# jirsat/wavenets

Measured on AMD Instinct MI355X. Metric: audio samples/sec (training step, 16 kHz mu-law), higher is better.
Workload: dtype f32 (fp16 hi|lo split operands, fp32 accumulate)

## Files before the change

### include/wn_hip.h

```cpp
#ifndef WN_HIP_H
#define WN_HIP_H
#include <stdint.h>

#ifdef __cplusplus
extern "C" {
#endif

#define WN_OK 0
#define WN_E_INVALID (-1)
#define WN_E_UNSUPPORTED (-2)
#define WN_E_HIP (-3)

#define WN_ACT_LINEAR 0
#define WN_ACT_RELU 1
#define WN_ACT_LEAKY_RELU 2
#define WN_ACT_TANH 3
#define WN_ACT_SIGMOID 4
#define WN_ACT_ELU 5

#define WN_HEAD_CATEGORICAL 0
#define WN_HEAD_LOGISTIC 1
#define WN_HEAD_GAUSSIAN 2

#define WN_MAX_FINAL 8
#define WN_MAX_MAPPING 8

typedef struct wn_config {
  int32_t kernel_size;
  int32_t channels;
  int32_t blocks;
  int32_t layers_per_block;
  int32_t activation;
  int32_t dilation_bound;
  int32_t num_mixtures;
  int32_t head;
  int32_t bits;
  int32_t skip_channels;
  int32_t dilation_channels;
  int32_t use_residual;
  int32_t use_skip;
  int32_t n_final;
  int32_t final_channels[WN_MAX_FINAL];
  int32_t cond_inputs;
  int32_t n_mapping;
  int32_t mapping_channels[WN_MAX_MAPPING];
  int32_t mapping_activation;
  float l2_reg_factor;
} wn_config;

typedef struct wn_plan wn_plan;

const char* wn_last_error_string(void);

wn_plan* wn_plan_create(const wn_config* cfg);
void wn_plan_destroy(wn_plan* p);

typedef struct wn_exec wn_exec;
wn_exec* wn_exec_create(const wn_plan* p);
void wn_exec_destroy(wn_exec* e);
int wn_exec_bind(wn_exec* e);
int64_t wn_plan_param_count(const wn_plan* p);
int32_t wn_plan_num_tensors(const wn_plan* p);
int wn_plan_tensor_info(const wn_plan* p, int32_t idx, int64_t* offset, int64_t* len,
                        int32_t* ndim, int64_t* shape3, int32_t* is_kernel);
int32_t wn_plan_receptive_field(const wn_plan* p);
int32_t wn_plan_out_channels(const wn_plan* p);
int32_t wn_plan_dilation(const wn_plan* p, int32_t conv_index);
int64_t wn_plan_workspace_floats(const wn_plan* p, int32_t B, int32_t T, int32_t training);

int wn_plan_set_dropout(wn_plan* p, float rate, uint64_t seed, uint64_t step);
uint32_t wn_dropout_key_for(uint64_t seed, int32_t block, uint64_t step);

int wn_debug_set(int key, int value);
int wn_debug_value(int key);
int wn_debug_gen_ts(unsigned long long* out_96);
int wn_plan_describe(const wn_plan* p, char* buf, int32_t len);
int wn_prof_enable(wn_plan* p, int32_t max_launches);
int wn_prof_read(wn_plan* p, int32_t* launches, float* avg_ms);
int wn_debug_ws_region(const wn_plan* p, int32_t B, int32_t T, int32_t what, int32_t idx, int64_t* off,
                       int64_t* len);
int wn_debug_eval_region(const wn_plan* p, int32_t B, int32_t T, int32_t what, int64_t* off, int64_t* len);
int wn_debug_fwd_paths(const wn_plan* p, int32_t B, int32_t T, int32_t training, int32_t loss, char* buf, int32_t len);
int wn_stack_prof_enable(wn_plan* p, int32_t max_passes);
int wn_stack_prof_read(wn_plan* p, int32_t* passes, float* avg_ms);
int wn_stack_prof_read_foldprep(wn_plan* p, int32_t* passes, float* avg_ms);
int wn_phase_enable(wn_plan* p, int32_t on);
int wn_phase_read(wn_plan* p, float* ms4);

int wn_forward(wn_plan* p, const float* params, const float* x, const float* cond, int32_t B,
               int32_t T, float* out, float* logits_out, float* workspace, int64_t ws_floats,
               void* stream);

int wn_forward_training(wn_plan* p, const float* params, const float* x, const float* cond, int32_t B,
                        int32_t T, float* out, float* logits_out, float* workspace, int64_t ws_floats,
                        void* stream);

int wn_train_fwd_bwd(wn_plan* p, const float* params, const float* x_full, const float* cond,
                     int32_t B, int32_t T, int32_t global_batch, int32_t n_replicas, float* grads,
                     float* loss_out, float* pred_out, float* workspace, int64_t ws_floats,
                     void* stream);

int wn_vjp(wn_plan* p, const float* params, const float* x, const float* cond, int32_t B, int32_t T,
           const float* g_out, int32_t g_kind, float* grads, float* g_x, float* g_cond,
           float* workspace, int64_t ws_floats, void* stream);

int wn_eval_loss(wn_plan* p, const float* params, const float* x_full, const float* cond,
                 int32_t B, int32_t T, int32_t global_batch, float* loss_out, float* pred_out,
                 float* workspace, int64_t ws_floats, void* stream);

int wn_score(wn_plan* p, const float* params, const float* x_full, const float* cond, int32_t B, int32_t T,
             float* nll_out, float* weight_out, float* rows_out, float* flag_out,
             float* workspace, int64_t ws_floats, void* stream);

int wn_adam_step(wn_plan* p, float* params, const float* grads, float* m, float* v, int64_t step,
                 float lr, float beta1, float beta2, float eps, float clipnorm, float* scratch,
                 void* stream);
int wn_adam_step_guarded(wn_plan* p, float* params, const float* grads, float* m, float* v, int64_t step,
                         float lr, float beta1, float beta2, float eps, float clipnorm, float* scratch,
                         const float* skip_flag, void* stream);
int wn_adam_step_ema(wn_plan* p, float* params, const float* grads, float* m, float* v, float* ema, int64_t step,
                     float lr, float beta1, float beta2, float eps, float clipnorm, float ema_momentum,
                     int32_t ema_overwrite, float* scratch, const float* skip_flag, void* stream);

int wn_clip_gradients(wn_plan* p, float* grads, float clipnorm, float* scratch, void* stream);

int64_t wn_plan_range_slot(const wn_plan* p, int32_t B, int32_t T, int32_t training);
float wn_range_limit(void);

int wn_generate(wn_plan* p, const float* params, const float* window, const float* cond, int32_t B,
                int32_t length, int32_t deterministic, int32_t queued, uint64_t seed, float* out,
                float* workspace, int64_t ws_floats, void* stream);
typedef struct wn_sampling { float temperature; int32_t top_k; uint64_t seed; float top_p; } wn_sampling;
int wn_generate_sampled(wn_plan* p, const float* params, const float* window, const float* cond, int32_t B,
                        int32_t length, int32_t deterministic, int32_t queued, const wn_sampling* sampling, float* out,
                        float* workspace, int64_t ws_floats, void* stream);
int wn_generate_chunk(wn_plan* p, const float* params, const float* window, const float* cond, int32_t B,
                      int64_t first, int32_t length, int32_t deterministic, int32_t queued, const wn_sampling* sampling,
                      float* out, float* workspace, int64_t ws_floats, void* stream);
typedef struct wn_sampling_row { float T, inv_T; int32_t top_k; float top_p; uint64_t seed, stream; } wn_sampling_row;
#define WN_SAMPLING_ROWS_ON 1
#define WN_SAMPLING_ROWS_TOP_P 2
int64_t wn_sampling_rows_floats(int32_t B);
int wn_sampling_rows_pack(const wn_sampling* sampling, const uint64_t* stream, int32_t B, int32_t head, int32_t classes,
                          wn_sampling_row* rows, int32_t* flags);
int wn_generate_rows_chunk(wn_plan* p, const float* params, const float* window, const float* cond, int32_t B,
                           int64_t first, int32_t length, int32_t deterministic, int32_t queued,
                           const wn_sampling_row* rows, int32_t rows_flags, float* out, float* workspace,
                           int64_t ws_floats, void* stream);
int wn_generate_rows_begin(wn_plan* p, const float* params, const float* window, const float* cond, int32_t B,
                           int64_t first, int32_t length, int32_t deterministic, int32_t queued,
                           const wn_sampling_row* rows, int32_t rows_flags, float* out, float* workspace,
                           int64_t ws_floats, void* stream);
int64_t wn_generate_admit_scratch_floats(const wn_plan* p, int32_t k);
int wn_generate_admit(wn_plan* p, const float* params, const float* windows, const float* cond, int32_t k,
                      const int32_t* slots, int32_t B, int64_t position, int32_t deterministic,
                      const wn_sampling_row* rows_k, int32_t rows_flags_k, float* first_out, float* workspace,
                      int64_t ws_floats, float* scratch, int64_t scratch_floats, void* stream);
int wn_generate_admit_describe(const wn_plan* p, int32_t k, int32_t B, char* buf, int32_t len);
int64_t wn_generate_workspace_floats(const wn_plan* p, int32_t B, int32_t queued);
int wn_generate_state_range(const wn_plan* p, int32_t B, int32_t queued, int64_t* offset, int64_t* floats);
int64_t wn_generate_guard_slot(const wn_plan* p, int32_t B, int32_t queued);

typedef struct wn_layer_desc {
  int32_t kernel_size, channels, dilation_channels, skip_channels ;
  int32_t depth;
  int32_t dilations[16];
  int32_t activation, residual, cond_channels ;
  int32_t in_channels;
} wn_layer_desc;
int64_t wn_layer_saved_floats(const wn_layer_desc* d, int32_t B, int32_t T);
int64_t wn_layer_workspace_floats(const wn_layer_desc* d, int32_t B, int32_t T);
int wn_layer_fwd(const wn_layer_desc* d, const float* params, const float* x, const float* cond,
                 int32_t B, int32_t T, float* x_out, float* skip_out, float* saved,
                 float* workspace, void* stream);
int wn_layer_bwd(const wn_layer_desc* d, const float* params, const float* x, const float* cond,
                 const float* saved, const float* g_x_out, const float* g_skip, int32_t B, int32_t T,
                 float* g_x, float* g_cond, float* g_params, float* workspace, void* stream);
int64_t wn_layer_param_count(const wn_layer_desc* d);
int wn_layer_describe(const wn_layer_desc* d, int32_t B, int32_t T, char* buf, int32_t len);

int wn_quantize(const float* x, int32_t* idx, int64_t n, int32_t bits, void* stream);
int wn_dequantize(const int32_t* idx, float* x, int64_t n, int32_t bits, void* stream);
int wn_mulaw(const float* x, float* y, int64_t n, void* stream);
int wn_inv_mulaw(const float* y, float* x, int64_t n, void* stream);
int wn_loss_fn(int32_t head, const void* target, const float* pred, int64_t rows, int32_t C,
               int32_t num_mixtures, int32_t bits, float* loss_rows, void* stream);
int wn_plan_arm_step_sample(wn_plan* plan, float* sample_out, int32_t deterministic, uint64_t seed, uint64_t offset);
int wn_plan_set_train_phases(wn_plan* plan, int32_t phases);
int wn_sum_squared_error(const float* a, const float* b, int64_t n, float scale, float* out, float* scratch,
                         void* stream);
int wn_plan_arm_row_weights(wn_plan* plan, const float* w, int64_t rows);
int wn_weighted_squared_error(const float* a, const float* b, const float* w, int64_t n, float scale, float* out,
                              float* scratch, void* stream);
int wn_sample_waveform(int32_t head, const float* pred, int64_t rows, int32_t C,
                       int32_t num_mixtures, int32_t bits, int32_t deterministic, uint64_t seed,
                       uint64_t offset, float* out, void* stream);
int wn_sample_waveform_sampled(int32_t head, const float* pred, int64_t rows, int32_t C,
                               int32_t num_mixtures, int32_t bits, int32_t deterministic, const wn_sampling* sampling,
                               uint64_t offset, float* out, void* stream);

#ifdef __cplusplus
}
#endif
#endif
```

### wavenets_amd/_lib.py

```python
from __future__ import annotations

import ctypes as C
import os
import subprocess

_HERE = os.path.dirname(os.path.abspath(__file__))
LIB_PATH = os.environ.get('WN_HIP_LIB') or os.path.join(_HERE, 'libwn_hip.so')

WN_OK, WN_E_INVALID, WN_E_UNSUPPORTED, WN_E_HIP = 0, -1, -2, -3
ACTIVATIONS = {None: 0, 'linear': 0, 'relu': 1, 'leaky_relu': 2, 'tanh': 3, 'sigmoid': 4, 'elu': 5}
HEADS = {'categorical': 0, 'logistic': 1, 'gaussian': 2}
WN_MAX_FINAL = 8
WN_MAX_MAPPING = 8
WN_TOP_K_MAX_CLASSES = 1024


class WnConfig(C.Structure):
  _fields_ = [
      ('kernel_size', C.c_int32), ('channels', C.c_int32), ('blocks', C.c_int32),
      ('layers_per_block', C.c_int32), ('activation', C.c_int32), ('dilation_bound', C.c_int32),
      ('num_mixtures', C.c_int32), ('head', C.c_int32), ('bits', C.c_int32),
      ('skip_channels', C.c_int32), ('dilation_channels', C.c_int32), ('use_residual', C.c_int32),
      ('use_skip', C.c_int32), ('n_final', C.c_int32), ('final_channels', C.c_int32 * WN_MAX_FINAL),
      ('cond_inputs', C.c_int32), ('n_mapping', C.c_int32),
      ('mapping_channels', C.c_int32 * WN_MAX_MAPPING), ('mapping_activation', C.c_int32),
      ('l2_reg_factor', C.c_float),
  ]


class WnSampling(C.Structure):
  _fields_ = [('temperature', C.c_float), ('top_k', C.c_int32), ('seed', C.c_uint64), ('top_p', C.c_float)]


class WnSamplingRow(C.Structure):
  _fields_ = [('T', C.c_float), ('inv_T', C.c_float), ('top_k', C.c_int32), ('top_p', C.c_float), ('seed', C.c_uint64),
              ('stream', C.c_uint64)]


WN_SAMPLING_ROWS_ON, WN_SAMPLING_ROWS_TOP_P = 1, 2


class WnLayerDesc(C.Structure):
  _fields_ = [
      ('kernel_size', C.c_int32), ('channels', C.c_int32), ('dilation_channels', C.c_int32),
      ('skip_channels', C.c_int32), ('depth', C.c_int32), ('dilations', C.c_int32 * 16),
      ('activation', C.c_int32), ('residual', C.c_int32), ('cond_channels', C.c_int32),
      ('in_channels', C.c_int32),
  ]


def build_library(verbose: bool = False) -> str:
  cmd = ['make', '-C', os.path.join(_HERE, 'csrc'), '-j8']
  res = subprocess.run(cmd, capture_output=not verbose, text=True)
  if res.returncode != 0:
    raise RuntimeError('building libwn_hip.so failed:\n' + (res.stdout or '') + (res.stderr or ''))
  return LIB_PATH


_P = C.c_void_p
_SIGS = {
    'wn_last_error_string': (C.c_char_p, []),
    'wn_plan_create': (_P, [C.POINTER(WnConfig)]),
    'wn_plan_destroy': (None, [_P]),
    'wn_plan_param_count': (C.c_int64, [_P]),
    'wn_plan_num_tensors': (C.c_int32, [_P]),
    'wn_plan_tensor_info': (C.c_int, [_P, C.c_int32, C.POINTER(C.c_int64), C.POINTER(C.c_int64),
                                      C.POINTER(C.c_int32), C.POINTER(C.c_int64), C.POINTER(C.c_int32)]),
    'wn_plan_receptive_field': (C.c_int32, [_P]),
    'wn_plan_out_channels': (C.c_int32, [_P]),
    'wn_plan_dilation': (C.c_int32, [_P, C.c_int32]),
    'wn_plan_workspace_floats': (C.c_int64, [_P, C.c_int32, C.c_int32, C.c_int32]),
    'wn_debug_set': (C.c_int, [C.c_int, C.c_int]),
    'wn_exec_create': (_P, [_P]),
    'wn_exec_destroy': (None, [_P]),
    'wn_exec_bind': (C.c_int, [_P]),
    'wn_debug_value': (C.c_int, [C.c_int]),
    'wn_debug_gen_ts': (C.c_int, [_P]),
    'wn_plan_set_dropout': (C.c_int, [_P, C.c_float, C.c_uint64, C.c_uint64]),
    'wn_dropout_key_for': (C.c_uint32, [C.c_uint64, C.c_int32, C.c_uint64]),
    'wn_plan_describe': (C.c_int, [_P, C.c_char_p, C.c_int32]),
    'wn_prof_enable': (C.c_int, [_P, C.c_int32]),
    'wn_prof_read': (C.c_int, [_P, C.POINTER(C.c_int32), C.POINTER(C.c_float)]),
    'wn_debug_ws_region': (C.c_int, [_P, C.c_int32, C.c_int32, C.c_int32, C.c_int32, C.POINTER(C.c_int64),
                                     C.POINTER(C.c_int64)]),
    'wn_debug_eval_region': (C.c_int, [_P, C.c_int32, C.c_int32, C.c_int32, C.POINTER(C.c_int64), C.POINTER(C.c_int64)]),
    'wn_debug_fwd_paths': (C.c_int, [_P, C.c_int32, C.c_int32, C.c_int32, C.c_int32, C.c_char_p, C.c_int32]),
    'wn_stack_prof_enable': (C.c_int, [_P, C.c_int32]),
    'wn_stack_prof_read': (C.c_int, [_P, C.POINTER(C.c_int32), C.POINTER(C.c_float)]),
    'wn_stack_prof_read_foldprep': (C.c_int, [_P, C.POINTER(C.c_int32), C.POINTER(C.c_float)]),
    'wn_phase_enable': (C.c_int, [_P, C.c_int32]),
    'wn_phase_read': (C.c_int, [_P, C.POINTER(C.c_float)]),
    'wn_forward': (C.c_int, [_P, _P, _P, _P, C.c_int32, C.c_int32, _P, _P, _P, C.c_int64, _P]),
    'wn_forward_training': (C.c_int, [_P, _P, _P, _P, C.c_int32, C.c_int32, _P, _P, _P, C.c_int64, _P]),
    'wn_train_fwd_bwd': (C.c_int, [_P, _P, _P, _P, C.c_int32, C.c_int32, C.c_int32, C.c_int32, _P, _P, _P,
                                   _P, C.c_int64, _P]),
    'wn_vjp': (C.c_int, [_P, _P, _P, _P, C.c_int32, C.c_int32, _P, C.c_int32, _P, _P, _P, _P, C.c_int64, _P]),
    'wn_eval_loss': (C.c_int, [_P, _P, _P, _P, C.c_int32, C.c_int32, C.c_int32, _P, _P, _P, C.c_int64, _P]),
    'wn_score': (C.c_int, [_P, _P, _P, _P, C.c_int32, C.c_int32, _P, _P, _P, _P, _P, C.c_int64, _P]),
    'wn_adam_step': (C.c_int, [_P, _P, _P, _P, _P, C.c_int64, C.c_float, C.c_float, C.c_float, C.c_float,
                               C.c_float, _P, _P]),
    'wn_adam_step_guarded': (C.c_int, [_P, _P, _P, _P, _P, C.c_int64, C.c_float, C.c_float, C.c_float, C.c_float,
                                       C.c_float, _P, _P, _P]),
    'wn_adam_step_ema': (C.c_int, [_P, _P, _P, _P, _P, _P, C.c_int64, C.c_float, C.c_float, C.c_float, C.c_float,
                                   C.c_float, C.c_float, C.c_int32, _P, _P, _P]),
    'wn_clip_gradients': (C.c_int, [_P, _P, C.c_float, _P, _P]),
    'wn_plan_range_slot': (C.c_int64, [_P, C.c_int32, C.c_int32, C.c_int32]),
    'wn_range_limit': (C.c_float, []),
    'wn_generate': (C.c_int, [_P, _P, _P, _P, C.c_int32, C.c_int32, C.c_int32, C.c_int32, C.c_uint64, _P,
                              _P, C.c_int64, _P]),
    'wn_generate_sampled': (C.c_int, [_P, _P, _P, _P, C.c_int32, C.c_int32, C.c_int32, C.c_int32, C.POINTER(WnSampling), _P,
                                      _P, C.c_int64, _P]),
    'wn_generate_chunk': (C.c_int, [_P, _P, _P, _P, C.c_int32, C.c_int64, C.c_int32, C.c_int32, C.c_int32,
                                    C.POINTER(WnSampling), _P, _P, C.c_int64, _P]),
    'wn_sampling_rows_floats': (C.c_int64, [C.c_int32]),
    'wn_sampling_rows_pack': (C.c_int, [C.POINTER(WnSampling), C.POINTER(C.c_uint64), C.c_int32, C.c_int32, C.c_int32,
                                        C.POINTER(WnSamplingRow), C.POINTER(C.c_int32)]),
    'wn_generate_rows_chunk': (C.c_int, [_P, _P, _P, _P, C.c_int32, C.c_int64, C.c_int32, C.c_int32, C.c_int32, _P,
                                         C.c_int32, _P, _P, C.c_int64, _P]),
    'wn_generate_rows_begin': (C.c_int, [_P, _P, _P, _P, C.c_int32, C.c_int64, C.c_int32, C.c_int32, C.c_int32, _P,
                                         C.c_int32, _P, _P, C.c_int64, _P]),
    'wn_generate_admit_scratch_floats': (C.c_int64, [_P, C.c_int32]),
    'wn_generate_admit': (C.c_int, [_P, _P, _P, _P, C.c_int32, C.POINTER(C.c_int32), C.c_int32, C.c_int64, C.c_int32, _P,
                                    C.c_int32, _P, _P, C.c_int64, _P, C.c_int64, _P]),
    'wn_generate_admit_describe': (C.c_int, [_P, C.c_int32, C.c_int32, C.c_char_p, C.c_int32]),
    'wn_generate_state_range': (C.c_int, [_P, C.c_int32, C.c_int32, C.POINTER(C.c_int64), C.POINTER(C.c_int64)]),
    'wn_generate_workspace_floats': (C.c_int64, [_P, C.c_int32, C.c_int32]),
    'wn_generate_guard_slot': (C.c_int64, [_P, C.c_int32, C.c_int32]),
    'wn_layer_saved_floats': (C.c_int64, [C.POINTER(WnLayerDesc), C.c_int32, C.c_int32]),
    'wn_layer_workspace_floats': (C.c_int64, [C.POINTER(WnLayerDesc), C.c_int32, C.c_int32]),
    'wn_layer_param_count': (C.c_int64, [C.POINTER(WnLayerDesc)]),
    'wn_layer_fwd': (C.c_int, [C.POINTER(WnLayerDesc), _P, _P, _P, C.c_int32, C.c_int32, _P, _P, _P, _P, _P]),
    'wn_layer_bwd': (C.c_int, [C.POINTER(WnLayerDesc), _P, _P, _P, _P, _P, _P, C.c_int32, C.c_int32, _P, _P,
                               _P, _P, _P]),
    'wn_layer_describe': (C.c_int, [C.POINTER(WnLayerDesc), C.c_int32, C.c_int32, C.c_char_p, C.c_int32]),
    'wn_quantize': (C.c_int, [_P, _P, C.c_int64, C.c_int32, _P]),
    'wn_dequantize': (C.c_int, [_P, _P, C.c_int64, C.c_int32, _P]),
    'wn_mulaw': (C.c_int, [_P, _P, C.c_int64, _P]),
    'wn_inv_mulaw': (C.c_int, [_P, _P, C.c_int64, _P]),
    'wn_loss_fn': (C.c_int, [C.c_int32, _P, _P, C.c_int64, C.c_int32, C.c_int32, C.c_int32, _P, _P]),
    'wn_plan_arm_step_sample': (C.c_int, [_P, _P, C.c_int32, C.c_uint64, C.c_uint64]),
    'wn_plan_set_train_phases': (C.c_int, [_P, C.c_int32]),
    'wn_sum_squared_error': (C.c_int, [_P, _P, C.c_int64, C.c_float, _P, _P, _P]),
    'wn_plan_arm_row_weights': (C.c_int, [_P, _P, C.c_int64]),
    'wn_weighted_squared_error': (C.c_int, [_P, _P, _P, C.c_int64, C.c_float, _P, _P, _P]),
    'wn_sample_waveform': (C.c_int, [C.c_int32, _P, C.c_int64, C.c_int32, C.c_int32, C.c_int32, C.c_int32,
                                     C.c_uint64, C.c_uint64, _P, _P]),
    'wn_sample_waveform_sampled': (C.c_int, [C.c_int32, _P, C.c_int64, C.c_int32, C.c_int32, C.c_int32, C.c_int32,
                                             C.POINTER(WnSampling), C.c_uint64, _P, _P]),
}
EXPORTS = tuple(_SIGS)

_lib = None


def lib() -> C.CDLL:
  global _lib
  if _lib is None:
    if not os.path.exists(LIB_PATH):
      raise RuntimeError(
          f'{LIB_PATH} is missing: build it with `python -c "import __graft_entry__ as g; g.build()"` '
          '(wavenets_amd has no CPU fallback)')
    l = C.CDLL(LIB_PATH)
    for name, (res, args) in _SIGS.items():
      fn = getattr(l, name)
      fn.restype = res
      fn.argtypes = args
    _lib = l
  return _lib


class WnError(RuntimeError):
  pass


def check(rc: int) -> None:
  if rc == WN_OK:
    return
  msg = lib().wn_last_error_string().decode()
  if rc == WN_E_INVALID:
    raise ValueError(msg)
  if rc == WN_E_UNSUPPORTED:
    raise NotImplementedError(msg)
  raise WnError(f'HIP error: {msg}')


def ptr(t):
  return None if t is None else C.c_void_p(t.data_ptr())


def stream_ptr():
  import torch
  return C.c_void_p(torch.cuda.current_stream().cuda_stream)
```

### wavenets_amd/csrc/wn_forward.hip

```cpp
#include "wn_plan_internal.h"

namespace {

__global__ void wn_ring_capture_kernel(const float* src, int B, int T, int C, int nslots, float* ring, int64_t t0) {
  const int64_t n = (int64_t)nslots * B * C;
  for (int64_t i = (int64_t)blockIdx.x * blockDim.x + threadIdx.x; i < n; i += (int64_t)gridDim.x * blockDim.x) {
    const int c = (int)(i % C);
    const int b = (int)((i / C) % B);
    const int k = (int)(i / ((int64_t)C * B));
    const int t = T - nslots + k;
    if (t >= 0) ring[((int64_t)((t + t0) % nslots) * B + b) * C + c] = src[((int64_t)b * T + t) * C + c];
  }
}

__global__ void wn_shift_split_kernel(const float* x_full, int B, int T, float* inputs, float* y_true) {
  const int64_t n = (int64_t)B * T;
  for (int64_t i = (int64_t)blockIdx.x * blockDim.x + threadIdx.x; i < n; i += (int64_t)gridDim.x * blockDim.x) {
    const int64_t b = i / T, t = i % T;
    inputs[i] = x_full[b * (T + 1) + t];
    y_true[i] = x_full[b * (T + 1) + t + 1];
  }
}

}

namespace wnp {

BlockPtrs block_ptrs(const wn_plan* p, int b, const float* params, const float* fragbase, int B, int T) {
  BlockPtrs k;
  memset(&k, 0, sizeof(k));
  const BlockInfo& bi = p->blocks[b];
  k.B = B; k.T = T; k.KS = p->KS; k.R = p->R; k.D = p->D; k.S = p->S; k.Cin = p->R; k.depth = p->LPB;
  k.act = p->c.activation; k.residual = p->c.use_residual;
  for (int i = 0; i < p->LPB; ++i) {
    const ConvInfo& c = bi.dil[i];
    k.dil[i] = c.dil;
    k.Wd[i] = params + p->tensors[c.kernel_t].off;
    k.bd[i] = params + p->tensors[c.bias_t].off;
    k.Fd[i] = fragbase + c.fragF; k.Fd_stride[i] = c.fragF_stride;
    k.Bd[i] = fragbase + c.fragB; k.Bd_stride[i] = c.fragB_stride;
  }
  k.br = params + p->tensors[bi.conv1.bias_t].off;
  k.Fr = fragbase + bi.conv1.fragF; k.Br_ = fragbase + bi.conv1.fragB;
  if (bi.has_skip) { k.bs = params + p->tensors[bi.conv_skip.bias_t].off; k.Bs = fragbase + bi.conv_skip.fragB; }
  k.Cc = 0; k.cond = nullptr; k.cb = nullptr;
  k.fused = p->fused_ok;
  if (p->fused16_ok && p->LPB == 1) { k.F16d = fragbase + bi.dil.back().frag16; k.F16r = fragbase + bi.conv1.frag16; }
  if (bi.f16gate >= 0) { k.F16g = fragbase + bi.f16gate; k.F16r = fragbase + bi.conv1.frag16; }
  if (bi.f16nat >= 0) k.F16n = fragbase + bi.f16nat;
  if (bi.g16u >= 0 && p->LPB == 1) k.G16u = fragbase + bi.g16u;
  if (bi.g16uf >= 0) k.G16uf = fragbase + bi.g16uf;
  if (p->LPB == 1 && bi.dil[0].frag16B >= 0) k.G16x = fragbase + bi.dil[0].frag16B;
  return k;
}

void deep16_ptrs(const wn_plan* p, int b, const float* fragbase, BlockPtrs& k) {
  if (!deep16(p)) return;
  const BlockInfo& bi = p->blocks[b];
  k.F16d = fragbase + bi.dil.back().frag16; k.F16r = fragbase + bi.conv1.frag16;
  for (int i = 0; i < p->LPB; ++i) {
    const ConvInfo& c = bi.dil[i];
    if (bi.d16F[i] >= 0) { k.F16i[i] = fragbase + bi.d16F[i]; k.JTi[i] = std::max(2, ceil32(c.cout)); }
    if (bi.d16B[i] >= 0) { k.G16i[i] = fragbase + bi.d16B[i]; k.JTb[i] = std::max(2, ceil32(c.cin)); }
  }
  if (bi.g16u >= 0) { k.G16u = fragbase + bi.g16u; k.JTu = std::max(2, ceil32(p->D)); }
}

int ring_capture(const float* src, int B, int T, int C, int nslots, float* ring, int64_t t0, hipStream_t s) {
  const int64_t n = (int64_t)nslots * B * C;
  hipLaunchKernelGGL(wn_ring_capture_kernel, dim3((unsigned)std::min<int64_t>((n + 255) / 256, 4096)), dim3(256), 0, s,
                     src, B, T, C, nslots, ring, t0);
  WN_HIP_CHECK(hipGetLastError());
  return WN_OK;
}

struct FwdCall {
  wn_exec& e;
  wn_plan* p; const float* params; const float* x; const float* cond; int B, T; bool training, prep;
  float* ws; const WsLayout& L; hipStream_t s; const GenRings* rings; LossFuse* lf;
  int64_t rows; float* fragbase;
  float* fam;
  FwdPaths fp;
  bool stack_prof = false;
  const float* hin = nullptr;

  FwdCall(wn_plan* p_, const float* params_, const float* x_, bool prep_, const float* cond_, int B_, int T_, bool training_,
          float* ws_, const WsLayout& L_, hipStream_t s_, const GenRings* rings_, LossFuse* lf_)
      : e(wnp::ex(p_)), p(p_), params(params_), x(x_), cond(cond_), B(B_), T(T_), training(training_), prep(prep_), ws(ws_),
        L(L_), s(s_), rings(rings_), lf(lf_), rows((int64_t)B_ * T_), fragbase(ws_ + L_.frag), fam(ws_ + L_.fwd_absmax),
        fp(fwd_paths(p_, e, B_, T_, training_, prep_, rings_ != nullptr, !lf_ ? FWD_LOSS_NONE : lf_->eval ? FWD_LOSS_EVAL : FWD_LOSS_TRAIN)) {}

  const float* par(int tensor) const { return params + p->tensors[tensor].off; }

  static bool pair_free(const std::vector<hipEvent_t>& ev, int used) { return used + 2 <= (int)ev.size(); }
  static void mark(const std::vector<hipEvent_t>& ev, int& used, bool stop, hipStream_t sp) {
    (void)hipEventRecord(ev[used + (stop ? 1 : 0)], sp);
    if (stop) used += 2;
  }

  int weight_images() {
    return prep ? wn_launch_prep_table(p->d_prep, (int)p->prep.size(), params, fragbase, s) : WN_OK;
  }

  int fold_prep(hipStream_t sp) {
    const bool fp_prof = fp.fold && pair_free(e.foldprep_ev, e.foldprep_used);
    if (fp_prof) mark(e.foldprep_ev, e.foldprep_used, false, sp);
    if (p->c.use_skip) {
      const ConvInfo& c0 = p->blocks[0].has_skip ? p->blocks[0].conv_skip : p->blocks[0].conv1;
      WnVecSumArgs v;
      v.base = params; v.off0 = p->tensors[c0.bias_t].off;
      v.stride = p->N > 1 ? (p->tensors[(p->blocks[1].has_skip ? p->blocks[1].conv_skip : p->blocks[1].conv1).bias_t].off - v.off0) : 0;
      v.count = p->N; v.len = p->Sh; v.out = ws + L.bias_sum;
      const int r = wn_launch_vecsum(v, sp);
      if (r) return r;
    }
    if (fp.fold) {
      const BlockInfo& b0 = p->blocks[0];
      const int64_t wst = p->N > 1 ? p->tensors[p->blocks[1].conv_skip.kernel_t].off - p->tensors[b0.conv_skip.kernel_t].off : 0;
      int r = wn_launch_skip_fold(params, p->tensors[b0.conv_skip.kernel_t].off, wst, p->tensors[p->finals[0].kernel_t].off,
                                  p->tensors[p->finals[0].bias_t].off, ws + L.bias_sum, p->N, p->D, p->S, p->fold_F0, ws + L.vfold,
                                  ws + L.bfold, ws + L.wsall, sp);
      if (r) return r;
      r = wn_launch_prep_table(p->d_prep2, (int)p->prep2.size(), ws, fragbase, sp, 64);
      if (r) return r;
    }
    if (fp_prof) mark(e.foldprep_ev, e.foldprep_used, true, sp);
    return WN_OK;
  }

  int fold_prep_fork() {
    if (!e.side) {
      WN_HIP_CHECK(hipStreamCreateWithFlags(&e.side, hipStreamNonBlocking));
      WN_HIP_CHECK(hipEventCreateWithFlags(&e.ev_fork, hipEventDisableTiming));
      WN_HIP_CHECK(hipEventCreateWithFlags(&e.ev_join, hipEventDisableTiming));
    }
    if (!e.ev_ffork) {
      WN_HIP_CHECK(hipEventCreateWithFlags(&e.ev_ffork, hipEventDisableTiming));
      WN_HIP_CHECK(hipEventCreateWithFlags(&e.ev_fjoin, hipEventDisableTiming));
    }
    WN_HIP_CHECK(hipEventRecord(e.ev_ffork, s));
    WN_HIP_CHECK(hipStreamWaitEvent(e.side, e.ev_ffork, 0));
    const int rc = fold_prep(e.side);
    if (rc) return rc;
    WN_HIP_CHECK(hipEventRecord(e.ev_fjoin, e.side));
    return WN_OK;
  }

  int condition() {
    if (fp.cond == FWD_COND_NONE) return WN_OK;
    if (!cond) { wn_set_error("Conditioning must be provided."); return WN_E_INVALID; }
    const bool small = fp.cond == FWD_COND_SMALL;
    const float* m = cond;
    int mc = p->c.cond_inputs, rc;
    for (size_t j = 0; j < p->mapping.size(); ++j) {
      const ConvInfo& c = p->mapping[j];
      if (small)
        rc = wn_launch_sgemm_small_batched(m, mc, 1, 0, par(c.kernel_t), c.cout, 1, 0, ws + L.M[j], c.cout, 0,
                                           B, c.cout, mc, 1, par(c.bias_t), p->c.mapping_activation, s);
      else
        rc = Gemm(1, B, c.cout, ceil32(c.cout)).seg(m, mc, mc, 0, fragbase + c.fragF)
                 .bias(par(c.bias_t)).act(p->c.mapping_activation).run(ws + L.M[j], c.cout, s);
      if (rc) return rc;
      m = ws + L.M[j]; mc = c.cout;
    }
    const int D2 = 2 * p->D;
    if (!fp.cond_batched) {
      for (int b = 0; b < p->N; ++b) {
        const ConvInfo& c = p->blocks[b].conv_cond;
        rc = Gemm(1, B, D2, ceil32(D2)).seg(m, p->Cc, p->Cc, 0, fragbase + c.fragF)
                 .bias(par(c.bias_t)).run(ws + L.cb + (int64_t)b * B * D2, D2, s);
        if (rc) return rc;
      }
      return WN_OK;
    }
    const ConvInfo& c0 = p->blocks[0].conv_cond;
    const int64_t bst = p->N > 1 ? p->tensors[p->blocks[1].conv_cond.bias_t].off - p->tensors[c0.bias_t].off : 0;
    if (small) {
      const int64_t wst = p->N > 1 ? p->tensors[p->blocks[1].conv_cond.kernel_t].off - p->tensors[c0.kernel_t].off : 0;
      rc = wn_launch_sgemm_small_batched(m, p->Cc, 1, 0, par(c0.kernel_t), D2, 1, wst, ws + L.cbt, p->N * D2, D2,
                                         B, D2, p->Cc, p->N, nullptr, 0, s);
    } else {
      rc = Gemm(1, B, p->N * D2, ceil32(p->N * D2)).seg(m, p->Cc, p->Cc, 0, fragbase + p->frag_condF).run(ws + L.cbt, p->N * D2, s);
    }
    if (rc) return rc;
    return wn_launch_cond_scatter(ws + L.cbt, params, p->tensors[c0.bias_t].off, bst, B, p->N, D2, ws + L.cb, s);
  }

  int input_conv() {
    WN_HIP_CHECK(hipMemsetAsync(fam, 0, sizeof(float), s));
    int rc;
    if (fp.inconv_elem) {
      rc = wn_launch_inconv_fwd(x, par(p->causal.kernel_t), par(p->causal.bias_t), B, T, p->R, p->KS, ws + L.H[0], fam, s);
    } else {
      Gemm g(B, T, p->R, ceil32(p->R));
      for (int t = 0; t < p->KS; ++t)
        g.seg(x, 1, 1, (p->KS - 1 - t), fragbase + p->causal.fragF + t * p->causal.fragF_stride);
      rc = g.bias(par(p->causal.bias_t)).run(ws + L.H[0], p->R, s);
    }
    if (rc) return rc;
    if (rings) {
      rc = ring_capture(x, B, T, 1, p->KS, rings->xin, rings->t0, s);
      if (!rc) rc = ring_capture(ws + L.H[0], B, T, p->R, rings->nslots[0], rings->h[0], rings->t0, s);
    }
    return rc;
  }

  int blocks() {
    int rc;
    if (fp.zfill) {
      rc = wn_launch_fill(ws + L.Z, 0.f, rows * p->N * p->Dp, s);
      if (rc) return rc;
    }
    const bool prof_chain = e.prof_on && !rings && p->LPB == 1 && p->c.cond_inputs == 0 && p->R == p->D && !fp.drop && p->fused_ok;
    stack_prof = !rings && pair_free(e.stack_ev, e.stack_used);
    if (stack_prof) mark(e.stack_ev, e.stack_used, false, s);
    if (fp.prep == FWD_PREP_SIDE) {
      rc = fold_prep_fork();
      if (rc) return rc;
    }
    for (int b = 0; b < p->N; ++b) {
      BlockPtrs k = block_ptrs(p, b, params, fragbase, B, T);
      if (fp.deep16) deep16_ptrs(p, b, fragbase, k);
      if (fp.cond != FWD_COND_NONE) k.cb = ws + L.cb + (int64_t)b * B * 2 * p->D;
      BlockBufs f;
      memset(&f, 0, sizeof(f));
      const int hi = training ? b : (b & 1), ho = training ? b + 1 : ((b + 1) & 1);
      f.x = ws + L.H[hi];
      if (fp.drop) {
        rc = wn_launch_dropout(ws + L.H[hi], nullptr, ws + L.XD[b], rows * p->R, e.drop_rate,
                               wn_dropout_key(e.drop_seed, b, e.drop_step), nullptr, s);
        if (rc) return rc;
        f.x = ws + L.XD[b];
        f.res = ws + L.H[hi];
      }
      for (int i = 0; i + 1 < p->LPB; ++i) f.P[i] = ws + L.P[b][i];
      f.U = ws + L.U;
      f.AG = training ? ws + L.AG[b] : nullptr;
      f.Z = ws + L.Z + (int64_t)b * rows * p->Dp; f.ldz = p->Dp;
      f.O = nullptr;
      f.x_out = ws + L.H[ho];
      f.fwd_absmax = fam;
      const bool prof = e.prof_on && pair_free(e.prof_ev, e.prof_used);
      if (prof && (!prof_chain || b == 0)) mark(e.prof_ev, e.prof_used, false, s);
      rc = block_forward(k, f, s);
      if (rc) return rc;
      if (prof && (!prof_chain || b == p->N - 1)) {
        e.prof_cnt[e.prof_used / 2] = prof_chain ? p->N : 1;
        mark(e.prof_ev, e.prof_used, true, s);
      }
      if (rings && b + 1 < p->N) {
        rc = ring_capture(f.x_out, B, T, p->R, rings->nslots[b + 1], rings->h[b + 1], rings->t0, s);
        if (rc) return rc;
      }
      if (rings)
        for (int i = 0; i + 1 < p->LPB; ++i) {
          rc = ring_capture(f.P[i], B, T, p->D, rings->nslots_p[b][i], rings->hp[b][i], rings->t0, s);
          if (rc) return rc;
        }
    }
    if (fp.prep == FWD_PREP_SIDE) WN_HIP_CHECK(hipStreamWaitEvent(s, e.ev_fjoin, 0));
    return WN_OK;
  }

  int skip() {
    int rc = WN_OK;
    switch (fp.skip) {
      case FWD_SKIP_FOLD_PLANES:
        rc = Planes(B, T, fp.hc0).operand(ws + L.Z, p->Dp, p->D, p->N, rows * p->Dp).w16(fragbase + p->frag16_foldF)
                 .bias(ws + L.bfold).act(p->c.activation).absmax_fwd(fam).run(ws + L.HA[0], fp.hc0, s);
        hin = ws + L.HA[0];
        break;
      case FWD_SKIP_FOLD_ROWS:
        rc = Gemm(B, T, fp.hc0, ceil32(fp.hc0)).seg_planes(ws + L.Z, p->Dp, rows * p->Dp, p->N * p->Dp, nullptr)
                 .w16(fragbase + p->frag16_foldF).bias(ws + L.bfold).act(p->c.activation).absmax_fwd(fam)
                 .run(ws + L.HA[0], fp.hc0, s);
        hin = ws + L.HA[0];
        break;
      case FWD_SKIP_SUM:
        rc = Gemm(B, T, p->Sh, ceil32(p->Sh)).seg_planes(ws + L.Z, p->Dp, rows * p->Dp, p->N * p->Dp, fragbase + p->frag_skipF)
                 .w16(p->frag16_skipF >= 0 ? fragbase + p->frag16_skipF : nullptr)
                 .bias(ws + L.bias_sum).absmax_fwd(fam).run(ws + L.skipsum, p->Sh, s);
        hin = ws + L.skipsum;
        break;
      case FWD_SKIP_NONE:
        hin = ws + L.H[training ? p->N : (p->N & 1)];
        break;
    }
    if (rc) return rc;
    if (stack_prof) mark(e.stack_ev, e.stack_used, true, s);
    return WN_OK;
  }

  int head() {
    int hc = fp.hc0;
    for (int i = fp.first_final; i < fp.nhead; ++i) {
      const ConvInfo& c = p->finals[i];
      const bool last = (i + 1 == fp.nhead);
      float* dst = last ? ws + L.logits : ws + L.HA[i];
      int rc;
      switch (fp.head[i]) {
        case FWD_HEAD_EPILOGUE:
          rc = Planes(B, T, c.cout).operand(hin, hc, hc).w16(fragbase + c.frag16).bias(par(c.bias_t)).act(WN_ACT_LINEAR)
                   .loss(*lf).run(lf->g_logits, c.cout, s);
          if (rc) return rc;
          lf->done = true;
          return WN_OK;
        case FWD_HEAD_PLANES:
          rc = Planes(B, T, c.cout).operand(hin, hc, hc).w16(fragbase + c.frag16).bias(par(c.bias_t))
                   .act(last ? WN_ACT_LINEAR : p->c.activation).absmax_fwd(last ? nullptr : fam).run(dst, c.cout, s);
          break;
        default:
          rc = Gemm(B, T, c.cout, ceil32(c.cout)).seg(hin, hc, hc, 0, fragbase + c.fragF)
                   .w16(c.frag16 >= 0 ? fragbase + c.frag16 : nullptr)
                   .bias(par(c.bias_t)).act(last ? WN_ACT_LINEAR : p->c.activation)
                   .absmax_fwd(last ? nullptr : fam).run(dst, c.cout, s);
          break;
      }
      if (rc) return rc;
      hin = dst; hc = c.cout;
    }
    return WN_OK;
  }
};

int forward_core(wn_plan* p, const float* params, const float* x, bool prep, const float* cond, int B,
                 int T, bool training, float* ws, const WsLayout& L, hipStream_t s, const GenRings* rings, LossFuse* lf) {
  int rc = ensure_device_tables(p);
  if (rc) return rc;
  FwdCall c(p, params, x, prep, cond, B, T, training, ws, L, s, rings, lf);
  if ((rc = c.weight_images())) return rc;
  if (c.fp.prep == FWD_PREP_INLINE && (rc = c.fold_prep(s))) return rc;
  if ((rc = c.condition())) return rc;
  if ((rc = c.input_conv())) return rc;
  if ((rc = c.blocks())) return rc;
  if ((rc = c.skip())) return rc;
  return c.head();
}

int emit_outputs(const wn_plan* p, const float* ws, const WsLayout& L, int64_t rows, float* logits_out, float* out, hipStream_t s) {
  const size_t bytes = rows * p->Cout * sizeof(float);
  if (logits_out) WN_HIP_CHECK(hipMemcpyAsync(logits_out, ws + L.logits, bytes, hipMemcpyDeviceToDevice, s));
  if (!out) return WN_OK;
  if (p->c.head == WN_HEAD_CATEGORICAL) return wn_launch_softmax(ws + L.logits, out, rows, p->Cout, s);
  WN_HIP_CHECK(hipMemcpyAsync(out, ws + L.logits, bytes, hipMemcpyDeviceToDevice, s));
  return WN_OK;
}

int shift_split(const float* x_full, int B, int T, float* inputs, float* y_true, hipStream_t s) {
  const int64_t rows = (int64_t)B * T;
  hipLaunchKernelGGL(wn_shift_split_kernel, dim3((unsigned)std::min<int64_t>((rows + 255) / 256, 4096)), dim3(256), 0, s,
                     x_full, B, T, inputs, y_true);
  WN_HIP_CHECK(hipGetLastError());
  return WN_OK;
}

bool loss_fusable(const wn_plan* p, int64_t rows) {
  if (p->c.head != WN_HEAD_CATEGORICAL || p->Cout != 256 || wn_debug_get(1) == 1 || p->finals.empty()) return false;
  const ConvInfo& c = p->finals.back();
  return c.frag16 >= 0 && c.cout == 256 && rows > 0;
}

int loss_stage(wn_plan* p, int B, int T, int global_batch, bool want_grad, float* ws, const WsLayout& L,
               float* loss_out, float* absmax_out, hipStream_t s, bool fused_done, const float* row_weight) {
  const int64_t rows = (int64_t)B * T;
  const float gscale = 1.0f / (float)global_batch;
  int rc;
  if (fused_done) return wn_launch_sum(ws + L.loss_rows, rows, gscale, loss_out, ws + L.sum_scratch, s);
  float* g_logits = want_grad ? ws + L.GF.back() : nullptr;
  rc = loss_rows_stage(p, rows, gscale, g_logits, want_grad, ws, L, absmax_out, s, row_weight);
  if (rc) return rc;
  return wn_launch_sum(ws + L.loss_rows, rows, gscale, loss_out, ws + L.sum_scratch, s);
}

int loss_rows_stage(wn_plan* p, int64_t rows, float gscale, float* g_logits, bool want_grad, float* ws, const WsLayout& L,
                    float* absmax_out, hipStream_t s, const float* row_weight) {
  int rc;
  if (p->c.head == WN_HEAD_CATEGORICAL) {
    rc = wn_launch_quantize(ws + L.yt, reinterpret_cast<int32_t*>(ws + L.target), rows, p->c.bits, s);
    if (rc) return rc;
    float* so = nullptr;
    if (want_grad && wnp::ex(p).step_sample && !wnp::ex(p).step_sample_det && p->Cout <= 256) { so = wnp::ex(p).step_sample; wnp::ex(p).step_sample = nullptr; }
    rc = wn_launch_cat_loss(ws + L.logits, reinterpret_cast<const int32_t*>(ws + L.target), rows, p->Cout,
                            gscale, ws + L.loss_rows, g_logits, absmax_out, s, so, p->c.bits, wnp::ex(p).step_sample_seed,
                            wnp::ex(p).step_sample_off, row_weight);
  } else {
    rc = wn_launch_mix_loss(ws + L.logits, ws + L.yt, rows, p->c.num_mixtures, p->c.bits,
                            p->c.head == WN_HEAD_LOGISTIC ? 1 : 2, gscale, ws + L.loss_rows, g_logits, absmax_out, s, row_weight);
  }
  return rc;
}

int row_weights_check(const char* who, const wn_exec& e, int B, int T) {
  if (!e.row_weights || e.row_weights_n == (int64_t)B * T) return WN_OK;
  wn_set_error("%s: the armed row weights cover %lld rows, the call has B * T = %lld", who, (long long)e.row_weights_n,
               (long long)((int64_t)B * T));
  return WN_E_INVALID;
}

}

using namespace wnp;

static int forward_entry(const char* who, bool training, wn_plan* p, const float* params, const float* x, const float* cond,
                         int32_t B, int32_t T, float* out, float* logits_out, float* workspace, int64_t ws_floats, void* stream) {
  if (!p || !params || !x || !workspace || B < 1 || T < 1) { wn_set_error("%s: bad arguments", who); return WN_E_INVALID; }
  hipStream_t s = (hipStream_t)stream;
  const WsLayout L = make_layout(p, B, T, training);
  if (ws_floats < L.total) { wn_set_error("%s: workspace too small (%lld < %lld floats)", who, (long long)ws_floats, (long long)L.total); return WN_E_INVALID; }
  const int rc = forward_core(p, params, x, true, cond, B, T, training, workspace, L, s);
  if (rc) return rc;
  return emit_outputs(p, workspace, L, (int64_t)B * T, logits_out, out, s);
}

extern "C" int wn_forward(wn_plan* p, const float* params, const float* x, const float* cond, int32_t B,
                          int32_t T, float* out, float* logits_out, float* workspace, int64_t ws_floats,
                          void* stream) {
  return forward_entry("forward", false, p, params, x, cond, B, T, out, logits_out, workspace, ws_floats, stream);
}

extern "C" int wn_forward_training(wn_plan* p, const float* params, const float* x, const float* cond, int32_t B,
                                   int32_t T, float* out, float* logits_out, float* workspace, int64_t ws_floats,
                                   void* stream) {
  return forward_entry("forward_training", true, p, params, x, cond, B, T, out, logits_out, workspace, ws_floats, stream);
}

extern "C" int wn_eval_loss(wn_plan* p, const float* params, const float* x_full, const float* cond,
                            int32_t B, int32_t T, int32_t global_batch, float* loss_out, float* pred_out,
                            float* workspace, int64_t ws_floats, void* stream) {
  if (!p || !params || !x_full || !workspace || !loss_out || B < 1 || T < 1) { wn_set_error("eval_loss: bad arguments"); return WN_E_INVALID; }
  if (row_weights_check("eval_loss", wnp::ex(p), B, T)) return WN_E_INVALID;
  hipStream_t s = (hipStream_t)stream;
  const WsLayout L = make_layout(p, B, T, false);
  if (ws_floats < L.total) { wn_set_error("eval_loss: workspace too small"); return WN_E_INVALID; }
  const int64_t rows = (int64_t)B * T;
  float* inputs = workspace + L.probs;
  { const int rcs = shift_split(x_full, B, T, inputs, workspace + L.yt, s); if (rcs) return rcs; }
  int rc = forward_core(p, params, inputs, true, cond, B, T, false, workspace, L, s);
  if (rc) return rc;
  rc = loss_stage(p, B, T, global_batch > 0 ? global_batch : B, false, workspace, L, loss_out, nullptr, s, false,
                  wnp::ex(p).row_weights);
  if (rc) return rc;
  rc = wn_launch_guard_flag(workspace + L.fwd_absmax, WN_RANGE_LIMIT, wn_debug_get(1) != 1, loss_out + 2, s);
  if (rc) return rc;
  return emit_outputs(p, workspace, L, rows, nullptr, pred_out, s);
}

extern "C" int wn_score(wn_plan* p, const float* params, const float* x_full, const float* cond, int32_t B, int32_t T,
                        float* nll_out, float* weight_out, float* rows_out, float* flag_out,
                        float* workspace, int64_t ws_floats, void* stream) {
  if (!p) { wn_set_error("score: null plan"); return WN_E_INVALID; }
  if (!params || !x_full || !nll_out || !flag_out || !workspace) {
    wn_set_error("score: null %s", !params ? "params" : !x_full ? "x_full" : !nll_out ? "nll_out" : !flag_out ? "flag_out" : "workspace");
    return WN_E_INVALID;
  }
  if (p->c.cond_inputs > 0 && !cond) { wn_set_error("score: the plan is conditioned (%d inputs) and cond is null", p->c.cond_inputs); return WN_E_INVALID; }
  if (B < 1 || T < 1) { wn_set_error("score: B = %d, T = %d: both must be at least 1", (int)B, (int)T); return WN_E_INVALID; }
  if (row_weights_check("score", wnp::ex(p), B, T)) return WN_E_INVALID;
  hipStream_t s = (hipStream_t)stream;
  const WsLayout L = make_layout(p, B, T, false);
  if (ws_floats < L.total) {
    wn_set_error("score: workspace too small (%lld < %lld floats)", (long long)ws_floats, (long long)L.total);
    return WN_E_INVALID;
// ... 29 lines not shown
```

### wavenets_amd/csrc/wn_gemm16s.hip

```cpp
#include "wn_split16.h"
#include "wn_sample.h"

using namespace wn_split16;

namespace {

template <int RT, int JT_>
struct GS {
  static constexpr int JT = JT_;
  static constexpr int CHUNK = JT * 2048, NBUF = 3;
  static constexpr int XB = 3, XBUF = RT * 2048;
  static constexpr int WAVES = 4, THREADS = 256;
  static constexpr int PITCH = 36, STAGE = 32 * PITCH * 4;
  static constexpr int REGION = XB * XBUF;
  static constexpr int LDS = NBUF * CHUNK + WAVES * REGION + 32 * JT * 4;
  static constexpr int PT = CHUNK / 16 / THREADS;
  static constexpr int PX = 2 * RT;
  static_assert(STAGE <= REGION, "the output stage lives in the activation ring");
};

}

template <int RT, int JT_, int ACT, bool SHIFT = false>
__global__ __launch_bounds__(256, 2) void wn_gemm_planes16s_kernel(WnGemmPlanesArgs a) {
  using C = GS<RT, JT_>;
  constexpr int JT = C::JT, PT = C::PT, PX = C::PX, PITCH = C::PITCH;
  __shared__ __attribute__((aligned(16))) unsigned char smem[C::LDS];
  const int tid = threadIdx.x;
  const int lane = tid & 63, wave = __builtin_amdgcn_readfirstlane(tid >> 6);
  const int tl = lane & 31, h = lane >> 5;
  unsigned char* const xbuf = smem + C::NBUF * C::CHUNK + wave * C::REGION;
  float* stage = reinterpret_cast<float*>(xbuf);
  const unsigned smem_addr = lds_addr_of(smem), xbuf_addr = lds_addr_of(xbuf);
  float* sbias = reinterpret_cast<float*>(smem + C::NBUF * C::CHUNK + C::WAVES * C::REGION);
  if (tid < 32 * JT) sbias[tid] = (a.bias && tid < a.N) ? a.bias[tid] : 0.f;
  const bool has_bias = a.bias != nullptr;
  __syncthreads();
  float sc = 1.0f, inv_sc = 1.0f;
  if (ACT == -2 && a.absmax_in) pow2_scale(*a.absmax_in, sc, inv_sc);

  const int kpp = a.plane_k >> 4;
  const int nsteps = a.nplanes * kpp;
  const int tiles_per_b = (a.T + 32 * RT - 1) / (32 * RT);
  const int64_t ntiles = (int64_t)a.B * tiles_per_b;
  const int64_t per_pass = (int64_t)gridDim.x * C::WAVES;
  const int passes = (int)((ntiles + per_pass - 1) / per_pass);

  const unsigned woff = (unsigned)tid * 16u;
  const char* const wimg = reinterpret_cast<const char*>(a.w16);
  int ws_next = 0, ws_slot = 0;
  auto wpiece = [&](int i) {
    dma16(wimg + (int64_t)ws_next * C::CHUNK + 4096 * i, woff, smem_addr + ws_slot * C::CHUNK + (C::THREADS * i + wave * 64) * 16);
  };
  auto wadvance = [&]() {
    ws_next = ws_next + 1 == nsteps ? 0 : ws_next + 1;
    ws_slot = ws_slot + 1 == C::NBUF ? 0 : ws_slot + 1;
  };
#pragma unroll
  for (int i = 0; i < PT; ++i) wpiece(i);
  wadvance();
#pragma unroll
  for (int i = 0; i < PT; ++i) wpiece(i);
  wadvance();
  int slot = 0;
  float wmax = 0.f;

  for (int pass = 0; pass < passes; ++pass) {
    const int64_t tile = ((int64_t)pass * gridDim.x + blockIdx.x) * C::WAVES + wave;
    const bool live = tile < ntiles;
    const int b = live ? (int)(tile / tiles_per_b) : 0;
    const int t0 = live ? (int)(tile % tiles_per_b) * 32 * RT : 0;
    const int64_t row0 = (int64_t)b * a.T + t0;
    unsigned xoff[RT];
    bool xok[RT];
#pragma unroll
    for (int rt = 0; rt < RT; ++rt) {
      const int t = t0 + 32 * rt + tl;
      xok[rt] = live && t < a.T;
      xoff[rt] = (unsigned)(((int64_t)b * a.T + (xok[rt] ? t : 0)) * a.ld + 4 * h) * 4u;
    }
    const char* xs_base = reinterpret_cast<const char*>(a.z);
    int xs_k = 0, xs_buf = 0, xs_p = 0;
    auto shifted = [&](int rt, int pl, bool& ok) -> unsigned {
      const int sh = pl == 0 ? a.shift[0] : (pl == 1 ? a.shift[1] : (pl == 2 ? a.shift[2] : a.shift[3]));
      const int t = t0 + 32 * rt + tl, ts = t - sh;
      ok = live && t < a.T && ts >= 0 && ts < a.T;
      return (unsigned)(((int64_t)b * a.T + (ok ? ts : 0)) * a.ld + 4 * h) * 4u;
    };
    auto xdma = [&]() {
      const char* base = xs_base + 64 * xs_k;
      const unsigned dst = xbuf_addr + xs_buf * C::XBUF;
#pragma unroll
      for (int rt = 0; rt < RT; ++rt) {
        bool okd;
        const unsigned off = SHIFT ? shifted(rt, xs_p, okd) : xoff[rt];
        dma16(base, off, dst + rt * 2048);
        dma16(base + 32, off, dst + rt * 2048 + 1024);
      }
      if (++xs_k == kpp) { xs_k = 0; xs_base += a.plane_stride * 4; ++xs_p; }
      xs_buf = xs_buf + 1 == C::XB ? 0 : xs_buf + 1;
    };

    f32x16 acc[RT][JT];
#pragma unroll
    for (int rt = 0; rt < RT; ++rt)
#pragma unroll
      for (int j = 0; j < JT; ++j)
#pragma unroll
        for (int r = 0; r < 16; ++r) acc[rt][j][r] = 0.f;

    xdma();
    xdma();
    int xcur = 0;
    int cs_k = 0, cs_p = 0;
    auto step = [&](auto wait_, bool xnext) {
      constexpr int WAIT = decltype(wait_)::value;
      asm volatile("s_waitcnt vmcnt(%0)" ::"n"(WAIT) : "memory");
      asm volatile("s_barrier" ::: "memory");
      const h8* wl = reinterpret_cast<const h8*>(smem + slot * C::CHUNK) + lane;
      const f32x4* xl = reinterpret_cast<const f32x4*>(xbuf + xcur * C::XBUF) + lane;
      h8 bh[RT], bl[RT];
#pragma unroll
      for (int rt = 0; rt < RT; ++rt) {
        f32x4 q0 = xl[rt * 128], q1 = xl[rt * 128 + 64];
        bool okc = xok[rt];
        if constexpr (SHIFT) (void)shifted(rt, cs_p, okc);
        if (!okc) { q0 = f32x4{0.f, 0.f, 0.f, 0.f}; q1 = q0; }
        if constexpr (ACT == -2) split8s(q0, q1, sc, bh[rt], bl[rt]);
        else split8(q0, q1, bh[rt], bl[rt]);
      }
      h8 fr[2][2];
      fr[0][0] = wl[0];
      fr[0][1] = wl[64];
      wn_static_for<JT>([&](auto jc) {
        constexpr int j = decltype(jc)::value;
        if constexpr (j + 1 < JT) {
          fr[(j + 1) & 1][0] = wl[((j + 1) * 2 + 0) * 64];
          fr[(j + 1) & 1][1] = wl[((j + 1) * 2 + 1) * 64];
        }
#pragma unroll
        for (int rt = 0; rt < RT; ++rt) {
          mfma3(fr[j & 1][0], fr[j & 1][1], bh[rt], bl[rt], acc[rt][j]);
        }
        if constexpr (j < PT) wpiece(j);
        if constexpr (j == PT) { if (xnext) xdma(); }
        __builtin_amdgcn_sched_barrier(0);
      });
      wadvance();
      slot = slot + 1 == C::NBUF ? 0 : slot + 1;
      xcur = xcur + 1 == C::XB ? 0 : xcur + 1;
      if (++cs_k == kpp) { cs_k = 0; ++cs_p; }
    };
    step(std::integral_constant<int, PX>{}, true);
    for (int c = 1; c + 1 < nsteps; ++c) step(std::integral_constant<int, PT + PX>{}, c + 2 < nsteps);
    step(std::integral_constant<int, PT>{}, false);

    const unsigned voff = (unsigned)(lane >> 3) * (unsigned)(a.ldy * 4) + (unsigned)(lane & 7) * 16u;
    if constexpr (ACT <= -3) {
      constexpr bool WEIGHTED = ACT == -4 || ACT == -6;
      constexpr bool EVAL = ACT <= -5;
      static_assert(RT == 1 && JT == 8, "the loss epilogue is the 256-class form");
      const int rows_valid = live ? max(0, min(32, a.T - t0)) : 0;
      const bool rok = xok[0];
      const int64_t row = row0 + tl;
      int tgt = rok ? a.target[row] : 0;
      tgt = wn_ce_target(tgt, 256);
      float rw = 1.0f;
      [[maybe_unused]] float gscale = EVAL ? 0.f : a.gscale;
      if constexpr (WEIGHTED) {
        rw = rok ? a.row_weight[row] : 0.f;
        if constexpr (!EVAL) gscale = wn_w_gscale(gscale, rw);
      }
      auto xch = [](float v) { return __shfl_xor(v, 32); };
      float m = -INFINITY;
#pragma unroll
      for (int j = 0; j < JT; ++j)
#pragma unroll
        for (int rq = 0; rq < 4; ++rq) {
          const f32x4 bv = *reinterpret_cast<const f32x4*>(sbias + 32 * j + 8 * rq + 4 * h);
          acc[0][j][4 * rq + 0] += bv.x; acc[0][j][4 * rq + 1] += bv.y; acc[0][j][4 * rq + 2] += bv.z; acc[0][j][4 * rq + 3] += bv.w;
          m = fmaxf(fmaxf(m, fmaxf(acc[0][j][4 * rq + 0], acc[0][j][4 * rq + 1])), fmaxf(acc[0][j][4 * rq + 2], acc[0][j][4 * rq + 3]));
        }
      m = fmaxf(m, xch(m));
      float tsum[JT];
      float z = 0.f;
#pragma unroll
      for (int j = 0; j < JT; ++j) {
        float ts = 0.f;
#pragma unroll
        for (int r = 0; r < 16; ++r) { acc[0][j][r] = __builtin_amdgcn_exp2f(1.4426950408889634f * (acc[0][j][r] - m)); ts += acc[0][j][r]; }
        ts += xch(ts);
        tsum[j] = ts;
        z += ts;
      }
      const float inv = 1.0f / z;
      if (!EVAL && a.sample_out) {
        uint32_t rnd[4];
        wn_philox((uint64_t)row, a.offset, a.seed, rnd);
        const float thr = wn_u01(rnd[0]) * (z * inv);
        float run = 0.f, before = 0.f;
        int jsel = JT - 1;
        bool found = false;
#pragma unroll
        for (int j = 0; j < JT; ++j) {
          const float nxt = run + tsum[j] * inv;
          if (!found && nxt > thr) { found = true; jsel = j; before = run; }
          run = nxt;
        }
        float qv[16];
#pragma unroll
        for (int r = 0; r < 16; ++r) {
          float v = acc[0][0][r];
#pragma unroll
          for (int j = 1; j < JT; ++j) v = jsel == j ? acc[0][j][r] : v;
          qv[r] = v * inv;
        }
        float gown[4], goth[4];
#pragma unroll
        for (int rq = 0; rq < 4; ++rq) {
          gown[rq] = (qv[4 * rq] + qv[4 * rq + 1]) + (qv[4 * rq + 2] + qv[4 * rq + 3]);
          goth[rq] = xch(gown[rq]);
        }
        int kstar = 7;
        float runb = before, rr = before;
        bool fk = false;
#pragma unroll
        for (int k = 0; k < 8; ++k) {
          const float gk = ((k & 1) == h) ? gown[k >> 1] : goth[k >> 1];
          const float nxt = rr + gk;
          if (!fk && nxt > thr) { fk = true; kstar = k; runb = rr; }
          rr = nxt;
        }
        const int rqs = kstar >> 1;
        float r_ = runb;
        int es = 3;
        bool fe = false;
#pragma unroll
        for (int e = 0; e < 4; ++e) {
          const float ve = rqs == 0 ? qv[e] : (rqs == 1 ? qv[4 + e] : (rqs == 2 ? qv[8 + e] : qv[12 + e]));
          r_ += ve;
          if (!fe && r_ > thr) { fe = true; es = e; }
        }
        const int mine = 32 * jsel + 8 * rqs + 4 * h + es;
        const int theirs = __shfl_xor(mine, 32);
        const int drawn = ((kstar & 1) == h) ? mine : theirs;
        if (rok && h == 0) a.sample_out[row] = (float)drawn * a.inv_lv - 1.0f;
      }
      float S = 0.f, A = 0.f, qt = 0.f;
#pragma unroll
      for (int j = 0; j < JT; ++j)
#pragma unroll
        for (int r = 0; r < 16; ++r) {
          const float q = acc[0][j][r] * inv;
          if constexpr (!EVAL) acc[0][j][r] = q;
          S += wn_ce_clip(q);
          if constexpr (!EVAL) { if (wn_ce_inside(q)) A += q; }
          if (32 * j + 8 * (r >> 2) + 4 * h + (r & 3) == tgt) qt = q;
        }
      S += xch(S);
      if constexpr (!EVAL) A += xch(A);
      qt += xch(qt);
      if constexpr (EVAL) {
        const float pt = wn_ce_clip(qt);
        if (rok && h == 0) a.loss_rows[row] = WEIGHTED ? wn_w_loss(rw, wn_ce_loss(pt, S)) : wn_ce_loss(pt, S);
        continue;
      }
      const WnCeRow ce(S, A, qt);
      if (rok && h == 0) a.loss_rows[row] = WEIGHTED ? wn_w_loss(rw, wn_ce_loss(ce.pt, S)) : wn_ce_loss(ce.pt, S);
#pragma unroll
      for (int j = 0; j < JT; ++j) {
#pragma unroll
        for (int r = 0; r < 16; ++r) {
          const float q = acc[0][j][r];
          float gl = ce.grad(q, 32 * j + 8 * (r >> 2) + 4 * h + (r & 3) == tgt, gscale);
          if constexpr (WEIGHTED) gl = wn_w_grad(rw, gl);
          acc[0][j][r] = gl;
          if (rok) wmax = fmaxf(wmax, fabsf(gl));
        }
        if (rows_valid > 0) {
          float* dst = a.y + row0 * a.ldy + 32 * j;
          if (rows_valid == 32) store_tile<PITCH, true>(acc[0][j], stage, dst, voff, (unsigned)(a.ldy * 4), rows_valid, lane);
          else store_tile<PITCH, false>(acc[0][j], stage, dst, voff, (unsigned)(a.ldy * 4), rows_valid, lane);
        }
      }
      continue;
    }
#pragma unroll
    for (int rt = 0; rt < RT; ++rt) {
      const int rows_valid = live ? max(0, min(32, a.T - (t0 + 32 * rt))) : 0;
      if (rows_valid <= 0) continue;
#pragma unroll
      for (int j = 0; j < JT; ++j) {
        if (32 * j >= a.N) continue;
#pragma unroll
        for (int rq = 0; rq < 4; ++rq) {
          const int n0 = 32 * j + 8 * rq + 4 * h;
          float v[4] = {acc[rt][j][4 * rq + 0], acc[rt][j][4 * rq + 1], acc[rt][j][4 * rq + 2], acc[rt][j][4 * rq + 3]};
          if constexpr (ACT == -2) {
#pragma unroll
            for (int e = 0; e < 4; ++e) v[e] *= inv_sc;
          }
          if (has_bias) {
            const f32x4 bv = *reinterpret_cast<const f32x4*>(sbias + n0);
            v[0] += bv.x; v[1] += bv.y; v[2] += bv.z; v[3] += bv.w;
          }
          if constexpr (ACT == -2) {
            if (a.aux && xok[rt]) {
              const f32x4 yv = *(const __attribute__((address_space(1))) f32x4*)(a.aux + (row0 + 32 * rt + tl) * a.ld_aux + n0);
              v[0] *= wn_dact_from_y(yv.x, a.act); v[1] *= wn_dact_from_y(yv.y, a.act);
              v[2] *= wn_dact_from_y(yv.z, a.act); v[3] *= wn_dact_from_y(yv.w, a.act);
            }
          } else {
#pragma unroll
            for (int e = 0; e < 4; ++e) v[e] = wn_act(v[e], ACT >= 0 ? ACT : a.act);
          }
          if (xok[rt]) wmax = wn_absmax_acc(wmax, v[0], v[1], v[2], v[3]);
          acc[rt][j][4 * rq + 0] = v[0]; acc[rt][j][4 * rq + 1] = v[1]; acc[rt][j][4 * rq + 2] = v[2]; acc[rt][j][4 * rq + 3] = v[3];
        }
        float* dst = a.y + (row0 + 32 * rt) * a.ldy + 32 * j;
        if (rows_valid == 32) store_tile<PITCH, true>(acc[rt][j], stage, dst, voff, (unsigned)(a.ldy * 4), rows_valid, lane);
        else store_tile<PITCH, false>(acc[rt][j], stage, dst, voff, (unsigned)(a.ldy * 4), rows_valid, lane);
      }
    }
  }
  asm volatile("s_waitcnt vmcnt(0)" ::: "memory");
  if (ACT > -5 && a.absmax_out) {
    wmax = wn_wave_absmax_bits(wmax);
    if (lane == 0) { if (ACT == -2 || ACT == -3 || ACT == -4) wn_absmax_publish(a.absmax_out, wmax); else wn_absmax_publish_any(a.absmax_out, wmax); }
  }
}

int wn_gemm_taps16s_supported(int N, int plane_k, int ntaps, int ld, int ldy) {
  return (N == 32 || N == 64) && ntaps >= 1 && ntaps <= 4 && plane_k >= 16 && plane_k % 16 == 0 && ntaps * (plane_k / 16) >= 3 &&
         ld % 4 == 0 && ld >= plane_k && ldy % 4 == 0 && ldy >= N;
}

int wn_gemm_planes16s_supported(int N, int plane_k, int nplanes, int ld, int ldy) {
  return (N == 128 || N == 256) && plane_k >= 16 && plane_k % 16 == 0 && nplanes * (plane_k / 16) >= 3 && ld % 4 == 0 && ld >= plane_k && ldy % 4 == 0 &&
         ldy >= N;
}

int wn_launch_gemm_planes16s(const WnGemmPlanesArgs& a, hipStream_t s) {
  if (!(a.nshift > 0 ? wn_gemm_taps16s_supported(a.N, a.plane_k, a.nplanes, a.ld, a.ldy)
                     : wn_gemm_planes16s_supported(a.N, a.plane_k, a.nplanes, a.ld, a.ldy))) {
    wn_set_error("gemm_planes16s: unsupported shape N=%d plane_k=%d planes=%d", a.N, a.plane_k, a.nplanes);
    return WN_E_UNSUPPORTED;
  }
  if ((int64_t)a.B * a.T * a.ld * 4 >= (int64_t)1 << 32) { wn_set_error("gemm_planes16s: plane beyond 4 GiB"); return WN_E_UNSUPPORTED; }
  if ((int64_t)a.B * a.T <= 0) return WN_OK;
  const int rt = a.N == 256 ? 1 : 2;
  const int64_t tiles = (int64_t)a.B * ((a.T + 32 * rt - 1) / (32 * rt));
  int64_t gx = (tiles + 3) / 4;
  if (gx > 512) gx = 512;
#define WN_GS_LAUNCH(RT_, JT_, ACT_) hipLaunchKernelGGL((wn_gemm_planes16s_kernel<RT_, JT_, ACT_>), dim3((unsigned)gx), dim3(256), 0, s, a)
#define WN_GS_LAUNCH_S(ACT_) hipLaunchKernelGGL((wn_gemm_planes16s_kernel<2, 2, ACT_, true>), dim3((unsigned)gx), dim3(256), 0, s, a)
  if (a.N <= 64) {
    if (a.nshift != a.nplanes || a.plane_stride != 0 || a.nplanes > 4) { wn_set_error("gemm_planes16s: narrow outputs are the shifted form"); return WN_E_UNSUPPORTED; }
    if (a.bwd) WN_GS_LAUNCH_S(-2);
    else switch (a.act) {
      case WN_ACT_LINEAR: WN_GS_LAUNCH_S(WN_ACT_LINEAR); break;
      case WN_ACT_RELU: WN_GS_LAUNCH_S(WN_ACT_RELU); break;
      case WN_ACT_LEAKY_RELU: WN_GS_LAUNCH_S(WN_ACT_LEAKY_RELU); break;
      default: WN_GS_LAUNCH_S(-1); break;
    }
  } else if (a.cat_loss) {
    const bool eval = a.cat_loss == 2;
    if (a.N != 256 || a.bwd || !a.target || !a.loss_rows || (!eval && !a.y)) { wn_set_error("gemm_planes16s: the loss epilogue is the 256-class forward form"); return WN_E_UNSUPPORTED; }
    if (eval) { if (a.row_weight) WN_GS_LAUNCH(1, 8, -6); else WN_GS_LAUNCH(1, 8, -5); }
    else if (a.row_weight) WN_GS_LAUNCH(1, 8, -4);
    else WN_GS_LAUNCH(1, 8, -3);
  } else if (a.bwd) {
    if (a.N == 256) WN_GS_LAUNCH(1, 8, -2);
    else WN_GS_LAUNCH(2, 4, -2);
  } else if (a.N == 256) switch (a.act) {
    case WN_ACT_LINEAR: WN_GS_LAUNCH(1, 8, WN_ACT_LINEAR); break;
    case WN_ACT_RELU: WN_GS_LAUNCH(1, 8, WN_ACT_RELU); break;
    case WN_ACT_LEAKY_RELU: WN_GS_LAUNCH(1, 8, WN_ACT_LEAKY_RELU); break;
    default: WN_GS_LAUNCH(1, 8, -1); break;
  }
  else switch (a.act) {
    case WN_ACT_LINEAR: WN_GS_LAUNCH(2, 4, WN_ACT_LINEAR); break;
    case WN_ACT_RELU: WN_GS_LAUNCH(2, 4, WN_ACT_RELU); break;
    case WN_ACT_LEAKY_RELU: WN_GS_LAUNCH(2, 4, WN_ACT_LEAKY_RELU); break;
    default: WN_GS_LAUNCH(2, 4, -1); break;
  }
#undef WN_GS_LAUNCH
#undef WN_GS_LAUNCH_S
  WN_HIP_CHECK(hipGetLastError());
  return WN_OK;
}
```

### wavenets_amd/csrc/wn_kernels.h

```cpp
#pragma once
#include "wn_common.h"

struct WnTensorDesc { int64_t off; int64_t len; };

struct WnPrepDesc {
  int64_t src_off;
  int64_t dst_off;
  int32_t I;
  int32_t KK;
  int32_t ld;
  int32_t transpose;
  int32_t q_off;
  int32_t j_off;
  int32_t JT;
  int32_t kind;
};
int wn_launch_prep_table(const WnPrepDesc* d_table, int n, const float* params, float* ws,
                         hipStream_t s, int gx = 16);
int wn_launch_prep_one(WnPrepDesc d, const float* params, float* ws, hipStream_t s);
struct WnVecSumArgs { const float* base; int64_t off0; int64_t stride; int32_t count; int32_t len; float* out; };
int wn_launch_vecsum(WnVecSumArgs a, hipStream_t s);

#define WN_MAXSEG 4
struct WnSeg {
  const float* x;
  const float* frag;
  int32_t ldx;
  int32_t K;
  int32_t shift;
  int32_t vec;
  int32_t plane_k;
  int64_t plane_stride;
};
struct WnGemmArgs {
  WnSeg seg[WN_MAXSEG];
  int32_t nseg;
  int32_t B, T;
  int32_t N;
  int32_t JTtot;
  const float* bias;
  const float* rowbias;
  int32_t ld_rowbias;
  const float* addc;
  int32_t ld_addc;
  int32_t act;
  int32_t epi;
  const float* aux;
  int32_t ld_aux;
  const float* aux2;
  int32_t ld_aux2;
  float* y;
  int32_t ldy;
  int32_t vec_out;
  float* y2;
  int32_t ld_y2;
  int32_t absmax_any;
};
int wn_launch_gemm_rows(const WnGemmArgs& a, hipStream_t s);
int wn_gemm_rows16_ok(const WnGemmArgs& a);
int wn_launch_gemm_rows16(const WnGemmArgs& a, const float* w16, const float* absmax_in0,
                          const float* absmax_in1, float* absmax_out, hipStream_t s);

struct WnGemmPlanesArgs {
  const float* z;
  int64_t plane_stride;
  int32_t ld, plane_k, nplanes;
  const float* w16;
  const float* bias;
  int32_t act;
  float* y; int32_t ldy;
  int32_t N;
  int32_t B, T;
  float* absmax_out;
  int32_t bwd;
  const float* absmax_in;
  const float* aux; int32_t ld_aux;
  int32_t nshift; int32_t shift[4];
  int32_t cat_loss;
  const int32_t* target;
  float gscale;
  float* loss_rows;
  float* sample_out;
  float inv_lv;
  uint64_t seed, offset;
  const float* row_weight;
};
int wn_gemm_planes16s_supported(int N, int plane_k, int nplanes, int ld, int ldy);
int wn_gemm_taps16s_supported(int N, int plane_k, int ntaps, int ld, int ldy);
int wn_launch_gemm_planes16s(const WnGemmPlanesArgs& a, hipStream_t s);

struct WnWgradArgs {
  const float* x; int32_t ldx; int32_t K; int32_t shift;
  const float* g; int32_t ldg; int32_t N;
  int32_t B, T;
  int32_t splits_per_b;
  float* slab;
  float* slab_bias;
};
int wn_wgrad_choose_splits(int B, int T, int K, int N);
int wn_launch_wgrad(const WnWgradArgs& a, hipStream_t s);
struct WnWgJob {
  int64_t x_off, g_off, out_off, bias_off;
  int64_t gmax_off;
  int32_t ldx, ldg, K, N, shift, k0, n0, pad_;
};
struct WnWgLayer {
  int64_t x_off, du_off, z_off, go_off;
  int64_t dwd_off, dbd_off, dwr_off, dbr_off;
  int64_t gmax_u_off, gmax_h_off;
  int32_t dilation, ldz;
};
int wn_wgrad_layer_supported(int R, int D, int KS);
int wn_launch_wgrad_layers(const WnWgLayer* d_layers, int nlayers, int R, float* ws, float* slab, int64_t P, int B,
                           int T, int splits_per_b, hipStream_t s, int inner = 0);
struct WnWgPair {
  int64_t x_off, g_off;
  int64_t w_off, b_off;
  int64_t gmax_off;
  int32_t shift;
  union { int32_t pad_; int32_t nseg; };
  union { int64_t g2_off; int64_t seg_stride; };
  int64_t w2_off, b2_off, gmax2_off;
  struct Seg { int64_t g_off, gmax_off, w_off, b_off; } seg[2];
};
int wn_wgrad_pair_kind(int K, int N);
int wn_launch_wgrad_pairs(int kind, const WnWgPair* d_jobs, int njobs, float* ws, float* slab, int64_t P, int B, int T,
                          int splits_per_b, hipStream_t s);
int wn_wgrad_tr_kind(int K, int N, int taps);
int wn_launch_wgrad_tr(int kind, const WnWgPair* d_jobs, int njobs, float* ws, float* slab, int64_t P, int B, int T,
                       int splits_per_b, hipStream_t s, float* slab2 = nullptr, int64_t P2 = 0);
struct WnBwdPairArgs {
  const float* gu_in;
  const float* gx_res;
  const float* gf;
  const float* ag;
  const float* z; int32_t ldz;
  float* gx_out;
  float* gu_out;
  const float* wx16;
  const float* wu16;
  const float* am_gu_in; const float* am_gf;
  float* am_gx; float* am_gu;
  int32_t B, T, dil;
};
int wn_bwd_pair_supported(int R, int D, int KS, int F0);
int wn_launch_bwd_pair(const WnBwdPairArgs& a, hipStream_t s);
int wn_bwd_s128_supported(int R, int D, int KS, int F0);
int wn_launch_bwd_s128(const WnBwdPairArgs& a, hipStream_t s);
int wn_wgrad_skip_supported(int D, int S, int KZ);
int wn_launch_wgrad_skip(const float* z, int ldz, const float* g, int ldg, int64_t rows, int KZ, int S, int D,
                         int nsplit, float* slab, int64_t P, int64_t w_off0, int64_t w_stride, int64_t b_off0,
                         int64_t b_stride, int nblocks, const float* gmax, hipStream_t s);
int wn_wgrad_tile_k();
int wn_wgrad_tile_n();
int wn_launch_wgrad_batched(const WnWgJob* d_jobs, int njobs, float* ws, float* slab, int64_t P, int B, int T,
                            int splits_per_b, hipStream_t s, bool exact_fp32 = false);
int wn_launch_reduce_table(const float* slab, int nsplit, int64_t P, float* out, const WnTensorDesc* d_table,
                           int n, hipStream_t s, const WnTensorDesc* h_table = nullptr);
struct WnReduceArgs {
  const float* slab; int32_t nsplit; int32_t K; int32_t N;
  float* out; int32_t seg_len; int64_t seg_stride; int32_t accumulate;
  int32_t replicate; int64_t rep_stride;
};
int wn_launch_reduce(const WnReduceArgs& a, hipStream_t s);
int wn_reduce_two_stage(int nsplit);

struct WnLayerFwdArgs {
  const float* x;
  const float* frag_d;
  const float* frag_r;
  const float* bias_d;
  const float* bias_r;
  const float* cb;
  float* x_out;
  float* o_out;
  float* z_out; int32_t ldz;
  float* ag_out;
  const float* res;
  const float* xt[3];
  int32_t B, T, R, D, KS, dilation, residual;
  float* absmax_out;
};
int wn_layer_fwd_supported(int R, int D, int KS);
int wn_layer_fwd_f16_supported(int R, int D, int KS);
int wn_launch_layer_fwd_f16(const WnLayerFwdArgs& a, hipStream_t s);
size_t wn_frag16_floats(int I, int KK);
int wn_layer_fwd_s128_supported(int R, int D, int KS);
int wn_launch_layer_fwd_s128(const WnLayerFwdArgs& a, hipStream_t s);
int wn_launch_layer_fwd(const WnLayerFwdArgs& a, hipStream_t s);
int wn_gen_block128_supported(int R, int D, int KS);
int wn_launch_gen_block128(const WnLayerFwdArgs& a, hipStream_t s);

struct WnGenBlock {
  int64_t ring_off;
  int64_t w16d_off;
  int64_t w16r_off;
  int64_t bias_d_off;
  int64_t bias_r_off;
  int64_t cb_off;
  int32_t nslots, dilation;
};
struct WnGenStepArgs {
  const float* params;
  float* ws;
  const WnGenBlock* blocks;
  const float* xin;
  const float* causal_w;
  const float* causal_b;
  int64_t zrow_off;
  int64_t hrow_off;
  int64_t skip_w16_off;
  int64_t skip_bias_off;
  int64_t skiprow_off;
  int32_t skip_tiles, skip_ld;
  int32_t skip_act, pad1_;
  int64_t u0_off;
  int64_t tau;
  int32_t B, nblocks, residual;
  int32_t ntiles;
  unsigned long long* ts;
  int64_t bias_r_off0, bias_r_stride;
  WnGenBlock blk0[3];
  float* guard;
};
struct WnGen128Args {
  const float* params;
  float* ws;
  const WnGenBlock* blocks;
  int64_t zrow_off;
// ... 138 lines not shown
```

### wavenets_amd/csrc/wn_plan.hip

```cpp
#include "wn_plan_internal.h"

#include <string>

namespace {
using namespace wnp;

int add_tensor(wn_plan* p, int ndim, int64_t s0, int64_t s1, int64_t s2, int is_kernel) {
  TensorInfo t;
  t.off = p->nparams;
  t.ndim = ndim;
  t.shape[0] = s0; t.shape[1] = s1; t.shape[2] = s2;
  t.len = s0 * (ndim > 1 ? s1 : 1) * (ndim > 2 ? s2 : 1);
  t.is_kernel = is_kernel;
  p->nparams += t.len;
  p->tensors.push_back(t);
  return (int)p->tensors.size() - 1;
}

ConvInfo add_conv(wn_plan* p, int taps, int cin, int cout, int dil) {
  ConvInfo c;
  c.taps = taps; c.cin = cin; c.cout = cout; c.dil = dil;
  c.kernel_t = add_tensor(p, 3, taps, cin, cout, 1);
  c.bias_t = add_tensor(p, 1, cout, 1, 1, 0);
  return c;
// ... 28 lines not shown
    c.fragB_stride = (int64_t)wn_frag_floats(c.cin, c.cout);
    for (int t = 0; t < c.taps; ++t) {
      WnPrepDesc d;
      memset(&d, 0, sizeof(d));
      d.src_off = k.off + (int64_t)t * c.cin * c.cout;
      d.dst_off = c.fragB + t * c.fragB_stride;
      d.I = c.cin; d.KK = c.cout; d.ld = c.cout; d.transpose = 0;
      d.q_off = 0; d.j_off = 0; d.JT = ceil32(c.cin);
      p->prep.push_back(d);
    }
    p->frag_floats += c.taps * c.fragB_stride;
  }
}

void add_image16(wn_plan* p, ConvInfo& c) {
  const TensorInfo& k = p->tensors[c.kernel_t];
  c.frag16 = p->frag_floats;
  for (int t = 0; t < c.taps; ++t) {
    WnPrepDesc d;
    memset(&d, 0, sizeof(d));
    d.src_off = k.off + (int64_t)t * c.cin * c.cout;
    d.dst_off = c.frag16;
    d.I = c.cout; d.KK = c.cin; d.ld = c.cout; d.transpose = 1;
    d.q_off = t * (c.cin / 16); d.j_off = 0; d.JT = ceil32(c.cout); d.kind = 1;
    p->prep.push_back(d);
  }
  p->frag_floats += (int64_t)wn_frag16_floats(c.cout, c.taps * c.cin);
}

int64_t new_image16(wn_plan* p, int I, int Ktotal) {
  const int64_t off = p->frag_floats;
  p->frag_floats += (int64_t)wn_frag16_floats(I, Ktotal);
  return off;
}
void add_piece16(wn_plan* p, int64_t img, int I, int64_t src_off, int KK, int ld, int transpose, int ks_off,
                 int j_off = 0, int JT_img = 0) {
  WnPrepDesc d;
  memset(&d, 0, sizeof(d));
  d.src_off = src_off; d.dst_off = img; d.I = I; d.KK = KK; d.ld = ld; d.transpose = transpose;
  d.q_off = ks_off; d.j_off = j_off; d.JT = JT_img > 0 ? JT_img : ceil32(I); d.kind = 1;
  p->prep.push_back(d);
}


int jobs_for(int K, int N) {
  return ((K + wn_wgrad_tile_k() - 1) / wn_wgrad_tile_k()) * ((N + wn_wgrad_tile_n() - 1) / wn_wgrad_tile_n());
}

int count_jobs(const wn_plan* p) {
  int n = p->KS * jobs_for(1, p->R);
  for (const BlockInfo& b : p->blocks) {
    n += p->KS * jobs_for(p->R, 2 * p->D) + jobs_for(p->D, p->R);
    for (int i = 0; i + 1 < p->LPB; ++i) n += p->KS * jobs_for(i == 0 ? p->R : p->D, p->D);
    if (b.has_skip && p->c.use_skip) n += jobs_for(p->D, p->S);
  }
  for (const ConvInfo& c : p->finals) n += jobs_for(c.cin, c.cout);
  return n;
}

}

namespace wnp {

int64_t slab_need(int B, int T, int K, int N) {
  const int sp = wn_wgrad_choose_splits(B, T, K, N);
  return (int64_t)B * sp * ((int64_t)K * N + N);
}

static thread_local wn_exec* g_bound_exec = nullptr;
wn_exec& ex(const wn_plan* p) {
  return (g_bound_exec && g_bound_exec->plan == p) ? *g_bound_exec : *p->own;
}

void exec_release(wn_exec* e) {
  if (!e) return;
  for (hipEvent_t ev : e->prof_ev) (void)hipEventDestroy(ev);
  for (hipEvent_t ev : e->stack_ev) (void)hipEventDestroy(ev);
  for (hipEvent_t ev : e->foldprep_ev) (void)hipEventDestroy(ev);
  for (hipEvent_t ev : e->phase_ev) if (ev) (void)hipEventDestroy(ev);
  e->wg.release();
  if (e->ev_fork) (void)hipEventDestroy(e->ev_fork);
  if (e->ev_join) (void)hipEventDestroy(e->ev_join);
  if (e->ev_ffork) (void)hipEventDestroy(e->ev_ffork);
  if (e->ev_fjoin) (void)hipEventDestroy(e->ev_fjoin);
  if (e->side) (void)hipStreamDestroy(e->side);
  e->gen.release();
  e->admit.release();
  if (g_bound_exec == e) g_bound_exec = nullptr;
  delete e;
}

int ensure_device_tables(wn_plan* p) {
  std::lock_guard<std::mutex> lock(p->tables_mu);
  if (p->tables_ready) return WN_OK;
  WN_HIP_CHECK(hipMalloc((void**)&p->d_prep, p->prep.size() * sizeof(WnPrepDesc)));
  WN_HIP_CHECK(hipMemcpy(p->d_prep, p->prep.data(), p->prep.size() * sizeof(WnPrepDesc), hipMemcpyHostToDevice));
  WN_HIP_CHECK(hipMalloc((void**)&p->d_tdesc, p->tdesc.size() * sizeof(WnTensorDesc)));
  WN_HIP_CHECK(hipMemcpy(p->d_tdesc, p->tdesc.data(), p->tdesc.size() * sizeof(WnTensorDesc), hipMemcpyHostToDevice));
  if (!p->kdesc.empty()) {
    WN_HIP_CHECK(hipMalloc((void**)&p->d_kdesc, p->kdesc.size() * sizeof(WnTensorDesc)));
    WN_HIP_CHECK(hipMemcpy(p->d_kdesc, p->kdesc.data(), p->kdesc.size() * sizeof(WnTensorDesc), hipMemcpyHostToDevice));
  }
  if (!p->prep2.empty()) {
    WN_HIP_CHECK(hipMalloc((void**)&p->d_prep2, p->prep2.size() * sizeof(WnPrepDesc)));
    WN_HIP_CHECK(hipMemcpy(p->d_prep2, p->prep2.data(), p->prep2.size() * sizeof(WnPrepDesc), hipMemcpyHostToDevice));
    WnTensorDesc d;
    d.off = 0; d.len = (int64_t)p->N * p->D * p->fold_F0 + p->fold_F0;
    WN_HIP_CHECK(hipMalloc((void**)&p->d_cov_fold, sizeof(WnTensorDesc)));
    WN_HIP_CHECK(hipMemcpy(p->d_cov_fold, &d, sizeof(WnTensorDesc), hipMemcpyHostToDevice));
    p->h_cov_fold = d;
  }
  p->tables_ready = true;
  return WN_OK;
}


bool deep16(const wn_plan* p) { return p->deep16_ok && wn_debug_get(1) != 1; }

bool cond_small(const wn_plan* p) {
  if (p->c.cond_inputs <= 0) return false;
  for (int b = 1; b < p->N; ++b) {
    const int64_t w0 = p->tensors[p->blocks[0].conv_cond.kernel_t].off, w1 = p->tensors[p->blocks[1].conv_cond.kernel_t].off;
    if (!p->blocks[b].has_cond || p->tensors[p->blocks[b].conv_cond.kernel_t].off != w0 + (int64_t)b * (w1 - w0)) return false;
  }
  return p->blocks[0].has_cond;
}

bool fold_ok(const wn_plan* p) { return p->fold_F0 > 0 && wn_debug_get(1) != 1; }

bool head_pairs_ok(const wn_plan* p) {
  if (p->finals.empty() || wn_debug_get(1) == 1) return false;
  for (size_t i = fold_ok(p) ? 1 : 0; i < p->finals.size(); ++i)
    if (wn_wgrad_pair_kind(p->finals[i].cin, p->finals[i].cout) != 0) return true;
  return false;
}

TrainPaths train_paths(const wn_plan* p) {
  TrainPaths t;
  const bool split = wn_debug_get(1) != 1;
  t.fold = fold_ok(p);
  t.deep16 = deep16(p);
  t.head_pairs = head_pairs_ok(p);
  t.skipk = p->c.use_skip && p->S > 0 && p->Dp == p->D && p->N >= 1 && split && wn_wgrad_skip_supported(p->D, p->S, p->N * p->D);
  const bool layerk = (p->LPB == 1 || t.deep16) && wn_wgrad_layer_supported(p->R, p->D, p->KS) && p->Dp == p->R && split;
  const bool pairk = !layerk && p->LPB == 1 && p->KS == 2 && p->R == p->D && p->Dp == p->D && split &&
                     wn_wgrad_pair_kind(p->R, 2 * p->D) == 1 && wn_wgrad_pair_kind(p->D, p->R) == 2;
  t.wg = layerk ? (p->LPB > 1 ? WG_LAYER_INNER : WG_LAYER) : pairk ? WG_TR_PAIRS : (p->LPB > 1 && !t.deep16) ? WG_GENERIC_FP32 : WG_GENERIC;
  const bool m128 = t.fold && p->fold_F0 == 128 && p->Dp == p->D && p->S > 0;
  t.mfused = pairk && p->D == 128 && m128;
  t.mtr = (layerk && m128) ? (p->D == 64 ? 7 : (p->D == 32 ? 8 : 0)) : 0;
  if (t.fold && p->N >= 2 && p->c.use_residual && (p->c.cond_inputs == 0 || p->frag_condB >= 0) && p->Dp == p->D &&
      (wn_bwd_pair_supported(p->R, p->D, p->KS, p->fold_F0) || wn_bwd_s128_supported(p->R, p->D, p->KS, p->fold_F0)))
    t.bwd = p->R == 128 ? BWD_S128 : BWD_PAIR;
  return t;
}

TrainPaths train_paths(const wn_plan* p, const wn_exec& e, const WsLayout& L, int64_t rows) {
  TrainPaths t = train_paths(p);
  t.drop = e.drop_rate > 0.f;
  t.head_split = L.hsplits > 0;
  t.in_split = L.isplits > 0;
  t.rows32 = rows * 2 * p->D * 4 < ((int64_t)1 << 32);
  return t;
}

static bool gen_head_layers_ok(const wn_plan* p, size_t first, size_t end) {
  for (size_t i = first; i < end; ++i) {
    const ConvInfo& c = p->finals[i];
    if (!(c.frag16 >= 0 && c.cout % 32 == 0 && c.cout >= 64 && c.cout <= 256 && c.cin % 16 == 0 && c.cin <= 256)) return false;
  }
  return true;
}

GenPaths gen_paths(const wn_plan* p, int B, int length, int cu_count, bool relay_area, bool deterministic, const WnSampleCtl& ctl) {
  GenPaths g;
  const bool split = wn_debug_get(1) != 1;
  const int RF = wn_plan_receptive_field(p);
  const size_t nf = p->finals.size();
  const bool fits32 = (int64_t)(RF + 1) * B * std::max(p->R, p->D) < (1LL << 31) && (int64_t)RF + length < (1LL << 31) &&
                      (int64_t)p->N * B * p->D < (1LL << 31);
  const bool chain64 = p->fused16_ok && p->LPB == 1 && split && fits32 && wn_gen_blocks_supported(p->R, p->D, p->KS) &&
                       p->N <= wn_gen_chain_max_blocks();
  const bool chain128 = !chain64 && p->LPB == 1 && p->Dp == p->D && wn_gen_block128_supported(p->R, p->D, p->KS) &&
                        !p->blocks.empty() && p->blocks[0].f16nat >= 0 && p->blocks[0].conv1.frag16 >= 0 && split && fits32;
  const bool relay = chain128 && relay_area && wn_debug_get(2) == 0 && (int64_t)((B + 31) / 32) * p->N <= cu_count;
  g.chain = chain64 ? GEN_CHAIN64 : relay ? GEN_RELAY128 : chain128 ? GEN_CHAIN128 : GEN_BLOCKS;
  g.inconv_in_chain = chain64 || (chain128 && p->KS == 2);
  g.fold = fold_ok(p);
  g.skipw = g.fold ? p->fold_F0 : p->Sh;
  g.skip_img = g.fold ? p->frag16_foldF : p->frag16_skipF;
  g.first_final = g.fold ? 1 : 0;
  g.hc0 = (g.fold && p->c.use_skip) ? g.skipw : p->Hin;
  const bool skip_in_chain = (chain64 && p->c.use_skip && g.skip_img >= 0 && wn_gen_skip_fusable(g.skipw)) ||
                             (chain128 && g.fold && p->c.use_skip && g.skipw == 128 && g.skip_img >= 0);
  g.skip = skip_in_chain ? GEN_SKIP_IN_CHAIN : p->c.use_skip ? GEN_SKIP_LAUNCH : GEN_SKIP_NONE;
  const size_t ff = (size_t)g.first_final;
  const bool hc_ok = g.hc0 % 16 == 0 && g.hc0 <= 256;
  const bool head_fused = chain64 && nf > ff && (int)(nf - ff) <= WN_GEN_HEAD_MAX && hc_ok && gen_head_layers_ok(p, ff, nf);
  bool head_mix = !head_fused && split && p->c.head != WN_HEAD_CATEGORICAL && p->c.num_mixtures > 0 && nf >= ff + 2 &&
                  (int)(nf - ff - 1) <= WN_GEN_HEAD_MAX && hc_ok && fits32 && gen_head_layers_ok(p, ff, nf - 1);
  if (head_mix) {
    const ConvInfo& cl = p->finals.back();
    head_mix = cl.cout == 3 * p->c.num_mixtures && cl.cout <= 32 && cl.cin % 64 == 0 && cl.cin <= 256 && cl.fragF >= 0;
  }
  g.head = head_fused ? GEN_HEAD_FUSED : head_mix ? GEN_HEAD_MIX : GEN_HEAD_LAYERS;
  g.pre_in_head = head_fused;
  const bool cat = p->c.head == WN_HEAD_CATEGORICAL;
  g.head_tail = head_fused && cat && p->Cout <= 256 && B <= 8 && (deterministic || !(ctl.top_p > 0.f));
  g.sampler = (g.head_tail || head_mix) ? GEN_SAMPLE_IN_HEAD : deterministic ? GEN_SAMPLE_DET
              : (!cat || wn_sample_from_logits_supported(p->Cout)) ? GEN_SAMPLE_RAND : GEN_SAMPLE_ROWS;
  return g;
}

FwdPaths fwd_paths(const wn_plan* p, const wn_exec& e, int B, int T, bool training, bool prep, bool rings, FwdLoss loss) {
  FwdPaths f;
  const bool split = wn_debug_get(1) != 1;
  const int64_t rows = (int64_t)B * T;
  if (p->c.cond_inputs > 0) {
    f.cond = cond_small(p) ? FWD_COND_SMALL : FWD_COND_ROWS;
    f.cond_batched = p->frag_condF >= 0;
  }
  f.inconv_elem = p->R % 4 == 0 && split;
  f.zfill = p->Dp != p->D;
  f.fold = fold_ok(p);
  f.prep = (prep && f.fold && p->c.use_skip && wn_debug_get(9) == 0) ? FWD_PREP_SIDE
           : (prep && (f.fold || p->c.use_skip)) ? FWD_PREP_INLINE : FWD_PREP_NONE;
  f.drop = training && e.drop_rate > 0.f;
  f.deep16 = training && !rings && deep16(p);
  const size_t nf = p->finals.size();
  if (f.fold) {
    const ConvInfo& c0 = p->finals[0];
    f.skip = (p->Dp == p->D && Planes::takes(false, c0.cout, p->D, p->N, p->Dp, c0.cout, rows, {p->Dp, c0.cout}))
             ? FWD_SKIP_FOLD_PLANES : FWD_SKIP_FOLD_ROWS;
    f.first_final = 1;
  } else if (p->c.use_skip) {
    f.skip = FWD_SKIP_SUM;
  }
  f.hc0 = f.fold ? p->finals[0].cout : p->Hin;
  f.nhead = (int)nf;
  int hc = f.hc0;
  for (size_t i = (size_t)f.first_final; i < nf; ++i) {
    const ConvInfo& c = p->finals[i];
    const bool planes = Planes::takes(false, c.cout, hc, 1, hc, c.cout, rows, {hc});
    if (i + 1 == nf && loss != FWD_LOSS_NONE && loss_fusable(p, rows) && planes) f.head[i] = FWD_HEAD_EPILOGUE;
    else if (c.frag16 >= 0 && split && planes) f.head[i] = FWD_HEAD_PLANES;
    else f.head[i] = FWD_HEAD_ROWS;
    hc = c.cout;
  }
  return f;
}

WsLayout make_layout(const wn_plan* p, int B, int T, bool training) {
  WsLayout L;
  Carver cv;
  const int64_t rows = (int64_t)B * T;
  L.frag = cv.take(p->frag_floats);
  L.bias_sum = cv.take(p->Hin);
  L.vfold = cv.take(p->fold_F0 > 0 ? (int64_t)(p->N * p->D + 1) * p->fold_F0 : 0);
  L.bfold = cv.take(p->fold_F0 > 0 ? p->fold_F0 : 0);
  L.wsall = cv.take(p->fold_F0 > 0 ? (int64_t)(p->N * p->D + 1) * p->S : 0);
  L.mslab = L.mtot = L.ytmp = 0;
  const int nH = training ? p->N + 1 : 2;
  const int hc = std::max(p->R, p->D);
  for (int i = 0; i < nH; ++i) L.H.push_back(cv.take(rows * hc));
  L.P.resize(p->N);
  if (p->LPB > 1) {
    const int nP = training ? p->N : 1;
    std::vector<std::vector<int64_t>> tmp(nP);
    for (int b = 0; b < nP; ++b)
      for (int i = 0; i < p->LPB - 1; ++i) tmp[b].push_back(cv.take(rows * p->D));
    for (int b = 0; b < p->N; ++b) L.P[b] = tmp[training ? b : 0];
  }
  L.Z = cv.take(rows * p->N * p->Dp);
  if (training) for (int b = 0; b < p->N; ++b) L.AG.push_back(cv.take(rows * p->D));
  L.U = cv.take(rows * 2 * p->D);
  L.O = cv.take(rows * p->R);
  L.skipsum = cv.take(rows * p->Hin);
  int maxC = std::max(p->Hin, p->Cout);
  for (size_t i = 0; i + 1 < p->finals.size(); ++i) {
    L.HA.push_back(cv.take(rows * p->finals[i].cout));
    maxC = std::max(maxC, p->finals[i].cout);
  }
  L.logits = cv.take(rows * p->Cout);
  L.probs = cv.take(rows * p->Cout);
  L.target = cv.take(rows);
  L.loss_rows = cv.take(rows);
  L.yt = cv.take(rows);
  L.sum_scratch = cv.take(2048 + 64);
  L.n_absmax = AbsmaxSlots{(int)p->finals.size(), p->N, p->LPB}.count();
  L.absmax = cv.take(L.n_absmax);
  L.fwd_absmax = cv.take(1);
  if (p->c.cond_inputs > 0) {
    for (size_t j = 0; j < p->mapping.size(); ++j) L.M.push_back(cv.take((int64_t)B * p->mapping[j].cout));
    L.cb = cv.take((int64_t)p->N * B * 2 * p->D);
    L.dcb = cv.take((int64_t)B * 2 * p->D);
    L.cbt = cv.take((int64_t)B * p->N * 2 * p->D);
    int mw = std::max(p->Cc, p->c.cond_inputs);
    for (auto& m : p->mapping) mw = std::max(mw, m.cout);
    L.g_m0 = cv.take((int64_t)B * mw);
    L.g_m1 = cv.take((int64_t)B * mw);
  } else {
    L.cb = L.dcb = L.g_m0 = L.g_m1 = L.cbt = 0;
  }
  L.gxd = 0;
  if (training && wnp::ex(p).drop_rate > 0.f) {
    for (int b = 0; b < p->N; ++b) L.XD.push_back(cv.take(rows * p->R));
    L.gxd = cv.take(rows * p->R);
  }
  if (training) {
    L.g_skipsum = cv.take(rows * p->Hin);
    int64_t need = 0;
    need = std::max(need, slab_need(B, T, 1, p->R));
    for (const BlockInfo& b : p->blocks) {
      for (const ConvInfo& c : b.dil) need = std::max(need, slab_need(B, T, c.cin, c.cout));
      need = std::max(need, slab_need(B, T, p->D, p->R));
      if (b.has_skip) need = std::max(need, slab_need(B, T, p->D, p->S));
    }
    for (const ConvInfo& c : p->finals) need = std::max(need, slab_need(B, T, c.cin, c.cout));
    if (p->fold_F0 > 0) need = std::max(need, slab_need(1, p->N * p->D + 1, p->S, p->fold_F0));
    for (const ConvInfo& c : p->mapping) need = std::max(need, slab_need(1, B, c.cin, c.cout));
    if (p->c.cond_inputs > 0) {
      need = std::max(need, slab_need(1, B, p->Cc, 2 * p->D));
      need = std::max(need, wn_colsum_scratch_floats(B, 2 * p->D));
    }
    L.slab_floats = need;
    L.slab = cv.take(need);
    L.bslab = 0; L.bsplits = 0;
    L.hslab = 0; L.hsplits = 0; L.head_base = 0; L.head_span = 0;
    L.islab = 0; L.isplits = 0;
    for (int b = 0; b < p->N; ++b) L.GU.push_back(cv.take(rows * 2 * p->D));
    L.GP.assign(p->N, std::vector<int64_t>());
    for (int b = 0; b < p->N; ++b)
      for (int i = 0; i + 1 < p->LPB; ++i) L.GP[b].push_back(cv.take(rows * p->D));
    for (int b = 0; b <= p->N; ++b) L.GH.push_back(cv.take(rows * p->R));
    if (p->S == 0) for (int b = 0; b < p->N; ++b) L.GO.push_back(cv.take(rows * p->R));
    for (size_t i = 0; i < p->finals.size(); ++i) L.GF.push_back(cv.take(rows * p->finals[i].cout));
    const int nj = count_jobs(p);
    int sp = (int)((5000 + (int64_t)nj * B - 1) / ((int64_t)nj * B));
    const int maxsp = std::max(1, (T + 255) / 256);
    sp = std::max(1, std::min(sp, maxsp));
    L.bsplits = sp;
    L.bslab = cv.take((int64_t)B * sp * p->nparams);
    if (p->fold_F0 > 0) {
      const int64_t pm = (int64_t)p->N * p->D * p->fold_F0 + p->fold_F0;
      L.mslab = cv.take((int64_t)B * sp * pm);
      L.mtot = cv.take(pm);
      L.ytmp = cv.take((int64_t)(p->N * p->D + 1) * p->S);
    }
    if (wn_inconv_wgrad_supported(p->R, p->KS) && p->tensors[p->causal.kernel_t].off == 0 &&
        p->tensors[p->causal.bias_t].off == (int64_t)p->KS * p->R) {
      L.isplits = std::max(1, std::min((512 + B - 1) / B, std::max(1, T / 64)));
      L.islab = cv.take((int64_t)B * L.isplits * (p->KS + 1) * p->R);
    }
    if (!p->finals.empty()) {
      int njh = 0;
      for (const ConvInfo& c : p->finals) njh += jobs_for(c.cin, c.cout);
      int hs = (int)((1536 + (int64_t)njh * B - 1) / ((int64_t)njh * B));
      if (head_pairs_ok(p)) hs = std::max(1, (256 + B - 1) / B);
      hs = std::max(sp, std::min(hs, maxsp));
      if (hs > sp) {
        L.head_base = p->tensors[p->finals.front().kernel_t].off;
        const TensorInfo& last = p->tensors[p->finals.back().bias_t];
        L.head_span = last.off + last.len - L.head_base;
        L.hsplits = hs;
        L.hslab = cv.take((int64_t)B * hs * L.head_span);
      }
    }
  } else {
    L.bslab = 0; L.bsplits = 0;
    L.hslab = 0; L.hsplits = 0; L.head_base = 0; L.head_span = 0;
    L.islab = 0; L.isplits = 0;
    L.g_skipsum = L.slab = 0;
    L.slab_floats = 0;
  }
  L.total = cv.pos;
  return L;
}

}

using namespace wnp;

extern "C" wn_plan* wn_plan_create(const wn_config* cfg) {
  if (!cfg) { wn_set_error("plan_create: null config"); return nullptr; }
  const wn_config& c = *cfg;
  if (c.kernel_size < 2) { wn_set_error("Kernel size must be at least 2."); return nullptr; }
  if (c.layers_per_block < 1 || c.layers_per_block > 16) { wn_set_error("Layers per block must be in 1..16."); return nullptr; }
  if (c.blocks < 1) { wn_set_error("Blocks must be at least 1."); return nullptr; }
  if (c.channels < 1) { wn_set_error("channels must be positive"); return nullptr; }
  {
    const double lg = log((double)c.dilation_bound) / log((double)c.kernel_size);
    int64_t pw = 1; int mp = 0;
    while (pw < c.dilation_bound) { pw *= c.kernel_size; ++mp; }
    if (pw != c.dilation_bound || mp < 1) { wn_set_error("dilation bound must be power of kernel_size."); return nullptr; }
    (void)lg;
  }
  if (c.head == WN_HEAD_CATEGORICAL && c.num_mixtures != 0) { wn_set_error("Categorical sampling cannot be used with mixtures."); return nullptr; }
  if (c.head != WN_HEAD_CATEGORICAL && c.num_mixtures < 1) { wn_set_error("Number of mixtures must be at least 1 for mixture heads."); return nullptr; }
  if (c.n_final < 0 || c.n_final > WN_MAX_FINAL || c.n_mapping < 0 || c.n_mapping > WN_MAX_MAPPING) { wn_set_error("too many final / mapping layers"); return nullptr; }
  if (c.bits < 1 || c.bits > 16) { wn_set_error("bits must be in 1..16"); return nullptr; }
  if (c.kernel_size > 3) { wn_set_error("kernel_size > 3 is not supported by the gfx950 kernels"); return nullptr; }

  wn_plan* p = new wn_plan();
  p->c = c;
  p->KS = c.kernel_size; p->R = c.channels; p->D = c.dilation_channels > 0 ? c.dilation_channels : c.channels;
  p->S = c.skip_channels; p->N = c.blocks; p->LPB = c.layers_per_block;
  p->Cout = c.num_mixtures > 0 ? 3 * c.num_mixtures : (1 << c.bits);
  p->Sh = p->S > 0 ? p->S : p->R;
  p->Hin = c.use_skip ? p->Sh : p->R;
  p->Dp = ceil8(p->D);
  {
    int mp = 0; int64_t pw = 1;
    while (pw < c.dilation_bound) { pw *= c.kernel_size; ++mp; }
    for (int i = 0; i < p->LPB * p->N; ++i) {
      int d = 1;
      for (int e = 0; e < i % mp; ++e) d *= c.kernel_size;
      p->dilations.push_back(d);
    }
  }
  p->Cc = 0;
  if (c.cond_inputs > 0) p->Cc = c.n_mapping > 0 ? c.mapping_channels[c.n_mapping - 1] : c.cond_inputs;

  p->causal = add_conv(p, p->KS, 1, p->R, 1);
  for (int b = 0; b < p->N; ++b) {
    BlockInfo bi;
    int cin = p->R;
    for (int i = 0; i < p->LPB; ++i) {
      const int cout = (i == p->LPB - 1) ? 2 * p->D : p->D;
      bi.dil.push_back(add_conv(p, p->KS, cin, cout, p->dilations[b * p->LPB + i]));
      cin = cout;
    }
    bi.conv1 = add_conv(p, 1, p->D, p->R, 1);
    bi.has_skip = p->S > 0;
    if (bi.has_skip) bi.conv_skip = add_conv(p, 1, p->D, p->S, 1);
    bi.has_cond = c.cond_inputs > 0;
    if (bi.has_cond) bi.conv_cond = add_conv(p, 1, p->Cc, 2 * p->D, 1);
    p->blocks.push_back(bi);
  }
  {
    int cprev = p->Hin;
    for (int i = 0; i < c.n_final; ++i) { p->finals.push_back(add_conv(p, 1, cprev, c.final_channels[i], 1)); cprev = c.final_channels[i]; }
    p->finals.push_back(add_conv(p, 1, cprev, p->Cout, 1));
  }
  if (c.cond_inputs > 0) {
    int cin = c.cond_inputs;
    for (int j = 0; j < c.n_mapping; ++j) { p->mapping.push_back(add_dense(p, cin, c.mapping_channels[j])); cin = c.mapping_channels[j]; }
  }
  for (const TensorInfo& t : p->tensors) {
    WnTensorDesc d; d.off = t.off; d.len = t.len;
    p->tdesc.push_back(d);
    if (t.is_kernel) p->kdesc.push_back(d);
  }

  add_images(p, p->causal, true, false);
  for (BlockInfo& bi : p->blocks) {
    for (ConvInfo& cv : bi.dil) add_images(p, cv, true, true);
    add_images(p, bi.conv1, true, true);
    if (bi.has_skip) add_images(p, bi.conv_skip, false, true);
    if (bi.has_cond) add_images(p, bi.conv_cond, true, true);
  }
  for (ConvInfo& cv : p->finals) add_images(p, cv, true, true);
  for (ConvInfo& cv : p->mapping) add_images(p, cv, true, true);
  {
    bool all_cond = p->c.cond_inputs > 0 && (2 * p->D) % 32 == 0 && p->N > 0;
    for (const BlockInfo& bi : p->blocks) all_cond = all_cond && bi.has_cond;
    if (all_cond) {
      const int D2 = 2 * p->D;
      p->frag_condF = p->frag_floats;
      for (int b = 0; b < p->N; ++b) {
        WnPrepDesc d;
        memset(&d, 0, sizeof(d));
        d.src_off = p->tensors[p->blocks[b].conv_cond.kernel_t].off;
        d.dst_off = p->frag_condF;
        d.I = D2; d.KK = p->Cc; d.ld = D2; d.transpose = 1;
        d.q_off = 0; d.j_off = b * (D2 / 32); d.JT = p->N * (D2 / 32);
        p->prep.push_back(d);
      }
      p->frag_floats += (int64_t)wn_frag_floats(p->N * D2, p->Cc);
      p->frag_condB = p->frag_floats;
      for (int b = 0; b < p->N; ++b) {
        WnPrepDesc d;
        memset(&d, 0, sizeof(d));
        d.src_off = p->tensors[p->blocks[b].conv_cond.kernel_t].off;
        d.dst_off = p->frag_condB;
        d.I = p->Cc; d.KK = D2; d.ld = D2; d.transpose = 0;
        d.q_off = b * (D2 / 8); d.j_off = 0; d.JT = ceil32(p->Cc);
        p->prep.push_back(d);
      }
      p->frag_floats += (int64_t)wn_frag_floats(p->Cc, p->N * D2);
    }
  }
  p->frag_skipF = p->frag_floats;
  for (int b = 0; b < p->N; ++b) {
    const ConvInfo& src = p->blocks[b].has_skip ? p->blocks[b].conv_skip : p->blocks[b].conv1;
    WnPrepDesc d;
    memset(&d, 0, sizeof(d));
    d.src_off = p->tensors[src.kernel_t].off;
    d.dst_off = p->frag_skipF;
    d.I = p->Sh; d.KK = p->D; d.ld = p->Sh; d.transpose = 1;
    d.q_off = b * (p->Dp / 8); d.j_off = 0; d.JT = ceil32(p->Sh);
    p->prep.push_back(d);
  }
  p->frag_floats += (int64_t)wn_frag_floats(p->Sh, p->N * p->Dp);
  p->fused_ok = wn_layer_fwd_supported(p->R, p->D, p->KS) != 0;
  p->fused16_ok = p->fused_ok && wn_layer_fwd_f16_supported(p->R, p->D, p->KS) != 0;
  if (p->fused16_ok)
    for (BlockInfo& bi : p->blocks) {
      add_image16(p, bi.dil.back());
      add_image16(p, bi.conv1);
    }
  if (!p->fused16_ok && p->LPB == 1 && p->D % 64 == 0 && m16(p->R) && m32(p->R))
    for (BlockInfo& bi : p->blocks) {
      const ConvInfo& c = bi.dil.back();
      bi.f16gate = new_image16(p, 2 * p->D, p->KS * p->R);
      for (int t = 0; t < p->KS; ++t)
        for (int q = 0; q < p->D / 64; ++q)
          for (int half = 0; half < 2; ++half)
            add_piece16(p, bi.f16gate, 64, p->tensors[c.kernel_t].off + (int64_t)t * p->R * 2 * p->D + half * p->D + 64 * q,
                        p->R, 2 * p->D, 1, t * (p->R / 16), 4 * q + 2 * half, 2 * p->D / 32);
// ... 129 lines not shown
  wnp::ex(p).prof_on = max_launches > 0;
  for (int i = 0; i < 2 * max_launches; ++i) {
    hipEvent_t e;
    WN_HIP_CHECK(hipEventCreate(&e));
    wnp::ex(p).prof_ev.push_back(e);
  }
  return WN_OK;
}
extern "C" int wn_stack_prof_enable(wn_plan* p, int32_t max_passes) {
  if (!p) return WN_E_INVALID;
  for (hipEvent_t e : wnp::ex(p).stack_ev) (void)hipEventDestroy(e);
  for (hipEvent_t e : wnp::ex(p).foldprep_ev) (void)hipEventDestroy(e);
  wnp::ex(p).stack_ev.clear();
  wnp::ex(p).foldprep_ev.clear();
  wnp::ex(p).stack_used = 0;
  wnp::ex(p).foldprep_used = 0;
  for (int i = 0; i < 2 * max_passes; ++i) {
    hipEvent_t e;
    WN_HIP_CHECK(hipEventCreate(&e));
    wnp::ex(p).stack_ev.push_back(e);
    WN_HIP_CHECK(hipEventCreate(&e));
    wnp::ex(p).foldprep_ev.push_back(e);
  }
  return WN_OK;
}
extern "C" int wn_stack_prof_read_foldprep(wn_plan* p, int32_t* passes, float* avg_ms) {
  if (!p || !passes || !avg_ms) return WN_E_INVALID;
  double tot = 0.0;
  int n = 0;
  for (int i = 0; i + 1 < wnp::ex(p).foldprep_used; i += 2) {
    float ms = 0.f;
    WN_HIP_CHECK(hipEventElapsedTime(&ms, wnp::ex(p).foldprep_ev[i], wnp::ex(p).foldprep_ev[i + 1]));
    tot += ms; ++n;
  }
  *passes = n;
  *avg_ms = n ? (float)(tot / n) : 0.f;
  wnp::ex(p).foldprep_used = 0;
  return WN_OK;
}
extern "C" int wn_stack_prof_read(wn_plan* p, int32_t* passes, float* avg_ms) {
  if (!p || !passes || !avg_ms) return WN_E_INVALID;
  double tot = 0.0;
  int n = 0;
  for (int i = 0; i + 1 < wnp::ex(p).stack_used; i += 2) {
    float ms = 0.f;
    WN_HIP_CHECK(hipEventElapsedTime(&ms, wnp::ex(p).stack_ev[i], wnp::ex(p).stack_ev[i + 1]));
    tot += ms; ++n;
  }
  *passes = n;
  *avg_ms = n ? (float)(tot / n) : 0.f;
  wnp::ex(p).stack_used = 0;
  return WN_OK;
}
extern "C" int wn_phase_enable(wn_plan* p, int32_t on) {
  if (!p) return WN_E_INVALID;
  if (on && !wnp::ex(p).phase_ev[0])
    for (hipEvent_t& e : wnp::ex(p).phase_ev) WN_HIP_CHECK(hipEventCreate(&e));
  wnp::ex(p).phase_on = on != 0;
  return WN_OK;
}
extern "C" int wn_phase_read(wn_plan* p, float* ms4) {
  if (!p || !ms4 || !wnp::ex(p).phase_ev[0]) return WN_E_INVALID;
  for (int i = 0; i < 4; ++i) WN_HIP_CHECK(hipEventElapsedTime(ms4 + i, wnp::ex(p).phase_ev[i], wnp::ex(p).phase_ev[i + 1]));
  return WN_OK;
}
extern "C" int wn_prof_read(wn_plan* p, int32_t* launches, float* avg_ms) {
  if (!p || !launches || !avg_ms) return WN_E_INVALID;
  double tot = 0.0;
  int n = 0;
  for (int i = 0; i + 1 < wnp::ex(p).prof_used; i += 2) {
    float ms = 0.f;
    WN_HIP_CHECK(hipEventElapsedTime(&ms, wnp::ex(p).prof_ev[i], wnp::ex(p).prof_ev[i + 1]));
    tot += ms; n += wnp::ex(p).prof_cnt[i / 2];
  }
  *launches = n;
  *avg_ms = n ? (float)(tot / n) : 0.f;
  wnp::ex(p).prof_used = 0;
  return WN_OK;
}

extern "C" int64_t wn_plan_param_count(const wn_plan* p) { return p ? p->nparams : 0; }
extern "C" int32_t wn_plan_num_tensors(const wn_plan* p) { return p ? (int32_t)p->tensors.size() : 0; }
extern "C" int wn_plan_tensor_info(const wn_plan* p, int32_t idx, int64_t* offset, int64_t* len,
                                   int32_t* ndim, int64_t* shape3, int32_t* is_kernel) {
  if (!p || idx < 0 || idx >= (int32_t)p->tensors.size()) { wn_set_error("tensor_info: bad index"); return WN_E_INVALID; }
  const TensorInfo& t = p->tensors[idx];
  if (offset) *offset = t.off;
  if (len) *len = t.len;
  if (ndim) *ndim = t.ndim;
  if (shape3) { shape3[0] = t.shape[0]; shape3[1] = t.shape[1]; shape3[2] = t.shape[2]; }
  if (is_kernel) *is_kernel = t.is_kernel;
  return WN_OK;
}
extern "C" int32_t wn_plan_receptive_field(const wn_plan* p) {
  int64_t s = 0;
  for (int d : p->dilations) s += d;
  return (int32_t)(1 + s * (p->KS - 1) + 1);
}
extern "C" int32_t wn_plan_out_channels(const wn_plan* p) { return p->Cout; }
extern "C" int32_t wn_plan_dilation(const wn_plan* p, int32_t i) {
  return (i >= 0 && i < (int32_t)p->dilations.size()) ? p->dilations[i] : -1;
}
extern "C" int64_t wn_plan_workspace_floats(const wn_plan* p, int32_t B, int32_t T, int32_t training) {
  if (!p || B < 1 || T < 1) return 0;
  return make_layout(p, B, T, training != 0).total;
}

extern "C" int wn_plan_describe(const wn_plan* p, char* buf, int32_t len) {
  if (!p || !buf || len < 1) return WN_E_INVALID;
  const bool exact = wn_debug_get(1) == 1;
  const char* fwd;
  if (p->LPB > 1 && deep16(p)) fwd = "per conv of the stack, split precision in training passes (rows contractions + the fused block kernel for the gated conv)";
  else if (p->LPB > 1) fwd = "composed per conv (rows GEMM fp32 + fused fp32 kernel for the gated conv where the shape allows)";
  else if (!exact && p->fused16_ok) fwd = "fused split-precision block kernel, weights LDS-resident (wn_layer_fwd_f16_kernel)";
  else if (!exact && !p->blocks.empty() && p->blocks[0].f16nat >= 0)
    fwd = "fused split-precision block kernel, weights streamed through an LDS ring (wn_layer_fwd_s128_kernel)";
  else if (!exact && !p->blocks.empty() && p->blocks[0].f16gate >= 0)
    fwd = "two split-precision contractions per block (gated conv + gate, 1x1 + residual)";
  else if (p->fused_ok) fwd = "fused exact-fp32 block kernel (wn_layer_fwd_kernel)";
  else fwd = "composed: rows GEMM -> gate kernel -> rows GEMM";
  const TrainPaths tp = train_paths(p);
  const bool fold = tp.fold;
  const char* bwd;
  if (p->LPB > 1) bwd = "per-block composed backward, one rows contraction per conv of the stack (layers_per_block > 1)";
  else if (tp.bwd == BWD_PAIR) bwd = "two products per launch (wn_bwd_pair_kernel: g_x(b+1) and g_u(b))";
  else if (tp.bwd == BWD_S128)
    bwd = "two products per launch, weights streamed through an LDS ring (wn_bwd_s128_kernel: g_x(b+1) and g_u(b))";
  else if (!exact) bwd = "two split-precision rows contractions per block (g_u with the gate derivative, g_x)";
  else bwd = "two exact-fp32 rows contractions per block";
  const char* wg = "";
  switch (tp.wg) {
    case WG_LAYER_INNER: wg = "one workgroup per (conv, utterance, time range): the last conv + 1x1 of a block as for depth 1, inner convs through the kernel's INNER form (wn_wgrad_layer_kernel)"; break;
    case WG_LAYER: wg = "one workgroup per (block, utterance, time range) for dW_d, db_d, dW_r, db_r (wn_wgrad_layer_kernel)"; break;
    case WG_TR_PAIRS:
      wg = tp.mfused ? "two jobs per block on transposed LDS reads: both taps of dW_d from one read of du; dW_r together with the "
                       "folded skip path's M = Z^T dL/da from one read of z (wn_wgrad_tr_kernel)"
                     : "two jobs per block on transposed LDS reads: both taps of dW_d from one read of du; dW_r (wn_wgrad_tr_kernel)";
      break;
    case WG_GENERIC_FP32: wg = "generic batched job table in exact fp32, every conv of every stack in one launch (wn_wgrad_batched_kernel)"; break;
    case WG_GENERIC:
      wg = p->LPB > 1 ? "generic batched job table, split precision, every conv of every stack in one launch (wn_wgrad_batched_kernel)"
                      : "generic batched job table (wn_wgrad_batched_kernel)";
      break;
  }
  snprintf(buf, (size_t)len,
           "math: %s | block forward: %s | skip path: %s | backward data: %s | block weight gradients: %s",
           exact ? "exact fp32 MFMA" : "fp16 hi|lo split, 3 products, fp32 accumulate", fwd,
           fold ? "folded into the head's first conv (V = W_s W_f0, training / inference / generation)"
                : (p->c.use_skip ? "one contraction over all blocks' gated activations, then the head" : "none (use_skip False)"),
           bwd, wg);
  return WN_OK;
}

extern "C" int wn_debug_fwd_paths(const wn_plan* p, int32_t B, int32_t T, int32_t training, int32_t loss, char* buf, int32_t len) {
  if (!p || !buf || len < 1 || B < 1 || T < 1 || loss < 0 || loss > 2) return WN_E_INVALID;
  wn_exec none;
  const FwdPaths f = fwd_paths(p, none, B, T, training != 0, true, false, (FwdLoss)loss);
  static const char* const cond[] = {"none", "small", "rows"};
  static const char* const prep[] = {"none", "inline", "side"};
  static const char* const skip[] = {"none", "folded/planes", "folded/rows", "sum"};
  static const char* const head[] = {"rows", "planes", "epilogue"};
  std::string h;
  for (int i = f.first_final; i < f.nhead; ++i) h += std::string(h.empty() ? "" : ",") + head[f.head[i]];
  snprintf(buf, (size_t)len, "cond=%s conv_cond=%s inconv=%s zfill=%d fold=%d prep=%s drop=%d deep16=%d skip=%s first_final=%d hc0=%d head=%s",
           cond[f.cond], f.cond == FWD_COND_NONE ? "none" : f.cond_batched ? "batched" : "per_block",
           f.inconv_elem ? "elementwise" : "rows", (int)f.zfill, (int)f.fold, prep[f.prep], (int)f.drop, (int)f.deep16, skip[f.skip],
           f.first_final, f.hc0, h.c_str());
  return WN_OK;
}

extern "C" int wn_debug_ws_region(const wn_plan* p, int32_t B, int32_t T, int32_t what, int32_t idx, int64_t* off,
                                  int64_t* len) {
  if (!p || !off || !len || B < 1 || T < 1) return WN_E_INVALID;
  const WsLayout L = make_layout(p, B, T, true);
  const int64_t rows = (int64_t)B * T;
  auto in = [&](size_t n) { return idx >= 0 && (size_t)idx < n; };
  *off = -1; *len = 0;
  switch (what) {
    case 0: if (in(L.H.size())) { *off = L.H[idx]; *len = rows * p->R; } break;
    case 1: if (in((size_t)p->N)) { *off = L.Z + (int64_t)idx * rows * p->Dp; *len = rows * p->Dp; } break;
    case 2: if (in(L.AG.size())) { *off = L.AG[idx]; *len = rows * p->D; } break;
    case 3: if (!fold_ok(p)) { *off = L.skipsum; *len = rows * p->Hin; } break;
    case 4: if (in(L.HA.size())) { *off = L.HA[idx]; *len = rows * p->finals[idx].cout; } break;
    case 5: *off = L.logits; *len = rows * p->Cout; break;
    case 6: if (in(L.GF.size())) { *off = L.GF[idx]; *len = rows * p->finals[idx].cout; } break;
    case 7: if (!fold_ok(p)) { *off = L.g_skipsum; *len = rows * p->Hin; } break;
    case 8: if (in(L.GU.size())) { *off = L.GU[idx]; *len = rows * 2 * p->D; } break;
    case 9: if (in(L.GH.size())) { *off = L.GH[idx]; *len = rows * p->R; } break;
    case 10: *off = L.absmax; *len = L.n_absmax; break;
    case 11: {
      const int inner = p->LPB - 1;
      if (inner > 0 && idx >= 0 && idx < p->N * inner && (size_t)(idx / inner) < L.P.size() &&
          (size_t)(idx % inner) < L.P[idx / inner].size()) { *off = L.P[idx / inner][idx % inner]; *len = rows * p->D; }
      break;
    }
    case 12: *off = L.loss_rows; *len = rows; break;
    case 13: {
      const int inner = p->LPB - 1;
      if (inner > 0 && idx >= 0 && idx < p->N * inner && (size_t)(idx / inner) < L.GP.size() &&
          (size_t)(idx % inner) < L.GP[idx / inner].size()) { *off = L.GP[idx / inner][idx % inner]; *len = rows * p->D; }
      break;
    }
    case 14: if (in(L.XD.size())) { *off = L.XD[idx]; *len = rows * p->R; } break;
    default: break;
  }
  if (*off < 0) { wn_set_error("ws_region: no such region (%d, %d)", what, idx); return WN_E_INVALID; }
  return WN_OK;
}

extern "C" int wn_debug_eval_region(const wn_plan* p, int32_t B, int32_t T, int32_t what, int64_t* off, int64_t* len) {
  if (!p || !off || !len || B < 1 || T < 1) return WN_E_INVALID;
  const WsLayout L = make_layout(p, B, T, false);
  const int64_t rows = (int64_t)B * T;
  switch (what) {
    case 5: *off = L.logits; *len = rows * p->Cout; return WN_OK;
    case 12: *off = L.loss_rows; *len = rows; return WN_OK;
    default: break;
  }
  *off = -1; *len = 0;
  wn_set_error("eval_region: no such region (%d)", what);
  return WN_E_INVALID;
}

extern "C" int64_t wn_plan_range_slot(const wn_plan* p, int32_t B, int32_t T, int32_t training) {
  if (!p || B < 1 || T < 1) return -1;
  return make_layout(p, B, T, training != 0).fwd_absmax;
}
extern "C" float wn_range_limit(void) { return WN_RANGE_LIMIT; }
```

### wavenets_amd/csrc/wn_plan_internal.h

```cpp
#pragma once
#include <math.h>
#include <stdlib.h>
#include <string.h>

#include <algorithm>
#include <mutex>
#include <vector>

#include "../../include/wn_hip.h"
#include "wn_kernels.h"

namespace wnp {

inline int64_t align64(int64_t v) { return (v + 63) & ~(int64_t)63; }
inline int ceil32(int v) { return (v + 31) / 32; }
inline int ceil8(int v) { return (v + 7) / 8 * 8; }

struct TensorInfo {
  int64_t off, len;
  int ndim;
  int64_t shape[3];
  int is_kernel;
};

struct ConvInfo {
  int kernel_t = -1, bias_t = -1;
  int taps = 1, cin = 0, cout = 0, dil = 1;
  int64_t fragF = -1;
  int64_t fragB = -1;
  int64_t fragF_stride = 0, fragB_stride = 0;
  int64_t frag16 = -1;
  int64_t frag16B = -1;
};

struct BlockInfo {
  std::vector<ConvInfo> dil;
  ConvInfo conv1, conv_skip, conv_cond;
  bool has_skip = false, has_cond = false;
  int64_t g16u = -1;
  int64_t f16gate = -1;
  int64_t f16nat = -1;
  int64_t g16uf = -1;
  int64_t d16F[16], d16B[16];
  BlockInfo() { for (int i = 0; i < 16; ++i) d16F[i] = d16B[i] = -1; }
};

struct AbsmaxSlots {
  int nf, N, LPB;
  int gf(int i) const { return i; }
  int gskip() const { return nf; }
  int gu(int b) const { return nf + 1 + b; }
  int gh(int b) const { return nf + 1 + N + b; }
  int gp(int b, int i) const { return nf + 1 + N + (N + 1) + b * (LPB - 1) + i; }
  int count() const { return gp(N, 0); }
};

enum WgFamily { WG_LAYER, WG_LAYER_INNER, WG_TR_PAIRS, WG_GENERIC, WG_GENERIC_FP32 };
enum BwdFamily { BWD_BLOCKS, BWD_PAIR, BWD_S128 };
struct TrainPaths {
  WgFamily wg = WG_GENERIC;
  BwdFamily bwd = BWD_BLOCKS;
  int mtr = 0;
  bool mfused = false;
  bool skipk = false, fold = false, deep16 = false, head_pairs = false;
  bool drop = false, head_split = false, in_split = false, rows32 = true;
  bool layerk() const { return wg == WG_LAYER || wg == WG_LAYER_INNER; }
  bool pairk() const { return wg == WG_TR_PAIRS; }
  bool headpairs() const { return head_pairs && head_split; }
  bool bwd_pairs() const { return bwd != BWD_BLOCKS && !drop && (bwd != BWD_S128 || rows32); }
  bool operator==(const TrainPaths& o) const {
    return wg == o.wg && bwd == o.bwd && mtr == o.mtr && mfused == o.mfused && skipk == o.skipk && fold == o.fold &&
           deep16 == o.deep16 && head_pairs == o.head_pairs && drop == o.drop && head_split == o.head_split &&
           in_split == o.in_split && rows32 == o.rows32;
  }
};

enum GenChain { GEN_BLOCKS, GEN_CHAIN64, GEN_CHAIN128, GEN_RELAY128 };
enum GenSkip { GEN_SKIP_NONE, GEN_SKIP_IN_CHAIN, GEN_SKIP_LAUNCH };
enum GenHead { GEN_HEAD_LAYERS, GEN_HEAD_FUSED, GEN_HEAD_MIX };
enum GenSampler { GEN_SAMPLE_IN_HEAD, GEN_SAMPLE_DET, GEN_SAMPLE_RAND, GEN_SAMPLE_ROWS };
struct GenPaths {
  GenChain chain = GEN_BLOCKS;
  bool inconv_in_chain = false;
  GenSkip skip = GEN_SKIP_NONE;
  bool fold = false;
  int skipw = 0, first_final = 0, hc0 = 0;
  int64_t skip_img = -1;
  GenHead head = GEN_HEAD_LAYERS;
  bool pre_in_head = false;
  bool head_tail = false;
  GenSampler sampler = GEN_SAMPLE_DET;
  bool chain128() const { return chain == GEN_CHAIN128 || chain == GEN_RELAY128; }
  bool table() const { return chain != GEN_BLOCKS; }
  bool operator==(const GenPaths& o) const {
    return chain == o.chain && inconv_in_chain == o.inconv_in_chain && skip == o.skip && fold == o.fold && skipw == o.skipw &&
           first_final == o.first_final && hc0 == o.hc0 && skip_img == o.skip_img && head == o.head &&
           pre_in_head == o.pre_in_head && head_tail == o.head_tail && sampler == o.sampler;
  }
};

enum FwdCond { FWD_COND_NONE, FWD_COND_SMALL, FWD_COND_ROWS };
enum FwdPrep { FWD_PREP_NONE, FWD_PREP_INLINE, FWD_PREP_SIDE };
enum FwdSkip { FWD_SKIP_NONE, FWD_SKIP_FOLD_PLANES, FWD_SKIP_FOLD_ROWS, FWD_SKIP_SUM };
enum FwdHead : uint8_t { FWD_HEAD_ROWS, FWD_HEAD_PLANES, FWD_HEAD_EPILOGUE };
enum FwdLoss { FWD_LOSS_NONE, FWD_LOSS_TRAIN, FWD_LOSS_EVAL };
struct FwdPaths {
  FwdCond cond = FWD_COND_NONE;
  bool cond_batched = false;
  bool inconv_elem = false;
  bool zfill = false;
  bool fold = false;
  FwdPrep prep = FWD_PREP_NONE;
  bool drop = false;
  bool deep16 = false;
  FwdSkip skip = FWD_SKIP_NONE;
  int first_final = 0, hc0 = 0;
  int nhead = 0;
  FwdHead head[WN_MAX_FINAL + 1] = {};
  bool operator==(const FwdPaths& o) const {
    return cond == o.cond && cond_batched == o.cond_batched && inconv_elem == o.inconv_elem && zfill == o.zfill && fold == o.fold &&
           prep == o.prep && drop == o.drop && deep16 == o.deep16 && skip == o.skip && first_final == o.first_final &&
           hc0 == o.hc0 && nhead == o.nhead && std::equal(head, head + WN_MAX_FINAL + 1, o.head);
  }
};

template <class T> struct DevTable {
  T* d = nullptr;
  void release() { if (d) (void)hipFree(d); d = nullptr; }
  int upload(const std::vector<T>& v, size_t min_count = 0) {
    release();
    const size_t n = std::max(v.size(), min_count);
    if (n == 0) return WN_OK;
    WN_HIP_CHECK(hipMalloc((void**)&d, n * sizeof(T)));
    if (!v.empty()) WN_HIP_CHECK(hipMemcpy(d, v.data(), v.size() * sizeof(T), hipMemcpyHostToDevice));
    return WN_OK;
  }
};

struct WgSpan {
  enum Op : uint8_t { INCONV, JOBS, PAIRS, TR, LAYERS, SKIP } op;
  enum Slab : uint8_t { BATCH, HEAD, MFOLD } slab;
  int kind;
  int first, count;
};

struct WgSchedule {
  bool valid = false;
  int B = 0, T = 0, bsplits = 0;
  TrainPaths paths;
  DevTable<WnWgJob> jobs;
  DevTable<WnWgLayer> layers, inner;
  DevTable<WnWgPair> pairs;
  DevTable<WnTensorDesc> cov;
  std::vector<WnTensorDesc> h_cov;
  std::vector<WgSpan> spans;
  int n_side = 0;
  bool overlap = false;
  int cov_head = 0;
  void release() { valid = false; jobs.release(); layers.release(); inner.release(); pairs.release(); cov.release(); }
};

struct GenTable {
  bool valid = false;
  int B = 0;
  bool chain128 = false;
  DevTable<WnGenBlock> blocks;
  WnGenBlock blk0[3]{};
  int64_t bias_stride = 0;
  void release() { valid = false; blocks.release(); }
};

struct WnAdmitSeg { int64_t src, dst; int32_t nslots, width; };

struct AdmitTable {
  bool valid = false;
  int k = 0, B = 0;
  std::vector<int32_t> slots;
  DevTable<WnAdmitSeg> segs;
  DevTable<int32_t> slots_d;
  void release() { valid = false; segs.release(); slots_d.release(); }
};

}

struct wn_exec {
  const struct wn_plan* plan = nullptr;
  float drop_rate = 0.f;
  uint64_t drop_seed = 0, drop_step = 0;
  float* step_sample = nullptr; int step_sample_det = 0; uint64_t step_sample_seed = 0, step_sample_off = 0;
  const float* row_weights = nullptr; int64_t row_weights_n = 0;
  wnp::WgSchedule wg;
  wnp::GenTable gen;
  wnp::AdmitTable admit;
  hipStream_t side = nullptr;
  hipEvent_t ev_fork = nullptr, ev_join = nullptr;
  hipEvent_t ev_ffork = nullptr, ev_fjoin = nullptr;
  int train_phases = 3;
  std::vector<hipEvent_t> prof_ev;
  std::vector<int> prof_cnt;
  hipEvent_t phase_ev[5] = {nullptr, nullptr, nullptr, nullptr, nullptr};
  bool phase_on = false;
  int prof_used = 0;
  bool prof_on = false;
  std::vector<hipEvent_t> stack_ev;
  std::vector<hipEvent_t> foldprep_ev;
  int foldprep_used = 0;
  int stack_used = 0;
};

struct wn_plan {
  wn_config c;
  int KS, R, D, S, N, LPB, Cout, Sh, Hin, Cc, Dp;
  std::vector<int> dilations;
  std::vector<wnp::TensorInfo> tensors;
  int64_t nparams = 0;
  wnp::ConvInfo causal;
  std::vector<wnp::BlockInfo> blocks;
  std::vector<wnp::ConvInfo> finals, mapping;
  int64_t frag_skipF = -1;
  int64_t frag_condF = -1, frag_condB = -1;
  int64_t frag16_skipF = -1;
  int64_t frag_floats = 0;
  int fold_F0 = 0;
  int64_t frag16_foldF = -1;
  std::vector<WnPrepDesc> prep2;
  WnPrepDesc* d_prep2 = nullptr;
  WnTensorDesc* d_cov_fold = nullptr;
  WnTensorDesc h_cov_fold = {0, 0};
  std::vector<WnPrepDesc> prep;
  std::vector<WnTensorDesc> tdesc, kdesc;
  WnPrepDesc* d_prep = nullptr;
  WnTensorDesc* d_tdesc = nullptr;
  WnTensorDesc* d_kdesc = nullptr;
  bool fused_ok = false, fused16_ok = false;
  bool deep16_ok = false;
  std::mutex tables_mu;
  bool tables_ready = false;
  struct wn_exec* own = nullptr;
};

namespace wnp {
wn_exec& ex(const wn_plan* p);
void exec_release(wn_exec* e);


struct Carver {
  int64_t pos = 0;
  int64_t take(int64_t n) { int64_t o = pos; pos = align64(pos + (n > 0 ? n : 0)); return o; }
};

struct WsLayout {
  int64_t frag, bias_sum;
  std::vector<int64_t> H;
  std::vector<std::vector<int64_t>> P;
  int64_t Z;
  std::vector<int64_t> AG;
  std::vector<std::vector<int64_t>> GP;
  int64_t U;
  int64_t O;
  int64_t skipsum;
  std::vector<int64_t> HA;
  int64_t logits, probs;
  int64_t target, loss_rows, yt;
  int64_t g_skipsum;
  int64_t slab, slab_floats;
  std::vector<int64_t> GU, GH, GO, GF;
  int64_t bslab; int bsplits;
  int64_t hslab; int hsplits; int64_t head_base, head_span;
  int64_t islab; int isplits;
  int64_t vfold, bfold, wsall, mslab, mtot, ytmp;
  std::vector<int64_t> XD;
  int64_t gxd;
  int64_t absmax; int n_absmax;
  int64_t fwd_absmax;
  int64_t sum_scratch;
  std::vector<int64_t> M;
  int64_t cb;
  int64_t dcb, g_m0, g_m1;
  int64_t cbt;
  int64_t total;
};

inline bool al16(const void* p) { return (((uintptr_t)p) & 15) == 0; }

struct Gemm {
  WnGemmArgs a;
  const float* w16_ = nullptr;
  const float* am0_ = nullptr;
  const float* am1_ = nullptr;
  float* amo_ = nullptr;
  Gemm& w16(const float* img) { w16_ = img; return *this; }
  Gemm& absmax(const float* in0, const float* in1, float* out) { am0_ = in0; am1_ = in1; amo_ = out; return *this; }
  Gemm& absmax_fwd(float* out) { amo_ = out; a.absmax_any = out ? 1 : 0; return *this; }
  Gemm(int B, int T, int N, int JTtot) {
    memset(&a, 0, sizeof(a));
    a.B = B; a.T = T; a.N = N; a.JTtot = JTtot; a.act = WN_ACT_LINEAR; a.epi = WN_EPI_PLAIN;
  }
  Gemm& seg(const float* x, int ldx, int K, int shift, const float* frag) {
    WnSeg& s = a.seg[a.nseg++];
    s.x = x; s.ldx = ldx; s.K = K; s.shift = shift; s.frag = frag;
    s.vec = (ldx % 4 == 0 && K % 4 == 0 && al16(x)) ? 1 : 0;
    s.plane_k = 0; s.plane_stride = 0;
    return *this;
  }
  Gemm& seg_planes(const float* x, int plane_k, int64_t plane_stride, int K, const float* frag) {
    seg(x, plane_k, K, 0, frag);
    WnSeg& s = a.seg[a.nseg - 1];
    s.plane_k = plane_k; s.plane_stride = plane_stride;
    s.vec = (plane_k % 4 == 0 && plane_stride % 4 == 0 && al16(x)) ? 1 : 0;
    return *this;
  }
  Gemm& bias(const float* b) { a.bias = b; return *this; }
  Gemm& rowbias(const float* b, int ld) { a.rowbias = b; a.ld_rowbias = ld; return *this; }
  Gemm& addc(const float* c, int ld) { a.addc = c; a.ld_addc = ld; return *this; }
  Gemm& act(int act) { a.act = act; return *this; }
  Gemm& dact(const float* ysaved, int ld, int act) { a.epi = WN_EPI_DACT; a.aux = ysaved; a.ld_aux = ld; a.act = act; return *this; }
  Gemm& gate_bwd(const float* g, int ldg, const float* z, int ldz) {
    a.epi = WN_EPI_GATE_BWD; a.aux = g; a.ld_aux = ldg; a.aux2 = z; a.ld_aux2 = ldz;
    return *this;
  }
  Gemm& gate_fwd(float* sig, int ld) { a.epi = WN_EPI_GATE_FWD; a.y2 = sig; a.ld_y2 = ld; return *this; }
  int run(float* y, int ldy, hipStream_t s) {
    a.y = y; a.ldy = ldy;
    bool v = (a.N % 4 == 0) && (ldy % 4 == 0) && al16(y);
    if (a.bias) v = v && al16(a.bias);
    if (a.addc) v = v && (a.ld_addc % 4 == 0) && al16(a.addc);
    if (a.aux) v = v && (a.ld_aux % 4 == 0) && al16(a.aux);
    if (a.aux2) v = v && (a.ld_aux2 % 4 == 0) && al16(a.aux2);
    if (a.y2) v = v && (a.ld_y2 % 4 == 0) && al16(a.y2);
    a.vec_out = v ? 1 : 0;
    if (w16_ && wn_debug_get(1) != 1 && wn_gemm_rows16_ok(a)) return wn_launch_gemm_rows16(a, w16_, am0_, am1_, amo_, s);
    if (a.epi == WN_EPI_GATE_FWD) { wn_set_error("gate-forward contraction needs the split-precision kernel (alignment / shape)"); return WN_E_UNSUPPORTED; }
    for (int i = 0; i < a.nseg; ++i)
      if (!a.seg[i].frag) { wn_set_error("contraction without an fp32 weight image needs the split-precision kernel"); return WN_E_UNSUPPORTED; }
    return wn_launch_gemm_rows(a, s);
  }
};

struct LossFuse {
  const int32_t* target; float gscale; float* loss_rows; float* g_logits; float* absmax_out;
  float* sample_out; float inv_lv; uint64_t seed, offset;
  const float* row_weight;
  bool done;
  bool eval;
};

struct Planes {
  WnGemmPlanesArgs a;
  static bool takes(bool taps, int N, int plane_k, int nplanes, int ld, int ldy, int64_t rows, std::initializer_list<int> widths) {
    if (!(taps ? wn_gemm_taps16s_supported(N, plane_k, nplanes, ld, ldy) : wn_gemm_planes16s_supported(N, plane_k, nplanes, ld, ldy)))
      return false;
    for (int w : widths)
      if (!((int64_t)rows * w * 4 < ((int64_t)1 << 32))) return false;
    return true;
  }
  Planes(int B, int T, int N) {
    memset(&a, 0, sizeof(a));
    a.B = B; a.T = T; a.N = N;
  }
  Planes& operand(const float* z, int ld, int plane_k, int nplanes = 1, int64_t plane_stride = 0) {
    a.z = z; a.ld = ld; a.plane_k = plane_k; a.nplanes = nplanes; a.plane_stride = plane_stride;
    return *this;
  }
  Planes& taps(int n, int step) {
    a.nplanes = n; a.nshift = n;
    for (int t = 0; t < n; ++t) a.shift[t] = (n - 1 - t) * step;
    return *this;
  }
  Planes& w16(const float* img) { a.w16 = img; return *this; }
  Planes& bias(const float* b) { a.bias = b; return *this; }
  Planes& act(int act) { a.act = act; return *this; }
  Planes& absmax_fwd(float* out) { a.absmax_out = out; return *this; }
  Planes& bwd(const float* am_in, float* am_out, const float* aux = nullptr, int ld_aux = 0) {
    a.bwd = 1; a.absmax_in = am_in; a.absmax_out = am_out; a.aux = aux; a.ld_aux = ld_aux;
    return *this;
  }
  Planes& loss(const LossFuse& lf) {
    a.absmax_out = lf.absmax_out;
    a.cat_loss = lf.eval ? 2 : 1; a.target = lf.target; a.gscale = lf.gscale; a.loss_rows = lf.loss_rows;
    a.sample_out = lf.sample_out; a.inv_lv = lf.inv_lv; a.seed = lf.seed; a.offset = lf.offset;
    a.row_weight = lf.row_weight;
    return *this;
  }
  int run(float* y, int ldy, hipStream_t s) {
    a.y = y; a.ldy = ldy;
    return wn_launch_gemm_planes16s(a, s);
  }
};

struct BlockPtrs {
  int B, T, KS, R, D, S, Cin, depth, act, residual;
  int dil[16];
  const float* Wd[16]; const float* bd[16];
  const float* br; const float* bs; const float* bc;
  const float* Fd[16]; const float* Bd[16]; int64_t Fd_stride[16], Bd_stride[16];
  const float* Fr; const float* Br_;
  const float* Fs; const float* Bs;
  const float* Fc; const float* Bc;
  int Cc;
  const float* cond;
  const float* cb;
  bool fused;
  const float* F16d; const float* F16r;
  const float* G16u; const float* G16x;
  const float* G16uf;
  const float* F16g;
  const float* F16n;
  const float* F16i[16]; const float* G16i[16];
  int JTi[16], JTb[16], JTu;
};

struct BlockBufs {
  const float* x;
  float* P[16];
  float* U;
  float* AG;
  float* Z; int ldz;
  float* O;
  float* x_out;
  const float* xt[3];
  const float* res;
  bool pre_done;
  float* fwd_absmax;
};

struct BlockGrads {
  const float* g_xout;
  const float* g_skip;
  float* g_o_tmp;
  float* g_u;
  float* g_p;
  float* g_pi[16];
  float* g_x;
  float* g_cond;
  float* dWd[16]; float* dbd[16];
  float* dWr; float* dbr; float* dWs; float* dbs; float* dWc; float* dbc;
  float* dcb;
  float* slab;
  bool defer;
  const float* am_gxout; const float* am_gskip;
  float* am_gu; float* am_gx;
  float* am_gp[16];
  const float* g_fold; int fold_F0; const float* am_gfold;
  float drop_rate; uint32_t drop_key; float* g_xd;
};

struct GenRings {
  float* xin;
  std::vector<float*> h;
  std::vector<int> nslots;
  std::vector<std::vector<float*>> hp;
  std::vector<std::vector<int>> nslots_p;
  int64_t t0 = 0;
};

inline bool m16(int v) { return v > 0 && v % 16 == 0; }
inline bool m32(int v) { return v >= 64 && v % 32 == 0; }

int ensure_device_tables(wn_plan* p);
WsLayout make_layout(const wn_plan* p, int B, int T, bool training);
bool deep16(const wn_plan* p);
bool cond_small(const wn_plan* p);
bool fold_ok(const wn_plan* p);
bool head_pairs_ok(const wn_plan* p);
TrainPaths train_paths(const wn_plan* p);
TrainPaths train_paths(const wn_plan* p, const wn_exec& e, const WsLayout& L, int64_t rows);
GenPaths gen_paths(const wn_plan* p, int B, int length, int cu_count, bool relay_area, bool deterministic, const WnSampleCtl& ctl);
FwdPaths fwd_paths(const wn_plan* p, const wn_exec& e, int B, int T, bool training, bool prep, bool rings, FwdLoss loss);
int64_t slab_need(int B, int T, int K, int N);
int wgrad(const float* x, int ldx, int K, int shift, const float* g, int ldg, int N, int B, int T,
          float* dW, float* db, float* per_batch, float* slab, hipStream_t s);
int block_forward(const BlockPtrs& k, const BlockBufs& f, hipStream_t s);
int block_backward(const BlockPtrs& k, const BlockBufs& f, const BlockGrads& g, hipStream_t s);
bool loss_fusable(const wn_plan* p, int64_t rows);
BlockPtrs block_ptrs(const wn_plan* p, int b, const float* params, const float* fragbase, int B, int T);
void deep16_ptrs(const wn_plan* p, int b, const float* fragbase, BlockPtrs& k);
int forward_core(wn_plan* p, const float* params, const float* x, bool prep, const float* cond, int B,
                 int T, bool training, float* ws, const WsLayout& L, hipStream_t s, const GenRings* rings = nullptr,
                 LossFuse* lf = nullptr);
int emit_outputs(const wn_plan* p, const float* ws, const WsLayout& L, int64_t rows, float* logits_out, float* out, hipStream_t s);
int shift_split(const float* x_full, int B, int T, float* inputs, float* y_true, hipStream_t s);
int loss_stage(wn_plan* p, int B, int T, int global_batch, bool want_grad, float* ws, const WsLayout& L,
               float* loss_out, float* absmax_out, hipStream_t s, bool fused_done = false, const float* row_weight = nullptr);
int loss_rows_stage(wn_plan* p, int64_t rows, float gscale, float* g_logits, bool want_grad, float* ws, const WsLayout& L,
                    float* absmax_out, hipStream_t s, const float* row_weight);
int row_weights_check(const char* who, const wn_exec& e, int B, int T);

}

int wn_sampling_check(const char* who, const wn_sampling* sp, int head, int classes, WnSampleCtl* ctl);
```

### wavenets_amd/csrc/wn_train.hip

```cpp
#include "wn_plan_internal.h"

namespace {
using namespace wnp;

void add_jobs(std::vector<WnWgJob>& jobs, int64_t x_off, int ldx, int K, int shift, int64_t g_off, int ldg, int N,
              int64_t out_off, int64_t bias_off, int64_t gmax_off) {
  const int tk = wn_wgrad_tile_k(), tn = wn_wgrad_tile_n();
  for (int k0 = 0; k0 < K; k0 += tk)
    for (int n0 = 0; n0 < N; n0 += tn) {
      WnWgJob j;
      memset(&j, 0, sizeof(j));
      j.x_off = x_off; j.g_off = g_off; j.out_off = out_off; j.bias_off = (k0 == 0) ? bias_off : -1;
      j.gmax_off = gmax_off;
      j.ldx = ldx; j.ldg = ldg; j.K = K; j.N = N; j.shift = shift; j.k0 = k0; j.n0 = n0;
      jobs.push_back(j);
    }
}

int ensure_schedule(const wn_plan* p, wn_exec& e, const WsLayout& L, int B, int T, const TrainPaths& tp) {
  WgSchedule& g = e.wg;
  if (g.valid && g.B == B && g.T == T && g.bsplits == L.bsplits && g.paths == tp) return WN_OK;
  const bool layerk = tp.layerk(), pairk = tp.pairk(), fold = tp.fold;
  std::vector<WnWgLayer> wgl, wgli;
  std::vector<WnWgPair> pairs[3];
// ... 133 lines not shown
    cover(c.kernel_t); cover(c.bias_t);
  }
  std::vector<WnWgPair> all;
  int pfirst[3], hfirst[6] = {0, 0, 0, 0, 0, 0};
  for (int kd = 0; kd <= 2; ++kd) { pfirst[kd] = (int)all.size(); all.insert(all.end(), pairs[kd].begin(), pairs[kd].end()); }
  for (int kd = 1; kd <= 5; ++kd) { hfirst[kd] = (int)all.size(); all.insert(all.end(), hpairs[kd].begin(), hpairs[kd].end()); }
  std::vector<WgSpan> spans;
  auto span = [&](WgSpan::Op op, WgSpan::Slab slab, int kind, int first, size_t count) {
    if (count > 0) spans.push_back(WgSpan{op, slab, kind, first, (int)count});
  };
  const int njobs = (int)jobs.size();
  const bool head_own = tp.head_split && (head_first < njobs || tp.headpairs());
  span(WgSpan::INCONV, WgSpan::BATCH, 0, 0, tp.in_split);
  span(WgSpan::JOBS, WgSpan::BATCH, tp.wg == WG_GENERIC_FP32, 0, head_own ? head_first : njobs);
  if (head_own) span(WgSpan::JOBS, WgSpan::HEAD, 0, head_first, njobs - head_first);
  for (int kd = 1; kd <= 5; ++kd) {
    const int trk = kd == 1 ? 3 : (kd == 3 ? 4 : (kd == 5 ? 5 : (kd == 2 ? 2 : 0)));
    if (trk != 0 && tp.pairk()) span(WgSpan::TR, WgSpan::HEAD, trk, hfirst[kd], hpairs[kd].size());
    else span(WgSpan::PAIRS, WgSpan::HEAD, kd, hfirst[kd], hpairs[kd].size());
  }
  const int n_side = (int)spans.size();
  span(WgSpan::TR, WgSpan::BATCH, 1, pfirst[1], pairs[1].size());
  span(WgSpan::TR, WgSpan::BATCH, tp.mfused ? 6 : 2, pfirst[2], pairs[2].size());
  span(WgSpan::LAYERS, WgSpan::BATCH, tp.mtr == 7 ? 2 : 0, 0, wgl.size());
  span(WgSpan::LAYERS, WgSpan::BATCH, 1, 0, wgli.size());
  if (tp.mtr != 0) span(WgSpan::TR, WgSpan::MFOLD, tp.mtr, pfirst[0], pairs[0].size());
  else if (tp.fold) span(WgSpan::SKIP, WgSpan::MFOLD, 0, 0, !tp.mfused);
  else span(WgSpan::SKIP, WgSpan::BATCH, 0, 0, tp.skipk);
  g.valid = false;
  int rc = g.jobs.upload(jobs, 1);
  if (!rc) rc = g.cov.upload(cov);
  if (!rc) rc = g.layers.upload(wgl);
  if (!rc) rc = g.inner.upload(wgli);
  if (!rc) rc = g.pairs.upload(all);
  if (rc) return rc;
  g.h_cov.swap(cov); g.spans.swap(spans);
  g.n_side = n_side; g.overlap = layerk || pairk; g.cov_head = head_own ? cov_head : (int)g.h_cov.size();
  g.B = B; g.T = T; g.bsplits = L.bsplits; g.paths = tp;
  g.valid = true;
  return WN_OK;
}

struct TrainCall {
  wn_exec& e;
  wn_plan* p; const float* params; const float* x_full; const float* cond;
  int B, T, global_batch, n_replicas;
  float* grads; float* loss_out; float* pred_out; float* ws; hipStream_t s;
  WsLayout L;
  int64_t rows;
  float* inputs;
  const float* fragbase; float* slab;
  float* am; AbsmaxSlots slot;
  int nf; float* am_gskip;
  const float* mlast = nullptr;
  TrainPaths tp;
  bool cond_batched = false;
  float* g_x = nullptr; float* g_cond = nullptr;
  int64_t pm = 0;
  float* am_GF(int i) const { return am + slot.gf(i); }
  float* am_GU(int b) const { return am + slot.gu(b); }
  float* am_GH(int b) const { return am + slot.gh(b); }
  float* am_GP(int b, int i) const { return am + slot.gp(b, i); }
  struct Strided { int64_t off, stride; };
  Strided strided(int t0, int t1) const { return {p->tensors[t0].off, p->N > 1 ? p->tensors[t1].off - p->tensors[t0].off : 0}; }
  Strided skip_w{0, 0}, skip_b{0, 0};

  void bind(wn_plan* p_, const float* params_, const float* cond_, int B_, int T_, float* grads_, float* workspace, hipStream_t s_) {
    p = p_; params = params_; x_full = nullptr; cond = cond_; B = B_; T = T_; global_batch = B_; n_replicas = 1;
    grads = grads_; loss_out = nullptr; pred_out = nullptr; ws = workspace; s = s_;
    L = make_layout(p, B, T, true);
    rows = (int64_t)B * T;
    inputs = workspace + L.probs;
    am = workspace + L.absmax;
    nf = (int)p->finals.size();
    slot = AbsmaxSlots{nf, p->N, p->LPB};
    am_gskip = am + slot.gskip();
  }

  int forward_and_loss() {
    int rc;
    { const int rcs = shift_split(x_full, B, T, inputs, ws + L.yt, s); if (rcs) return rcs; }
    if (e.phase_on) (void)hipEventRecord(e.phase_ev[0], s);
    WN_HIP_CHECK(hipMemsetAsync(am, 0, L.n_absmax * sizeof(float), s));
    LossFuse lf;
    memset(&lf, 0, sizeof(lf));
    const bool fuse = !pred_out && loss_fusable(p, rows);
    if (fuse) {
      rc = wn_launch_quantize(ws + L.yt, reinterpret_cast<int32_t*>(ws + L.target), rows, p->c.bits, s);
      if (rc) return rc;
      lf.target = reinterpret_cast<const int32_t*>(ws + L.target);
      lf.gscale = 1.0f / (float)global_batch;
      lf.loss_rows = ws + L.loss_rows; lf.g_logits = ws + L.GF.back(); lf.absmax_out = am_GF(nf - 1);
      if (e.step_sample && !e.step_sample_det) {
        lf.sample_out = e.step_sample; lf.inv_lv = 1.0f / (float)(1 << (p->c.bits - 1));
        lf.seed = e.step_sample_seed; lf.offset = e.step_sample_off;
      }
      lf.row_weight = e.row_weights;
    }
    rc = forward_core(p, params, inputs, true, cond, B, T, true, ws, L, s, nullptr, fuse ? &lf : nullptr);
    if (rc) return rc;
    if (lf.done && lf.sample_out) e.step_sample = nullptr;
    if (e.phase_on) (void)hipEventRecord(e.phase_ev[1], s);
    rc = loss_stage(p, B, T, global_batch, true, ws, L, loss_out, am_GF(nf - 1), s, lf.done, e.row_weights);
    if (rc) return rc;
    rc = emit_outputs(p, ws, L, rows, nullptr, pred_out, s);
    if (rc) return rc;
    if (e.step_sample) {
      float* so = e.step_sample;
      e.step_sample = nullptr;
      if (p->c.head == WN_HEAD_CATEGORICAL) {
        if (e.step_sample_det) {
          wn_set_error("step sample: deterministic categorical draws go through wn_sample_waveform");
          return WN_E_UNSUPPORTED;
        }
        rc = wn_launch_sample_rand_cat_logits(ws + L.logits, rows, p->Cout, p->c.bits, e.step_sample_seed, e.step_sample_off, so, s);
      } else {
        if (e.step_sample_det) rc = wn_launch_sample_det(ws + L.logits, rows, p->Cout, p->c.num_mixtures, p->c.bits, so, s);
        else rc = wn_launch_sample_rand(ws + L.logits, rows, p->Cout, p->c.num_mixtures, p->c.bits, p->c.head, e.step_sample_seed, e.step_sample_off, so, s);
      }
      if (rc) return rc;
    }
    if (p->c.l2_reg_factor > 0.f) {
      float* norms = ws + L.loss_rows;
      rc = wn_launch_sumsq(params, p->d_kdesc, (int)p->kdesc.size(), norms, s);
      if (rc) return rc;
      rc = wn_launch_sum(norms, (int64_t)p->kdesc.size(), p->c.l2_reg_factor / (float)n_replicas, loss_out + 1, ws + L.sum_scratch, s);
      if (rc) return rc;
    } else {
      rc = wn_launch_fill(loss_out + 1, 0.f, 1, s);
      if (rc) return rc;
    }
    rc = wn_launch_guard_flag(ws + L.fwd_absmax, WN_RANGE_LIMIT * (e.drop_rate > 0.f ? 1.f - e.drop_rate : 1.f),
                              wn_debug_get(1) != 1, loss_out + 2, s);
    if (rc) return rc;
    if (e.phase_on) (void)hipEventRecord(e.phase_ev[2], s);
    return WN_OK;
  }

  int cond_block_bwd(const BlockInfo& bi) {
    const ConvInfo& c = bi.conv_cond;
    int r = wgrad(mlast, p->Cc, p->Cc, 0, ws + L.dcb, 2 * p->D, 2 * p->D, 1, B, grads + p->tensors[c.kernel_t].off,
                  grads + p->tensors[c.bias_t].off, nullptr, slab, s);
    if (r) return r;
    return Gemm(1, B, p->Cc, ceil32(p->Cc)).seg(ws + L.dcb, 2 * p->D, 2 * p->D, 0, fragbase + c.fragB)
        .addc(ws + L.g_m0, p->Cc).run(ws + L.g_m0, p->Cc, s);
  }

  int head_backward() {
    int rc;
    float* head_out = p->c.use_skip ? ws + L.g_skipsum : ws + L.GH[p->N];
    for (int i = (int)p->finals.size() - 1; i >= (tp.fold ? 1 : 0); --i) {
      const ConvInfo& c = p->finals[i];
      float* dst = (i == 0) ? head_out : ws + L.GF[i - 1];
      if (c.frag16B >= 0 && wn_debug_get(1) != 1 && Planes::takes(false, c.cin, c.cout, 1, c.cout, c.cin, rows, {c.cout})) {
        rc = Planes(B, T, c.cin).operand(ws + L.GF[i], c.cout, c.cout).w16(fragbase + c.frag16B).act(p->c.activation)
                 .bwd(am_GF(i), i > 0 ? am_GF(i - 1) : (p->c.use_skip ? am_gskip : am_GH(p->N)),
                      i > 0 ? ws + L.HA[i - 1] : nullptr, i > 0 ? c.cin : 0)
                 .run(dst, c.cin, s);
        if (rc) return rc;
        continue;
      }
      Gemm gm(B, T, c.cin, ceil32(c.cin));
      gm.seg(ws + L.GF[i], c.cout, c.cout, 0, fragbase + c.fragB);
      if (i > 0) gm.dact(ws + L.HA[i - 1], c.cin, p->c.activation);
      if (c.frag16B >= 0)
        gm.w16(fragbase + c.frag16B).absmax(am_GF(i), nullptr, i > 0 ? am_GF(i - 1) : (p->c.use_skip ? am_gskip : am_GH(p->N)));
      rc = gm.run(dst, c.cin, s);
      if (rc) return rc;
    }
    return WN_OK;
  }

  int chain_backward() {
    int rc;
    const float* g_skip = (p->c.use_skip && !tp.fold) ? ws + L.g_skipsum : nullptr;
    if (p->c.use_skip) {
      rc = wn_launch_fill(ws + L.GH[p->N], 0.f, rows * p->R, s);
      if (rc) return rc;
    }
    const bool pairk = tp.bwd_pairs();
    for (int b = p->N - 1; b >= 0; --b) {
      BlockPtrs k = block_ptrs(p, b, params, fragbase, B, T);
      deep16_ptrs(p, b, fragbase, k);
      const BlockInfo& bi = p->blocks[b];
      if (pairk && b < p->N - 1) {
        const BlockPtrs k1 = block_ptrs(p, b + 1, params, fragbase, B, T);
        WnBwdPairArgs a;
        memset(&a, 0, sizeof(a));
        a.gu_in = ws + L.GU[b + 1]; a.gx_res = ws + L.GH[b + 2]; a.gf = ws + L.GF[0];
        a.ag = ws + L.AG[b]; a.z = ws + L.Z + (int64_t)b * rows * p->Dp; a.ldz = p->Dp;
        a.gx_out = ws + L.GH[b + 1]; a.gu_out = ws + L.GU[b];
        a.wx16 = k1.G16x; a.wu16 = k.G16uf;
        a.am_gu_in = am_GU(b + 1); a.am_gf = am_GF(0); a.am_gx = am_GH(b + 1); a.am_gu = am_GU(b);
        a.B = B; a.T = T; a.dil = k1.dil[0];
        if (!a.wx16 || !a.wu16) { wn_set_error("bwd_pair: weight images missing"); return WN_E_UNSUPPORTED; }
        rc = tp.bwd == BWD_S128 ? wn_launch_bwd_s128(a, s) : wn_launch_bwd_pair(a, s);
        if (rc) return rc;
        if (b == 0) {
          Gemm gm(B, T, p->R, ceil32(p->R));
          for (int t = 0; t < p->KS; ++t)
            gm.seg(ws + L.GU[0], 2 * p->D, 2 * p->D, -(p->KS - 1 - t) * k.dil[0], k.Bd[0] + t * k.Bd_stride[0]);
          if (p->c.use_residual) gm.addc(ws + L.GH[1], p->R);
          gm.w16(k.G16x).absmax(am_GU(0), nullptr, am_GH(0));
          rc = gm.run(ws + L.GH[0], p->R, s);
          if (rc) return rc;
        }
        continue;
      }
      BlockBufs f;
      memset(&f, 0, sizeof(f));
      f.x = tp.drop ? ws + L.XD[b] : ws + L.H[b];
      for (int i = 0; i + 1 < p->LPB; ++i) f.P[i] = ws + L.P[b][i];
      f.AG = ws + L.AG[b];
      f.Z = ws + L.Z + (int64_t)b * rows * p->Dp; f.ldz = p->Dp;
      BlockGrads bg;
      memset(&bg, 0, sizeof(bg));
      bg.defer = true;
      for (int i = 0; i + 1 < p->LPB; ++i) bg.g_pi[i] = ws + L.GP[b][i];
      if (tp.deep16)
        for (int i = 0; i + 1 < p->LPB; ++i) bg.am_gp[i] = am_GP(b, i);
      if (tp.drop) {
        bg.drop_rate = e.drop_rate; bg.drop_key = wn_dropout_key(e.drop_seed, b, e.drop_step); bg.g_xd = ws + L.gxd;
      }
      bg.g_xout = (p->c.use_skip && b == p->N - 1 && p->S == 0) ? nullptr : ws + L.GH[b + 1];
      bg.g_skip = g_skip;
      bg.g_o_tmp = p->S == 0 ? ws + L.GO[b] : nullptr;
      bg.g_u = ws + L.GU[b];
      bg.g_x = pairk ? nullptr : ws + L.GH[b];
      bg.dcb = (bi.has_cond && !cond_batched) ? ws + L.dcb : nullptr;
      bg.slab = slab;
      bg.am_gxout = bg.g_xout ? am_GH(b + 1) : nullptr;
      bg.am_gskip = g_skip ? am_gskip : nullptr;
      bg.am_gu = am_GU(b); bg.am_gx = am_GH(b);
      if (tp.fold) { bg.g_fold = ws + L.GF[0]; bg.fold_F0 = p->fold_F0; bg.am_gfold = am_GF(0); }
      rc = block_backward(k, f, bg, s);
      if (rc) return rc;
      if (p->S == 0 && bg.g_xout == nullptr && g_skip) {
        WN_HIP_CHECK(hipMemcpyAsync(ws + L.GO[b], g_skip, rows * p->R * sizeof(float), hipMemcpyDeviceToDevice, s));
      }
      if (bi.has_cond && !cond_batched) {
        rc = cond_block_bwd(bi);
        if (rc) return rc;
      }
    }
    return WN_OK;
  }

  int fold_weight_gradients() {
    const int F0 = p->fold_F0;
    int rc = wn_launch_reduce_table(ws + L.mslab, B * L.bsplits, pm, ws + L.mtot, p->d_cov_fold, 1, s, &p->h_cov_fold);
    if (rc) return rc;
    const ConvInfo& c0 = p->finals[0];
    const int nd1 = p->N * p->D + 1;
    const float* wf0 = params + p->tensors[c0.kernel_t].off;
    rc = wn_launch_sgemm_small(ws + L.mtot, F0, 1, wf0, 1, F0, ws + L.ytmp, p->S, nd1, p->S, F0, s);
    if (rc) return rc;
    const int nzk = (nd1 + 127) / 128;
    if ((int64_t)nzk * p->S * F0 <= L.slab_floats) {
      rc = wn_launch_sgemm_small_batched(ws + L.wsall, 1, p->S, (int64_t)128 * p->S, ws + L.mtot, F0, 1, (int64_t)128 * F0, slab, F0,
                                         (int64_t)p->S * F0, p->S, F0, nd1, nzk, nullptr, 0, s, 128);
      if (rc) return rc;
      WnVecSumArgs v;
      v.base = slab; v.off0 = 0; v.stride = (int64_t)p->S * F0; v.count = nzk; v.len = p->S * F0;
      v.out = grads + p->tensors[c0.kernel_t].off;
      rc = wn_launch_vecsum(v, s);
    } else
    rc = wgrad(ws + L.wsall, p->S, p->S, 0, ws + L.mtot, F0, F0, 1, nd1, grads + p->tensors[c0.kernel_t].off, nullptr, nullptr,
               slab, s);
    if (rc) return rc;
    return wn_launch_skip_scatter(ws + L.ytmp, ws + L.mtot + (int64_t)p->N * p->D * F0, skip_w.off, skip_w.stride, skip_b.off,
                                  skip_b.stride, p->tensors[c0.bias_t].off, p->N, p->D, p->S, F0, grads, s);
  }

  int cond_weight_gradients() {
    int rc;
    const int D2 = 2 * p->D;
    const BlockInfo& b0 = p->blocks[0]; const BlockInfo& b1 = p->blocks[p->N > 1 ? 1 : 0];
    const Strided db = strided(b0.dil.back().bias_t, b1.dil.back().bias_t);
    const Strided cw = strided(b0.conv_cond.kernel_t, b1.conv_cond.kernel_t), cbi = strided(b0.conv_cond.bias_t, b1.conv_cond.bias_t);
    rc = wn_launch_cond_gather(ws + L.bslab, p->nparams, L.bsplits, db.off, db.stride, B, p->N, D2, ws + L.cbt, s);
    if (rc) return rc;
    if (cond_small(p) && (int64_t)p->N * B * p->Cc <= L.slab_floats) {
      rc = wn_launch_sgemm_small_batched(ws + L.cbt, p->N * D2, 1, D2, params + cw.off, 1, D2, cw.stride,
                                         slab, p->Cc, (int64_t)B * p->Cc, B, p->Cc, D2, p->N, nullptr, 0, s);
      if (rc) return rc;
      WnVecSumArgs v;
      v.base = slab; v.off0 = 0; v.stride = (int64_t)B * p->Cc; v.count = p->N; v.len = B * p->Cc; v.out = ws + L.g_m0;
      rc = wn_launch_vecsum(v, s);
    } else
    rc = Gemm(1, B, p->Cc, ceil32(p->Cc)).seg(ws + L.cbt, p->N * D2, p->N * D2, 0, fragbase + p->frag_condB).run(ws + L.g_m0, p->Cc, s);
    if (rc) return rc;
    return wn_launch_cond_wgrad(mlast, ws + L.cbt, B, p->Cc, p->N, D2, grads, cw.off, cw.stride, cbi.off, cbi.stride, s);
  }

  int launch(const WgSpan& sp, hipStream_t st) {
    const WgSchedule& g = e.wg;
    float* out = ws + L.bslab; int64_t pitch = p->nparams; int splits = L.bsplits;
    if (sp.slab == WgSpan::HEAD) { out = ws + L.hslab - L.head_base; pitch = L.head_span; splits = L.hsplits; }
    if (sp.slab == WgSpan::MFOLD) { out = ws + L.mslab; pitch = pm; }
    switch (sp.op) {
      case WgSpan::INCONV:
        return wn_launch_inconv_wgrad(inputs, ws + L.GH[0], B, T, p->R, p->KS, L.isplits, ws + L.islab, (int64_t)(p->KS + 1) * p->R,
                                      0, (int64_t)p->KS * p->R, st);
      case WgSpan::JOBS: return wn_launch_wgrad_batched(g.jobs.d + sp.first, sp.count, ws, out, pitch, B, T, splits, st, sp.kind != 0);
      case WgSpan::PAIRS: return wn_launch_wgrad_pairs(sp.kind, g.pairs.d + sp.first, sp.count, ws, out, pitch, B, T, splits, st);
      case WgSpan::TR:
        return wn_launch_wgrad_tr(sp.kind, g.pairs.d + sp.first, sp.count, ws, out, pitch, B, T, splits, st,
                                  sp.kind == 6 ? ws + L.mslab : (sp.kind == 7 ? ws + L.bslab : nullptr),
                                  sp.kind == 6 ? pm : (sp.kind == 7 ? p->nparams : 0));
      case WgSpan::LAYERS: return wn_launch_wgrad_layers(sp.kind == 1 ? g.inner.d : g.layers.d, sp.count, p->R, ws, out, pitch, B, T, splits, st, sp.kind);
      case WgSpan::SKIP:
        if (sp.slab == WgSpan::MFOLD)
          return wn_launch_wgrad_skip(ws + L.Z, p->Dp, ws + L.GF[0], p->fold_F0, rows, p->N * p->D, p->fold_F0, p->D, B * splits, out, pitch,
                                      0, (int64_t)p->D * p->fold_F0, (int64_t)p->N * p->D * p->fold_F0, 0, 1, am_GF(0), st);
        return wn_launch_wgrad_skip(ws + L.Z, p->Dp, ws + L.g_skipsum, p->S, rows, p->N * p->D, p->S, p->D, B * splits, out, pitch,
                                    skip_w.off, skip_w.stride, skip_b.off, skip_b.stride, p->N, am_gskip, st);
    }
    return WN_E_INVALID;
  }

  int weight_gradients() {
    int rc;
    const WgSchedule& g = e.wg;
    if (e.phase_on) (void)hipEventRecord(e.phase_ev[3], s);
    const bool fork = g.overlap && wn_debug_get(9) != 1;
    if (fork && !e.side) {
      WN_HIP_CHECK(hipStreamCreateWithFlags(&e.side, hipStreamNonBlocking));
      WN_HIP_CHECK(hipEventCreateWithFlags(&e.ev_fork, hipEventDisableTiming));
      WN_HIP_CHECK(hipEventCreateWithFlags(&e.ev_join, hipEventDisableTiming));
    }
    struct SideJoin {
      wn_exec& e; hipStream_t s; bool armed;
      ~SideJoin() {
        if (!armed) return;
        if (hipEventRecord(e.ev_join, e.side) != hipSuccess || hipStreamWaitEvent(s, e.ev_join, 0) != hipSuccess)
          (void)hipStreamSynchronize(e.side);
      }
    } side_join{e, s, false};
    if (fork) {
      WN_HIP_CHECK(hipEventRecord(e.ev_fork, s));
      WN_HIP_CHECK(hipStreamWaitEvent(e.side, e.ev_fork, 0));
      side_join.armed = true;
    }
    size_t i = 0;
    for (; i < (size_t)g.n_side; ++i)
      if ((rc = launch(g.spans[i], fork ? e.side : s))) return rc;
    if (fork) WN_HIP_CHECK(hipEventRecord(e.ev_join, e.side));
    for (; i < g.spans.size(); ++i)
      if ((rc = launch(g.spans[i], s))) return rc;
    if (tp.fold && (rc = fold_weight_gradients())) return rc;
    if (fork) { WN_HIP_CHECK(hipStreamWaitEvent(s, e.ev_join, 0)); side_join.armed = false; }
    if (cond_batched && (rc = cond_weight_gradients())) return rc;
    const int cov0 = tp.in_split ? 2 : 0, ncov = (int)g.h_cov.size(), cov1 = g.cov_head;
    rc = wn_launch_reduce_table(ws + L.bslab, B * L.bsplits, p->nparams, grads, g.cov.d + cov0, cov1 - cov0, s, g.h_cov.data() + cov0);
    if (rc) return rc;
    if (tp.in_split && (rc = wn_launch_reduce_table(ws + L.islab, B * L.isplits, (int64_t)(p->KS + 1) * p->R, grads, g.cov.d, 2, s, g.h_cov.data())))
      return rc;
    if (cov1 < ncov && (rc = wn_launch_reduce_table(ws + L.hslab - L.head_base, B * L.hsplits, L.head_span, grads, g.cov.d + cov1, ncov - cov1,
                                                    s, g.h_cov.data() + cov1)))
      return rc;
    if (!p->c.use_skip && p->S > 0) {
      for (const BlockInfo& bi : p->blocks) {
        rc = wn_launch_fill(grads + p->tensors[bi.conv_skip.kernel_t].off, 0.f, p->tensors[bi.conv_skip.kernel_t].len, s);
        if (!rc) rc = wn_launch_fill(grads + p->tensors[bi.conv_skip.bias_t].off, 0.f, p->tensors[bi.conv_skip.bias_t].len, s);
        if (rc) return rc;
      }
    }
    return WN_OK;
  }

  int mapping_backward() {
    int rc;
    if (p->c.cond_inputs > 0) {
      const float* gm_cur = ws + L.g_m0;
      float* gm_other = ws + L.g_m1;
      if (g_cond && p->mapping.empty())
        WN_HIP_CHECK(hipMemcpyAsync(g_cond, gm_cur, (int64_t)B * p->Cc * sizeof(float), hipMemcpyDeviceToDevice, s));
      for (int j = (int)p->mapping.size() - 1; j >= 0; --j) {
        const ConvInfo& c = p->mapping[j];
        const float* yin = (j == 0) ? cond : ws + L.M[j - 1];
        rc = wn_launch_dact_mul(gm_cur, ws + L.M[j], gm_other, (int64_t)B * c.cout, p->c.mapping_activation, s);
        if (rc) return rc;
        if (j == 0 && g_cond) {
          rc = wn_launch_sgemm_small_batched(gm_other, c.cout, 1, 0, params + p->tensors[c.kernel_t].off, 1, c.cout, 0, g_cond, c.cin, 0,
                                             B, c.cin, c.cout, 1, nullptr, 0, s);
          if (rc) return rc;
        }
        if (cond_small(p)) {
          rc = wn_launch_sgemm_small_batched(yin, 1, c.cin, 0, gm_other, c.cout, 1, 0, grads + p->tensors[c.kernel_t].off, c.cout, 0,
                                             c.cin, c.cout, B, 1, nullptr, 0, s);
          if (rc) return rc;
          WnVecSumArgs v;
          v.base = gm_other; v.off0 = 0; v.stride = c.cout; v.count = B; v.len = c.cout; v.out = grads + p->tensors[c.bias_t].off;
          rc = wn_launch_vecsum(v, s);
          if (rc) return rc;
          if (j > 0) {
            float* dst = const_cast<float*>(gm_cur);
            rc = wn_launch_sgemm_small_batched(gm_other, c.cout, 1, 0, params + p->tensors[c.kernel_t].off, 1, c.cout, 0, dst, c.cin, 0,
                                               B, c.cin, c.cout, 1, nullptr, 0, s);
            if (rc) return rc;
          }
          continue;
        }
        rc = wgrad(yin, c.cin, c.cin, 0, gm_other, c.cout, c.cout, 1, B, grads + p->tensors[c.kernel_t].off,
                   grads + p->tensors[c.bias_t].off, nullptr, slab, s);
        if (rc) return rc;
        if (j > 0) {
          float* dst = const_cast<float*>(gm_cur);
          rc = Gemm(1, B, c.cin, ceil32(c.cin)).seg(gm_other, c.cout, c.cout, 0, fragbase + c.fragB).run(dst, c.cin, s);
          if (rc) return rc;
        }
      }
    }
    return WN_OK;
  }

  int backward_from_logits() {
    int rc;
    fragbase = ws + L.frag;
    slab = ws + L.slab;
    if (p->c.cond_inputs > 0) {
      mlast = p->mapping.empty() ? cond : ws + L.M.back();
      rc = wn_launch_fill(ws + L.g_m0, 0.f, (int64_t)B * p->Cc, s);
      if (rc) return rc;
    }
    cond_batched = p->frag_condB >= 0;
    tp = train_paths(p, e, L, rows);
    pm = (int64_t)p->N * p->D * p->fold_F0 + p->fold_F0;
    if (p->blocks[0].has_skip) {
      const BlockInfo& b0 = p->blocks[0]; const BlockInfo& b1 = p->blocks[p->N > 1 ? 1 : 0];
      skip_w = strided(b0.conv_skip.kernel_t, b1.conv_skip.kernel_t); skip_b = strided(b0.conv_skip.bias_t, b1.conv_skip.bias_t);
    }
    rc = ensure_schedule(p, e, L, B, T, tp);
    if (rc) return rc;
    if ((rc = head_backward())) return rc;
    if ((rc = chain_backward())) return rc;
    if ((rc = weight_gradients())) return rc;
    if ((rc = mapping_backward())) return rc;
    if (g_x)
      return wn_launch_inconv_bwd_data(ws + L.GH[0], params + p->tensors[p->causal.kernel_t].off, B, T, p->R, p->KS, g_x, s);
    return WN_OK;
  }

  int backward() {
    int rc = backward_from_logits();
    if (rc) return rc;
    if (p->c.l2_reg_factor > 0.f) {
      rc = wn_launch_axpy_table(grads, params, p->d_kdesc, (int)p->kdesc.size(), 2.0f * p->c.l2_reg_factor / (float)n_replicas, s);
      if (rc) return rc;
    }
    if (e.phase_on) {
      (void)hipEventRecord(e.phase_ev[4], s);
    }

    return WN_OK;
  }
};

}

extern "C" int wn_plan_set_train_phases(wn_plan* p, int32_t phases) {
  if (!p || phases < 1 || phases > 3) { wn_set_error("set_train_phases: 1 (forward + loss), 2 (backward), 3 (both)"); return WN_E_INVALID; }
  wnp::ex(p).train_phases = phases;
  return WN_OK;
}

extern "C" int wn_train_fwd_bwd(wn_plan* p, const float* params, const float* x_full, const float* cond,
                                int32_t B, int32_t T, int32_t global_batch, int32_t n_replicas, float* grads,
                                float* loss_out, float* pred_out, float* workspace, int64_t ws_floats,
                                void* stream) {
  if (!p || !params || !x_full || !workspace || !loss_out || !grads || B < 1 || T < 1) { wn_set_error("train_fwd_bwd: bad arguments"); return WN_E_INVALID; }
  if (wnp::row_weights_check("train_fwd_bwd", wnp::ex(p), B, T)) return WN_E_INVALID;
  TrainCall c{wnp::ex(p)};
  c.bind(p, params, cond, B, T, grads, workspace, (hipStream_t)stream);
  c.x_full = x_full;
  c.global_batch = global_batch > 0 ? global_batch : B;
  c.n_replicas = n_replicas > 0 ? n_replicas : 1;
  c.loss_out = loss_out; c.pred_out = pred_out;
  if (ws_floats < c.L.total) { wn_set_error("train_fwd_bwd: workspace too small (%lld < %lld floats)", (long long)ws_floats, (long long)c.L.total); return WN_E_INVALID; }
  const int phases = c.e.train_phases;
  int rc = WN_OK;
  if (phases & 1) rc = c.forward_and_loss();
  if (!rc && (phases & 2)) rc = c.backward();
  return rc;
}

extern "C" int wn_vjp(wn_plan* p, const float* params, const float* x, const float* cond, int32_t B, int32_t T,
                      const float* g_out, int32_t g_kind, float* grads, float* g_x, float* g_cond,
                      float* workspace, int64_t ws_floats, void* stream) {
  if (!p || !params || !x || !g_out || !grads || !workspace) { wn_set_error("vjp: bad arguments (null plan, params, x, g_out, grads or workspace)"); return WN_E_INVALID; }
  if (B < 1 || T < 1) { wn_set_error("vjp: B and T must be >= 1 (got %d, %d)", (int)B, (int)T); return WN_E_INVALID; }
  if (g_kind != 0 && g_kind != 1) { wn_set_error("vjp: g_kind must be 0 (network output) or 1 (logits) (got %d)", (int)g_kind); return WN_E_INVALID; }
  if (p->c.cond_inputs > 0 && !cond) { wn_set_error("vjp: the plan is conditioned and cond is null"); return WN_E_INVALID; }
  if (p->c.cond_inputs <= 0 && g_cond) { wn_set_error("vjp: g_cond on a plan without conditioning"); return WN_E_INVALID; }
  TrainCall c{wnp::ex(p)};
  c.bind(p, params, cond, B, T, grads, workspace, (hipStream_t)stream);
  c.g_x = g_x; c.g_cond = g_cond;
  if (ws_floats < c.L.total) { wn_set_error("vjp: workspace too small (%lld < %lld floats)", (long long)ws_floats, (long long)c.L.total); return WN_E_INVALID; }
  hipStream_t s = c.s;
  WN_HIP_CHECK(hipMemcpyAsync(c.inputs, x, c.rows * sizeof(float), hipMemcpyDeviceToDevice, s));
  WN_HIP_CHECK(hipMemsetAsync(c.am, 0, c.L.n_absmax * sizeof(float), s));
  const int rc = wn_launch_vjp_seed(workspace + c.L.logits, g_out, c.rows, p->Cout,
                                    g_kind == 0 && p->c.head == WN_HEAD_CATEGORICAL, workspace + c.L.GF.back(), c.am_GF(c.nf - 1), s);
  if (rc) return rc;
  return c.backward_from_logits();
}

extern "C" int wn_adam_step_guarded(wn_plan* p, float* params, const float* grads, float* m, float* v, int64_t step,
                                    float lr, float beta1, float beta2, float eps, float clipnorm, float* scratch,
                                    const float* skip_flag, void* stream) {
  if (!p || !params || !grads || !m || !v || !scratch || step < 1) { wn_set_error("adam_step: bad arguments"); return WN_E_INVALID; }
  hipStream_t s = (hipStream_t)stream;
  int rc = ensure_device_tables(p);
  if (rc) return rc;
  const int n = (int)p->tdesc.size();
  if (clipnorm > 0.f) {
    rc = wn_launch_sumsq(grads, p->d_tdesc, n, scratch, s);
    if (rc) return rc;
  }
  const double alpha = (double)lr * sqrt(1.0 - pow((double)beta2, (double)step)) / (1.0 - pow((double)beta1, (double)step));
  return wn_launch_adam(params, grads, m, v, p->d_tdesc, n, scratch, clipnorm, (float)alpha, beta1, beta2, eps, skip_flag, s);
}

extern "C" int wn_adam_step_ema(wn_plan* p, float* params, const float* grads, float* m, float* v, float* ema, int64_t step,
                                float lr, float beta1, float beta2, float eps, float clipnorm, float ema_momentum,
                                int32_t ema_overwrite, float* scratch, const float* skip_flag, void* stream) {
  if (!p || !params || !grads || !m || !v || !ema || !scratch || step < 1) { wn_set_error("adam_step_ema: bad arguments"); return WN_E_INVALID; }
  if (!std::isfinite(ema_momentum) || ema_momentum < 0.f || ema_momentum > 1.f) {
    wn_set_error("adam_step_ema: ema_momentum must be finite and in [0, 1] (got %g)", (double)ema_momentum);
    return WN_E_INVALID;
  }
  if (ema_overwrite != 0 && ema_overwrite != 1) { wn_set_error("adam_step_ema: ema_overwrite must be 0 or 1 (got %d)", (int)ema_overwrite); return WN_E_INVALID; }
  hipStream_t s = (hipStream_t)stream;
  int rc = ensure_device_tables(p);
  if (rc) return rc;
  const int n = (int)p->tdesc.size();
  if (clipnorm > 0.f) {
    rc = wn_launch_sumsq(grads, p->d_tdesc, n, scratch, s);
    if (rc) return rc;
  }
  const double alpha = (double)lr * sqrt(1.0 - pow((double)beta2, (double)step)) / (1.0 - pow((double)beta1, (double)step));
  return wn_launch_adam_ema(params, grads, m, v, ema, p->d_tdesc, n, scratch, clipnorm, (float)alpha, beta1, beta2, eps,
                            ema_momentum, step == 1 ? 1 : 0, (int)ema_overwrite, skip_flag, s);
}

extern "C" int wn_clip_gradients(wn_plan* p, float* grads, float clipnorm, float* scratch, void* stream) {
  if (!p || !grads || !scratch) { wn_set_error("clip_gradients: bad arguments"); return WN_E_INVALID; }
  if (!(clipnorm > 0.f) || !std::isfinite(clipnorm)) { wn_set_error("clip_gradients: clipnorm must be finite and > 0 (got %g)", (double)clipnorm); return WN_E_INVALID; }
  int rc = ensure_device_tables(p);
  if (rc) return rc;
  return wn_launch_clip(grads, p->d_tdesc, (int)p->tdesc.size(), clipnorm, scratch, (hipStream_t)stream);
}

extern "C" int wn_adam_step(wn_plan* p, float* params, const float* grads, float* m, float* v, int64_t step,
                            float lr, float beta1, float beta2, float eps, float clipnorm, float* scratch,
                            void* stream) {
  return wn_adam_step_guarded(p, params, grads, m, v, step, lr, beta1, beta2, eps, clipnorm, scratch, nullptr, stream);
}
```

### wavenets_amd/model.py

```python
from __future__ import annotations

import ctypes as C
import math
from typing import List, Optional

import numpy as np
import torch

from . import _lib
from . import spec as _spec
from .layers import WaveNetLayer
from .optim import Adam


class _ConvHandle:

  def __init__(self, model, name):
    self._model, self._name = model, name

  @property
  def kernel(self):
    return self._model._tensor(self._name + '/kernel')

  @property
# ... 343 lines not shown
               mapping_activation=None,
               dropout: float = 0,
               dilation_bound: int = 512,
               num_mixtures=None,
               sampling_function: str = 'categorical',
               bits=8,
               skip_channels=None,
               dilation_channels=None,
               use_residual=True,
               use_skip=True,
               final_layers_channels=None,
               l2_reg_factor: float = 0,
               device=None,
               seed: int = 0):
    super().__init__()
    s = _spec.validate(kernel_size, channels, blocks, layers_per_block, activation, conditioning,
                       mapping_layers, mapping_activation, dropout, dilation_bound, num_mixtures,
                       sampling_function, bits, skip_channels, dilation_channels, use_residual,
                       use_skip, final_layers_channels, l2_reg_factor)
    self.spec = s
    self.regularization = s.l2_reg_factor > 0
    self.num_mixtures = num_mixtures
    self.use_skip = use_skip
    self.sampling_function = sampling_function
    self.bits = bits
    self.conditioning = conditioning
    self.dropout = s.dropout
    self.receptive_field = s.receptive_field
    self._device = torch.device(device) if device is not None else torch.device('cuda', 0)
    self._seed = seed
    self._plan = None
    self._cond_inputs = None
    self._names: List[str] = []
    self._ws = {}
    self.built = False
    self.optimizer = None
    self._averaged = None
    self._metrics_from_compilation = []
    self.loss_tracker = _Mean('loss')
    self.reg_loss = _Mean('reg_loss') if self.regularization else None
    self._sample_calls = 0
    self.train_guard_trips = 0
    self.test_guard_trips = 0
    self.score_guard_trips = 0
    self.generation_guard_trips = 0
    self.early_logs = None
    self.range_check = True
    self._last_fwd = None
    self._log_mirror, self._log_event = None, None
    self._drop_step = 0
    self._fused_step_sample = True
    self._drop_armed_step = 0
    self._train_gen = 0
    self._vjp_anchor = None
    dil = s.dilations
    lpb = s.layers_per_block
    self.causal = _ConvHandle(self, 'causal')
    self.wavenet_blocks = [
        WaveNetLayer(kernel=s.kernel_size, channels=s.channels,
                     dilation_rate=dil[b * lpb:(b + 1) * lpb], activation=s.activation,
                     dilation_channels=s.dilation_channels, residual=s.use_residual,
                     skip_channels=s.skip_channels, l2_reg_factor=s.l2_reg_factor, dropout=s.dropout,
                     condition=conditioning is not None, _owner=(self, b))
        for b in range(s.blocks)]
    self.final = [_ConvHandle(self, f'final{i}') for i in range(len(s.final_layers_channels) + 1)]
    self.mapping = [_ConvHandle(self, f'mapping{j}') for j in range(len(s.mapping_layers))] \
        if conditioning == 'global' else None
    if conditioning is None:
      self.build(None)

  def build(self, input_shape):
    if self.built:
      return
    s = self.spec
    cond_inputs = 0
    if self.conditioning is not None:
      cond_inputs = int(input_shape[1][-1])
    self._cond_inputs = cond_inputs
    cfg = _lib.WnConfig()
    cfg.kernel_size, cfg.channels, cfg.blocks = s.kernel_size, s.channels, s.blocks
    cfg.layers_per_block = s.layers_per_block
    cfg.activation = _lib.ACTIVATIONS[s.activation]
    cfg.dilation_bound = s.dilation_bound
    cfg.num_mixtures = s.num_mixtures or 0
    cfg.head = _lib.HEADS[s.sampling_function]
    cfg.bits = s.bits
    cfg.skip_channels = s.skip_channels or 0
    cfg.dilation_channels = s.dilation_channels or 0
    cfg.use_residual, cfg.use_skip = int(s.use_residual), int(s.use_skip)
    if len(s.final_layers_channels) > _lib.WN_MAX_FINAL or len(s.mapping_layers) > _lib.WN_MAX_MAPPING:
      raise NotImplementedError('too many final / mapping layers')
    cfg.n_final = len(s.final_layers_channels)
    for i, c in enumerate(s.final_layers_channels):
      cfg.final_channels[i] = c
    cfg.cond_inputs = cond_inputs
    cfg.n_mapping = len(s.mapping_layers)
    for i, c in enumerate(s.mapping_layers):
      cfg.mapping_channels[i] = c
    cfg.mapping_activation = _lib.ACTIVATIONS[s.mapping_activation]
    cfg.l2_reg_factor = s.l2_reg_factor
    L = _lib.lib()
    plan = L.wn_plan_create(C.byref(cfg))
    if not plan:
      raise ValueError(L.wn_last_error_string().decode())
    self._plan = C.c_void_p(plan)
    if s.dropout > 0:
      if s.dropout >= 1:
        raise ValueError('Dropout must be between 0 and 1.')
      _lib.check(L.wn_plan_set_dropout(self._plan, s.dropout, self._seed, 0))
    shapes = s.param_shapes(cond_inputs)
    n = L.wn_plan_num_tensors(self._plan)
    assert n == len(shapes), (n, len(shapes))
    self._names = [nm for nm, _ in shapes]
    self._offsets, self._shapes = [], []
    off, ln = C.c_int64(), C.c_int64()
    nd, isk = C.c_int32(), C.c_int32()
    sh = (C.c_int64 * 3)()
    for i, (nm, shp) in enumerate(shapes):
      _lib.check(L.wn_plan_tensor_info(self._plan, i, C.byref(off), C.byref(ln), C.byref(nd), sh, C.byref(isk)))
      assert tuple(sh[:nd.value]) == tuple(shp), (nm, tuple(sh[:nd.value]), shp)
      self._offsets.append(off.value)
      self._shapes.append(tuple(shp))
    total = L.wn_plan_param_count(self._plan)
    g = torch.Generator().manual_seed(self._seed)
    flat = torch.zeros(total, dtype=torch.float32)
    for nm, shp, o in zip(self._names, self._shapes, self._offsets):
      if nm.endswith('kernel'):
        if len(shp) == 3:
          fan_in, fan_out = shp[0] * shp[1], shp[0] * shp[2]
        else:
          fan_in, fan_out = shp
        lim = math.sqrt(6.0 / (fan_in + fan_out))
        cnt = int(np.prod(shp))
        flat[o:o + cnt] = (torch.rand(cnt, generator=g) * 2 - 1) * lim
    self.flat_params = torch.nn.Parameter(flat.to(self._device), requires_grad=False)
    self._grad_bucket = torch.zeros(self.flat_params.numel() + 3 + self._TAIL_METRICS, dtype=torch.float32,
                                    device=self._device)
    self.flat_grads = self._grad_bucket[:self.flat_params.numel()]
    self.built = True
    if self.optimizer is not None:
      self.optimizer.build(self)

  def __del__(self):
    try:
      if self._plan is not None:
        _lib.lib().wn_plan_destroy(self._plan)
        self._plan = None
    except Exception:
      pass

  def kernel_report(self) -> str:
    buf = C.create_string_buffer(2048)
    _lib.check(_lib.lib().wn_plan_describe(self._plan, buf, 2048))
    return buf.value.decode()

  def _log_kernels_once(self):
    import os
    import sys
    if not getattr(self, '_kernels_logged', False) and os.environ.get('WN_LOG_KERNELS'):
      self._kernels_logged = True
      print('[wavenets_amd] ' + self.kernel_report(), file=sys.stderr)

  def _tensor(self, name):
    i = self._names.index(name)
    o, shp = self._offsets[i], self._shapes[i]
    return self.flat_params.data[o:o + int(np.prod(shp))].view(*shp)

  @property
  def trainable_variables(self):
    return [self._tensor(n) for n in self._names]

  @property
  def variable_names(self):
    return list(self._names)

  def get_weights(self):
    return [t.detach().cpu().numpy().copy() for t in self.trainable_variables]

  def set_weights(self, weights):
    self._not_averaged('set_weights')
    self._train_gen += 1
    if len(weights) != len(self._names):
      raise ValueError(f'expected {len(self._names)} arrays, got {len(weights)}')
    for t, w in zip(self.trainable_variables, weights):
      w = torch.as_tensor(np.asarray(w), dtype=torch.float32)
      if tuple(w.shape) != tuple(t.shape):
        raise ValueError(f'shape mismatch {tuple(w.shape)} vs {tuple(t.shape)}')
      t.copy_(w)

  def _not_averaged(self, what):
    if self._averaged is not None:
      raise RuntimeError(f'{what} inside averaged_weights(): the scope runs on the averaged weights and is read-only')

  def averaged_weights(self):
    import contextlib

    @contextlib.contextmanager
    def _cm():
      opt = self.optimizer
      if opt is None or not getattr(opt, 'use_ema', False):
        raise RuntimeError('averaged_weights() needs compile(optimizer=Adam(use_ema=True))')
      self._not_averaged('averaged_weights()')
      if not self.built:
        raise RuntimeError('averaged_weights(): the model is not built yet')
      opt.build(self)
      raw = self.flat_params.data
      self._averaged = raw
      self.flat_params.data = opt.ema
      try:
        yield self
      finally:
        self.flat_params.data = raw
        self._averaged = None
    return _cm()

  def gradients(self):
    return [self.flat_grads[o:o + int(np.prod(s))].view(*s) for o, s in zip(self._offsets, self._shapes)]

  def compile(self, **kwargs):
    if 'loss' in kwargs:
      raise ValueError('Loss must be set in the model init function.')
    self._metrics_from_compilation = []
    if 'metrics' in kwargs and kwargs['metrics'] is not None:
      for metric in kwargs['metrics']:
        self._metrics_from_compilation.append(metric)
    self.loss_tracker = _Mean('loss')
    if self.regularization:
      self.reg_loss = _Mean('reg_loss')
    self.optimizer = kwargs.get('optimizer')
    if self.optimizer is not None and self.built:
      self.optimizer.build(self)

  @property
  def metrics(self):
    m = list(self._metrics_from_compilation) + [self.loss_tracker]
    if self.regularization:
      m.append(self.reg_loss)
    return m

  def _workspace(self, key, floats):
    ws = self._ws.get(key)
    if ws is None or ws.numel() < floats:
      ws = torch.empty(int(floats), dtype=torch.float32, device=self._device)
      self._ws[key] = ws
    return ws

  def _split_inputs(self, inputs):
    if self.conditioning is not None:
      x, cond = inputs
      cond = torch.as_tensor(cond, dtype=torch.float32, device=self._device).contiguous()
    else:
      x, cond = inputs, None
    x = torch.as_tensor(x, dtype=torch.float32, device=self._device).contiguous()
    if x.dim() != 3 or x.shape[-1] != 1:
      raise ValueError('input must have shape (batch, samples, 1)')
    if not self.built:
      self.build([tuple(x.shape), tuple(cond.shape)] if cond is not None else tuple(x.shape))
    if cond is not None and (cond.dim() != 2 or cond.shape[0] != x.shape[0] or cond.shape[1] != self._cond_inputs):
      raise ValueError('condition must have shape (batch, n_cond)')
    return x, cond

  def call(self, inputs, training=False):
    x, cond = self._split_inputs(inputs)
    return self._forward_guarded(x, cond, want_probs=True, training=bool(training and self.dropout > 0))

  def _forward_guarded(self, x, cond, want_probs, training):
    B, T = x.shape[0], x.shape[1]
    L = _lib.lib()
    ws = self._workspace('train' if training else 'fwd', L.wn_plan_workspace_floats(self._plan, B, T, int(training)))
    out = torch.empty(B, T, self.spec.out_channels, dtype=torch.float32, device=self._device)
    fn = L.wn_forward_training if training else L.wn_forward
    if training:
      self._train_gen += 1
      self._arm_dropout()

    def run():
      _lib.check(fn(self._plan, _lib.ptr(self.flat_params), _lib.ptr(x), _lib.ptr(cond), B, T,
                    _lib.ptr(out) if want_probs else None, None if want_probs else _lib.ptr(out), _lib.ptr(ws), ws.numel(),
                    _lib.stream_ptr()))
    run()
    slot = L.wn_plan_range_slot(self._plan, B, T, int(training))
    self._last_fwd = (ws[slot:slot + 1].clone(), training)
    if self.range_check and L.wn_debug_value(1) != 1 and self._guard_over(*self._last_fwd):
      with self.exact_fp32():
        run()
    return out

  def range_tripped_last_forward(self) -> bool:
    if self._last_fwd is None:
      return False
    return bool(self._guard_over(*self._last_fwd))

  def forward(self, inputs, training=False):
    return self.call(inputs, training=training)

  def logits(self, inputs):
    x, cond = self._split_inputs(inputs)
    return self._forward_guarded(x, cond, want_probs=False, training=False)

  @staticmethod
  def _world():
    import torch.distributed as dist
    if dist.is_available() and dist.is_initialized():
      return dist.get_world_size()
    return 1

  @staticmethod
# ... 480 lines not shown
```

Baseline: 23.93 million.

## Store relu sign bitmasks in head forward and use them for backward act derivative

The head forward GEMM kernels now write a 1-bit-per-element sign plane for relu or leaky-relu activations. The head backward kernel loads that plane into LDS and applies the derivative from the bits, instead of reading the full fp32 saved activations. This removes most of the global read traffic for the activation derivative in the head backward pass. In exchange it adds extra workspace, extra LDS per wave, bitmask writes in the forward, and new template instantiations.

Measured after the change: 24.27 million (median of 6 runs). 1.4% higher.

```diff
diff --git a/include/wn_hip.h b/include/wn_hip.h
--- a/include/wn_hip.h
+++ b/include/wn_hip.h
@@ -75,6 +75,7 @@
 int wn_debug_value(int key);
 int wn_debug_gen_ts(unsigned long long* out_96);
 int wn_plan_describe(const wn_plan* p, char* buf, int32_t len);
+int wn_plan_describe_train(const wn_plan* p, char* buf, int32_t len);
 int wn_prof_enable(wn_plan* p, int32_t max_launches);
 int wn_prof_read(wn_plan* p, int32_t* launches, float* avg_ms);
 int wn_debug_ws_region(const wn_plan* p, int32_t B, int32_t T, int32_t what, int32_t idx, int64_t* off,
diff --git a/wavenets_amd/_lib.py b/wavenets_amd/_lib.py
--- a/wavenets_amd/_lib.py
+++ b/wavenets_amd/_lib.py
@@ -79,6 +79,7 @@
     'wn_plan_set_dropout': (C.c_int, [_P, C.c_float, C.c_uint64, C.c_uint64]),
     'wn_dropout_key_for': (C.c_uint32, [C.c_uint64, C.c_int32, C.c_uint64]),
     'wn_plan_describe': (C.c_int, [_P, C.c_char_p, C.c_int32]),
+    'wn_plan_describe_train': (C.c_int, [_P, C.c_char_p, C.c_int32]),
     'wn_prof_enable': (C.c_int, [_P, C.c_int32]),
     'wn_prof_read': (C.c_int, [_P, C.POINTER(C.c_int32), C.POINTER(C.c_float)]),
     'wn_debug_ws_region': (C.c_int, [_P, C.c_int32, C.c_int32, C.c_int32, C.c_int32, C.POINTER(C.c_int64),
diff --git a/wavenets_amd/csrc/wn_forward.hip b/wavenets_amd/csrc/wn_forward.hip
--- a/wavenets_amd/csrc/wn_forward.hip
+++ b/wavenets_amd/csrc/wn_forward.hip
@@ -91,6 +91,10 @@
         fp(fwd_paths(p_, e, B_, T_, training_, prep_, rings_ != nullptr, !lf_ ? FWD_LOSS_NONE : lf_->eval ? FWD_LOSS_EVAL : FWD_LOSS_TRAIN)) {}
 
   const float* par(int tensor) const { return params + p->tensors[tensor].off; }
+  float* sign_plane(int j) const {
+    if (!training || (size_t)j >= L.HS.size() || L.HS[j] < 0 || !((head_sign_layers(p, fp, rows) >> j) & 1u)) return nullptr;
+    return ws + L.HS[j];
+  }
 
   static bool pair_free(const std::vector<hipEvent_t>& ev, int used) { return used + 2 <= (int)ev.size(); }
   static void mark(const std::vector<hipEvent_t>& ev, int& used, bool stop, hipStream_t sp) {
@@ -267,7 +271,7 @@
     switch (fp.skip) {
       case FWD_SKIP_FOLD_PLANES:
         rc = Planes(B, T, fp.hc0).operand(ws + L.Z, p->Dp, p->D, p->N, rows * p->Dp).w16(fragbase + p->frag16_foldF)
-                 .bias(ws + L.bfold).act(p->c.activation).absmax_fwd(fam).run(ws + L.HA[0], fp.hc0, s);
+                 .bias(ws + L.bfold).act(p->c.activation).absmax_fwd(fam).signs(sign_plane(0)).run(ws + L.HA[0], fp.hc0, s);
         hin = ws + L.HA[0];
         break;
       case FWD_SKIP_FOLD_ROWS:
@@ -307,7 +311,8 @@
           return WN_OK;
         case FWD_HEAD_PLANES:
           rc = Planes(B, T, c.cout).operand(hin, hc, hc).w16(fragbase + c.frag16).bias(par(c.bias_t))
-                   .act(last ? WN_ACT_LINEAR : p->c.activation).absmax_fwd(last ? nullptr : fam).run(dst, c.cout, s);
+                   .act(last ? WN_ACT_LINEAR : p->c.activation).absmax_fwd(last ? nullptr : fam)
+                   .signs(last ? nullptr : sign_plane(i)).run(dst, c.cout, s);
           break;
         default:
           rc = Gemm(B, T, c.cout, ceil32(c.cout)).seg(hin, hc, hc, 0, fragbase + c.fragF)
diff --git a/wavenets_amd/csrc/wn_gemm16s.hip b/wavenets_amd/csrc/wn_gemm16s.hip
--- a/wavenets_amd/csrc/wn_gemm16s.hip
+++ b/wavenets_amd/csrc/wn_gemm16s.hip
@@ -14,6 +14,7 @@
   static constexpr int PITCH = 36, STAGE = 32 * PITCH * 4;
   static constexpr int REGION = XB * XBUF;
   static constexpr int LDS = NBUF * CHUNK + WAVES * REGION + 32 * JT * 4;
+  static constexpr int SIGNS = WAVES * 1024;
   static constexpr int PT = CHUNK / 16 / THREADS;
   static constexpr int PX = 2 * RT;
   static_assert(STAGE <= REGION, "the output stage lives in the activation ring");
@@ -21,11 +22,13 @@
 
 }
 
-template <int RT, int JT_, int ACT, bool SHIFT = false>
+template <int RT, int JT_, int ACT, bool SHIFT = false, bool SG = false>
 __global__ __launch_bounds__(256, 2) void wn_gemm_planes16s_kernel(WnGemmPlanesArgs a) {
   using C = GS<RT, JT_>;
   constexpr int JT = C::JT, PT = C::PT, PX = C::PX, PITCH = C::PITCH;
-  __shared__ __attribute__((aligned(16))) unsigned char smem[C::LDS];
+  static_assert(!SG || (!SHIFT && (ACT == -2 || ACT == WN_ACT_RELU || ACT == WN_ACT_LEAKY_RELU) && RT * JT == 8),
+                "sign planes: 128 elements per lane, relu / leaky relu");
+  __shared__ __attribute__((aligned(16))) unsigned char smem[C::LDS + (SG && ACT == -2 ? C::SIGNS : 0)];
   const int tid = threadIdx.x;
   const int lane = tid & 63, wave = __builtin_amdgcn_readfirstlane(tid >> 6);
   const int tl = lane & 31, h = lane >> 5;
@@ -35,6 +38,9 @@
   float* sbias = reinterpret_cast<float*>(smem + C::NBUF * C::CHUNK + C::WAVES * C::REGION);
   if (tid < 32 * JT) sbias[tid] = (a.bias && tid < a.N) ? a.bias[tid] : 0.f;
   const bool has_bias = a.bias != nullptr;
+  [[maybe_unused]] const unsigned char* const sgn = smem + C::LDS + wave * 1024;
+  [[maybe_unused]] const unsigned sgn_addr = lds_addr_of(smem) + C::LDS + wave * 1024;
+  [[maybe_unused]] const float slope = SG && ACT == -2 ? wn_dact_from_y(-1.f, a.act) : 0.f;
   __syncthreads();
   float sc = 1.0f, inv_sc = 1.0f;
   if (ACT == -2 && a.absmax_in) pow2_scale(*a.absmax_in, sc, inv_sc);
@@ -109,6 +115,7 @@
 #pragma unroll
         for (int r = 0; r < 16; ++r) acc[rt][j][r] = 0.f;
 
+    if constexpr (SG && ACT == -2) dma16(a.signs_in, (unsigned)(live ? tile : 0) * 1024u + (unsigned)lane * 16u, sgn_addr);
     xdma();
     xdma();
     int xcur = 0;
@@ -285,6 +292,8 @@
       }
       continue;
     }
+    [[maybe_unused]] u32x4 sg = {0u, 0u, 0u, 0u};
+    if constexpr (SG && ACT == -2) sg = *reinterpret_cast<const u32x4*>(sgn + lane * 16);
 #pragma unroll
     for (int rt = 0; rt < RT; ++rt) {
       const int rows_valid = live ? max(0, min(32, a.T - (t0 + 32 * rt))) : 0;
@@ -304,7 +313,14 @@
             const f32x4 bv = *reinterpret_cast<const f32x4*>(sbias + n0);
             v[0] += bv.x; v[1] += bv.y; v[2] += bv.z; v[3] += bv.w;
           }
-          if constexpr (ACT == -2) {
+          [[maybe_unused]] const int sw = (rt * JT + j) >> 1;
+          [[maybe_unused]] const int sb = ((rt * JT + j) & 1) * 16 + 4 * rq;
+          if constexpr (SG && ACT == -2) {
+            if (xok[rt]) {
+#pragma unroll
+              for (int e = 0; e < 4; ++e) v[e] *= ((sg[sw] >> (sb + e)) & 1u) ? 1.f : slope;
+            }
+          } else if constexpr (ACT == -2) {
             if (a.aux && xok[rt]) {
               const f32x4 yv = *(const __attribute__((address_space(1))) f32x4*)(a.aux + (row0 + 32 * rt + tl) * a.ld_aux + n0);
               v[0] *= wn_dact_from_y(yv.x, a.act); v[1] *= wn_dact_from_y(yv.y, a.act);
@@ -313,6 +329,10 @@
           } else {
 #pragma unroll
             for (int e = 0; e < 4; ++e) v[e] = wn_act(v[e], ACT >= 0 ? ACT : a.act);
+            if constexpr (SG) {
+#pragma unroll
+              for (int e = 0; e < 4; ++e) sg[sw] |= (wn_dact_from_y(v[e], ACT) == 1.f ? 1u : 0u) << (sb + e);
+            }
           }
           if (xok[rt]) wmax = wn_absmax_acc(wmax, v[0], v[1], v[2], v[3]);
           acc[rt][j][4 * rq + 0] = v[0]; acc[rt][j][4 * rq + 1] = v[1]; acc[rt][j][4 * rq + 2] = v[2]; acc[rt][j][4 * rq + 3] = v[3];
@@ -321,6 +341,9 @@
         if (rows_valid == 32) store_tile<PITCH, true>(acc[rt][j], stage, dst, voff, (unsigned)(a.ldy * 4), rows_valid, lane);
         else store_tile<PITCH, false>(acc[rt][j], stage, dst, voff, (unsigned)(a.ldy * 4), rows_valid, lane);
       }
+    }
+    if constexpr (SG && ACT >= 0) {
+      if (live) *(__attribute__((address_space(1))) u32x4*)(a.signs_out + tile * 256 + lane * 4) = sg;
     }
   }
   asm volatile("s_waitcnt vmcnt(0)" ::: "memory");
@@ -353,6 +376,7 @@
   int64_t gx = (tiles + 3) / 4;
   if (gx > 512) gx = 512;
 #define WN_GS_LAUNCH(RT_, JT_, ACT_) hipLaunchKernelGGL((wn_gemm_planes16s_kernel<RT_, JT_, ACT_>), dim3((unsigned)gx), dim3(256), 0, s, a)
+#define WN_GS_LAUNCH_G(RT_, JT_, ACT_) hipLaunchKernelGGL((wn_gemm_planes16s_kernel<RT_, JT_, ACT_, false, true>), dim3((unsigned)gx), dim3(256), 0, s, a)
 #define WN_GS_LAUNCH_S(ACT_) hipLaunchKernelGGL((wn_gemm_planes16s_kernel<2, 2, ACT_, true>), dim3((unsigned)gx), dim3(256), 0, s, a)
   if (a.N <= 64) {
     if (a.nshift != a.nplanes || a.plane_stride != 0 || a.nplanes > 4) { wn_set_error("gemm_planes16s: narrow outputs are the shifted form"); return WN_E_UNSUPPORTED; }
@@ -369,9 +393,24 @@
     if (eval) { if (a.row_weight) WN_GS_LAUNCH(1, 8, -6); else WN_GS_LAUNCH(1, 8, -5); }
     else if (a.row_weight) WN_GS_LAUNCH(1, 8, -4);
     else WN_GS_LAUNCH(1, 8, -3);
+  } else if (a.bwd && a.signs_in) {
+    if (a.act != WN_ACT_RELU && a.act != WN_ACT_LEAKY_RELU) { wn_set_error("gemm_planes16s: sign planes are for relu / leaky relu"); return WN_E_UNSUPPORTED; }
+    if (a.N == 256) WN_GS_LAUNCH_G(1, 8, -2);
+    else WN_GS_LAUNCH_G(2, 4, -2);
   } else if (a.bwd) {
     if (a.N == 256) WN_GS_LAUNCH(1, 8, -2);
     else WN_GS_LAUNCH(2, 4, -2);
+  } else if (a.signs_out) {
+    if (a.N == 256) switch (a.act) {
+      case WN_ACT_RELU: WN_GS_LAUNCH_G(1, 8, WN_ACT_RELU); break;
+      case WN_ACT_LEAKY_RELU: WN_GS_LAUNCH_G(1, 8, WN_ACT_LEAKY_RELU); break;
+      default: wn_set_error("gemm_planes16s: sign planes are for relu / leaky relu"); return WN_E_UNSUPPORTED;
+    }
+    else switch (a.act) {
+      case WN_ACT_RELU: WN_GS_LAUNCH_G(2, 4, WN_ACT_RELU); break;
+      case WN_ACT_LEAKY_RELU: WN_GS_LAUNCH_G(2, 4, WN_ACT_LEAKY_RELU); break;
+      default: wn_set_error("gemm_planes16s: sign planes are for relu / leaky relu"); return WN_E_UNSUPPORTED;
+    }
   } else if (a.N == 256) switch (a.act) {
     case WN_ACT_LINEAR: WN_GS_LAUNCH(1, 8, WN_ACT_LINEAR); break;
     case WN_ACT_RELU: WN_GS_LAUNCH(1, 8, WN_ACT_RELU); break;
@@ -385,6 +424,7 @@
     default: WN_GS_LAUNCH(2, 4, -1); break;
   }
 #undef WN_GS_LAUNCH
+#undef WN_GS_LAUNCH_G
 #undef WN_GS_LAUNCH_S
   WN_HIP_CHECK(hipGetLastError());
   return WN_OK;
diff --git a/wavenets_amd/csrc/wn_kernels.h b/wavenets_amd/csrc/wn_kernels.h
--- a/wavenets_amd/csrc/wn_kernels.h
+++ b/wavenets_amd/csrc/wn_kernels.h
@@ -75,6 +75,7 @@
   int32_t bwd;
   const float* absmax_in;
   const float* aux; int32_t ld_aux;
+  uint32_t* signs_out; const uint32_t* signs_in;
   int32_t nshift; int32_t shift[4];
   int32_t cat_loss;
   const int32_t* target;
diff --git a/wavenets_amd/csrc/wn_plan.hip b/wavenets_amd/csrc/wn_plan.hip
--- a/wavenets_amd/csrc/wn_plan.hip
+++ b/wavenets_amd/csrc/wn_plan.hip
@@ -204,16 +204,38 @@
   if (t.fold && p->N >= 2 && p->c.use_residual && (p->c.cond_inputs == 0 || p->frag_condB >= 0) && p->Dp == p->D &&
       (wn_bwd_pair_supported(p->R, p->D, p->KS, p->fold_F0) || wn_bwd_s128_supported(p->R, p->D, p->KS, p->fold_F0)))
     t.bwd = p->R == 128 ? BWD_S128 : BWD_PAIR;
+  {
+    wn_exec none;
+    t.head_signs = (wn_debug_get(30) & 1) ? 0u : head_sign_layers(p, fwd_paths(p, none, 1, 1, true, true, false, FWD_LOSS_NONE), 1);
+  }
   return t;
 }
 
-TrainPaths train_paths(const wn_plan* p, const wn_exec& e, const WsLayout& L, int64_t rows) {
+TrainPaths train_paths(const wn_plan* p, const wn_exec& e, const WsLayout& L, int B, int T) {
   TrainPaths t = train_paths(p);
+  const int64_t rows = (int64_t)B * T;
   t.drop = e.drop_rate > 0.f;
   t.head_split = L.hsplits > 0;
   t.in_split = L.isplits > 0;
   t.rows32 = rows * 2 * p->D * 4 < ((int64_t)1 << 32);
+  t.head_signs = (wn_debug_get(30) & 1) ? 0u : head_sign_layers(p, fwd_paths(p, e, B, T, true, true, false, FWD_LOSS_NONE), rows);
   return t;
+}
+
+bool head_bwd_planes(const wn_plan* p, int i, int64_t rows) {
+  const ConvInfo& c = p->finals[i];
+  return c.frag16B >= 0 && wn_debug_get(1) != 1 && Planes::takes(false, c.cin, c.cout, 1, c.cout, c.cin, rows, {c.cout});
+}
+
+uint32_t head_sign_layers(const wn_plan* p, const FwdPaths& f, int64_t rows) {
+  if (p->c.activation != WN_ACT_RELU && p->c.activation != WN_ACT_LEAKY_RELU) return 0u;
+  uint32_t m = 0;
+  for (int j = 0; j + 1 < (int)p->finals.size(); ++j) {
+    const bool wr = j < f.first_final ? (j == 0 && f.skip == FWD_SKIP_FOLD_PLANES) : f.head[j] == FWD_HEAD_PLANES;
+    const int w = p->finals[j].cout;
+    if (wr && (w == 128 || w == 256) && p->finals[j + 1].cin == w && head_bwd_planes(p, j + 1, rows)) m |= 1u << j;
+  }
+  return m;
 }
 
 static bool gen_head_layers_ok(const wn_plan* p, size_t first, size_t end) {
@@ -417,6 +439,11 @@
         L.hsplits = hs;
         L.hslab = cv.take((int64_t)B * hs * L.head_span);
       }
+    }
+    for (size_t j = 0; j + 1 < p->finals.size(); ++j) {
+      const int w = p->finals[j].cout;
+      const bool relu = p->c.activation == WN_ACT_RELU || p->c.activation == WN_ACT_LEAKY_RELU;
+      L.HS.push_back(relu && (w == 128 || w == 256) ? cv.take((int64_t)B * ((T + 31) / 32) * 256) : (int64_t)-1);
     }
   } else {
     L.bslab = 0; L.bsplits = 0;
@@ -852,6 +879,19 @@
   return WN_OK;
 }
 
+extern "C" int wn_plan_describe_train(const wn_plan* p, char* buf, int32_t len) {
+  if (!p || !buf || len < 1) return WN_E_INVALID;
+  const TrainPaths tp = train_paths(p);
+  std::string layers;
+  for (int j = 0; j < 32; ++j)
+    if ((tp.head_signs >> j) & 1u) layers += std::string(layers.empty() ? "" : ",") + std::to_string(j);
+  if (tp.head_signs)
+    snprintf(buf, (size_t)len, "head backward: act' of head activations %s from sign planes written by their forward kernels "
+             "(wn_gemm_planes16s_kernel, sign forms), other layers from the saved outputs", layers.c_str());
+  else snprintf(buf, (size_t)len, "head backward: act' from the saved outputs (value path)");
+  return WN_OK;
+}
+
 extern "C" int wn_debug_fwd_paths(const wn_plan* p, int32_t B, int32_t T, int32_t training, int32_t loss, char* buf, int32_t len) {
   if (!p || !buf || len < 1 || B < 1 || T < 1 || loss < 0 || loss > 2) return WN_E_INVALID;
   wn_exec none;
diff --git a/wavenets_amd/csrc/wn_plan_internal.h b/wavenets_amd/csrc/wn_plan_internal.h
--- a/wavenets_amd/csrc/wn_plan_internal.h
+++ b/wavenets_amd/csrc/wn_plan_internal.h
@@ -64,6 +64,7 @@
   bool mfused = false;
   bool skipk = false, fold = false, deep16 = false, head_pairs = false;
   bool drop = false, head_split = false, in_split = false, rows32 = true;
+  uint32_t head_signs = 0;
   bool layerk() const { return wg == WG_LAYER || wg == WG_LAYER_INNER; }
   bool pairk() const { return wg == WG_TR_PAIRS; }
   bool headpairs() const { return head_pairs && head_split; }
@@ -71,7 +72,7 @@
   bool operator==(const TrainPaths& o) const {
     return wg == o.wg && bwd == o.bwd && mtr == o.mtr && mfused == o.mfused && skipk == o.skipk && fold == o.fold &&
            deep16 == o.deep16 && head_pairs == o.head_pairs && drop == o.drop && head_split == o.head_split &&
-           in_split == o.in_split && rows32 == o.rows32;
+           in_split == o.in_split && rows32 == o.rows32 && head_signs == o.head_signs;
   }
 };
 
@@ -260,6 +261,7 @@
   int64_t O;
   int64_t skipsum;
   std::vector<int64_t> HA;
+  std::vector<int64_t> HS;
   int64_t logits, probs;
   int64_t target, loss_rows, yt;
   int64_t g_skipsum;
@@ -371,6 +373,8 @@
   Planes& bias(const float* b) { a.bias = b; return *this; }
   Planes& act(int act) { a.act = act; return *this; }
   Planes& absmax_fwd(float* out) { a.absmax_out = out; return *this; }
+  Planes& signs(float* plane) { a.signs_out = reinterpret_cast<uint32_t*>(plane); return *this; }
+  Planes& bwd_signs(const float* plane) { a.signs_in = reinterpret_cast<const uint32_t*>(plane); a.aux = nullptr; a.ld_aux = 0; return *this; }
   Planes& bwd(const float* am_in, float* am_out, const float* aux = nullptr, int ld_aux = 0) {
     a.bwd = 1; a.absmax_in = am_in; a.absmax_out = am_out; a.aux = aux; a.ld_aux = ld_aux;
     return *this;
@@ -464,7 +468,9 @@
 bool fold_ok(const wn_plan* p);
 bool head_pairs_ok(const wn_plan* p);
 TrainPaths train_paths(const wn_plan* p);
-TrainPaths train_paths(const wn_plan* p, const wn_exec& e, const WsLayout& L, int64_t rows);
+TrainPaths train_paths(const wn_plan* p, const wn_exec& e, const WsLayout& L, int B, int T);
+bool head_bwd_planes(const wn_plan* p, int i, int64_t rows);
+uint32_t head_sign_layers(const wn_plan* p, const FwdPaths& f, int64_t rows);
 GenPaths gen_paths(const wn_plan* p, int B, int length, int cu_count, bool relay_area, bool deterministic, const WnSampleCtl& ctl);
 FwdPaths fwd_paths(const wn_plan* p, const wn_exec& e, int B, int T, bool training, bool prep, bool rings, FwdLoss loss);
 int64_t slab_need(int B, int T, int K, int N);
diff --git a/wavenets_amd/csrc/wn_train.hip b/wavenets_amd/csrc/wn_train.hip
--- a/wavenets_amd/csrc/wn_train.hip
+++ b/wavenets_amd/csrc/wn_train.hip
@@ -309,11 +309,13 @@
     for (int i = (int)p->finals.size() - 1; i >= (tp.fold ? 1 : 0); --i) {
       const ConvInfo& c = p->finals[i];
       float* dst = (i == 0) ? head_out : ws + L.GF[i - 1];
-      if (c.frag16B >= 0 && wn_debug_get(1) != 1 && Planes::takes(false, c.cin, c.cout, 1, c.cout, c.cin, rows, {c.cout})) {
-        rc = Planes(B, T, c.cin).operand(ws + L.GF[i], c.cout, c.cout).w16(fragbase + c.frag16B).act(p->c.activation)
-                 .bwd(am_GF(i), i > 0 ? am_GF(i - 1) : (p->c.use_skip ? am_gskip : am_GH(p->N)),
-                      i > 0 ? ws + L.HA[i - 1] : nullptr, i > 0 ? c.cin : 0)
-                 .run(dst, c.cin, s);
+      if (head_bwd_planes(p, i, rows)) {
+        Planes pl(B, T, c.cin);
+        pl.operand(ws + L.GF[i], c.cout, c.cout).w16(fragbase + c.frag16B).act(p->c.activation)
+            .bwd(am_GF(i), i > 0 ? am_GF(i - 1) : (p->c.use_skip ? am_gskip : am_GH(p->N)),
+                 i > 0 ? ws + L.HA[i - 1] : nullptr, i > 0 ? c.cin : 0);
+        if (i > 0 && ((tp.head_signs >> (i - 1)) & 1u)) pl.bwd_signs(ws + L.HS[i - 1]);
+        rc = pl.run(dst, c.cin, s);
         if (rc) return rc;
         continue;
       }
@@ -582,7 +584,7 @@
       if (rc) return rc;
     }
     cond_batched = p->frag_condB >= 0;
-    tp = train_paths(p, e, L, rows);
+    tp = train_paths(p, e, L, B, T);
     pm = (int64_t)p->N * p->D * p->fold_F0 + p->fold_F0;
     if (p->blocks[0].has_skip) {
       const BlockInfo& b0 = p->blocks[0]; const BlockInfo& b1 = p->blocks[p->N > 1 ? 1 : 0];
diff --git a/wavenets_amd/model.py b/wavenets_amd/model.py
--- a/wavenets_amd/model.py
+++ b/wavenets_amd/model.py
@@ -519,7 +519,9 @@
   def kernel_report(self) -> str:
     buf = C.create_string_buffer(2048)
     _lib.check(_lib.lib().wn_plan_describe(self._plan, buf, 2048))
-    return buf.value.decode()
+    text = buf.value.decode()
+    _lib.check(_lib.lib().wn_plan_describe_train(self._plan, buf, 2048))
+    return text + ' | ' + buf.value.decode()
 
   def _log_kernels_once(self):
     import os
```
